# WarranWeng/EBFI-BE

Measured on AMD Instinct MI355X. Metric: interpolated frames/sec (train fwd+bwd) at B=8 256x256, higher is better.
Workload: dtype bf16x3 fwd (f16 KernelConv) / f16 bwd; 1 GPU; EVFIAutoEx (config/train_ours.yml defaults, 5.69 M params) train step: fwd + Lap/census loss + bwd + flat grad all-reduce + Adam; B=8 per GPU, 256x256 frames, TB=16 event bins, Poisson(0.35) event counts; global_batch=8, parallelism=dp1, world_size=1, launch=hipGraph replay of fwd+loss+bwd+grad packing; all-reduce and Adam eager, graph_capture_failed=False, fp16_steps_skipped=0

## Files before the change

ebfi-be_amd/csrc/conv2d.hip:

```cpp
#include <type_traits>

#include "common.hpp"
#include "c16.hpp"

using namespace ebfi;

namespace {

typedef float f32x16 __attribute__((ext_vector_type(16)));

enum { ACT_NONE = 0, ACT_LEAKY = 1, ACT_SIGMOID = 2 };

struct ConvGeom {
    int B, Cin, H, W, Cout, Ho, Wo, pad;
    int groups = 1;
    int store = 0;
};

struct EpiExtra {
    const float *addend;
    const float *mask_y;
    int mask_act;
    float mask_slope;
    _Float16 *out16 = nullptr;
// ... 1774 lines not shown
template <int KS, int DACT>
__global__ __launch_bounds__(256, 2) void conv_wgrad_bf16(const float *__restrict__ x, const float *__restrict__ gout,
                                                         const float *__restrict__ yact, float *__restrict__ slab,
                                                         ConvGeom g, float dslope, int total_tiles, int need_bias) {
    using C = WCfgB<KS>;
    constexpr int KK = KS * KS, WTX = C::WTX, CIB = C::CIB, ROWP = C::ROWP, PLANE = C::PLANE, GP = C::GP;
    constexpr int NI = C::NI, NTAP = C::NTAP;
    extern __shared__ __attribute__((aligned(16))) __bf16 smemb[];
    __bf16 *sG = smemb;
    __bf16 *sB = smemb + 64 * GP;
    unsigned *sG32 = reinterpret_cast<unsigned *>(sG), *sB32 = reinterpret_cast<unsigned *>(sB);

    const int tid = threadIdx.x, lane = tid & 63, wave = tid >> 6;
    const int co_base = blockIdx.y * 64, ci_base = blockIdx.z * CIB;
    const int ci_cnt = min(CIB, g.Cin - ci_base);
    const int mt = wave & 1, th = wave >> 1;
    const int tiles_x = (g.Wo + WTX - 1) / WTX, tiles_y = (g.Ho + WTY - 1) / WTY;
    const int HW = g.H * g.W, HWo = g.Ho * g.Wo;

    f32x16 acc[NTAP];
#pragma unroll
    for (int q = 0; q < NTAP; ++q)
#pragma unroll
        for (int r = 0; r < 16; ++r) acc[q][r] = 0.f;
    for (int i = tid; i < (KS * CIB * PLANE + ROWP) / 2; i += 256) sB32[i] = 0u;

    const int gp = tid & 31, grow = tid >> 5, gpy = gp >> 4, gpx = 2 * (gp & 15);
    const int pc = tid & 15, trow = tid >> 4;
    const unsigned go_bytes = (unsigned)g.Cout * (unsigned)HWo * 4u, x_bytes = (unsigned)g.Cin * (unsigned)HW * 4u;

    float rg[16], ri[2 * NI];
    float bsum = 0.f;
    auto prefetch = [&](int tile) {
        int t = tile;
        const int tx = t % tiles_x; t /= tiles_x;
        const int ty = t % tiles_y;
        const int b = t / tiles_y;
        const int y0 = ty * WTY, x0 = tx * WTX;
        const int iy0 = y0 - g.pad, ix0 = x0 - g.pad;
        const bool live = tile < total_tiles;
        const __amdgpu_buffer_rsrc_t rgo = make_rsrc(gout + (int64_t)(live ? b : 0) * g.Cout * HWo, live ? go_bytes : 0u);
        const __amdgpu_buffer_rsrc_t rya = make_rsrc((DACT ? yact : gout) + (int64_t)(live ? b : 0) * g.Cout * HWo,
                                                     (live && DACT) ? go_bytes : 0u);
        const __amdgpu_buffer_rsrc_t rxi = make_rsrc(x + (int64_t)(live ? b : 0) * g.Cin * HW, live ? x_bytes : 0u);
        const int gy = y0 + gpy, gx0 = x0 + gpx;
        const bool row_ok = gpx < WTX && gy < g.Ho;
        const unsigned base = (unsigned)((co_base + grow) * HWo + gy * g.Wo + gx0) * 4u;
        const unsigned g0 = (row_ok && gx0 < g.Wo) ? base : SENT, g1 = (row_ok && gx0 + 1 < g.Wo) ? base + 4u : SENT;
#pragma unroll
        for (int it = 0; it < 8; ++it) {
            const unsigned step = (unsigned)(8 * it) * (unsigned)HWo * 4u;
            float v0 = buf_ld(rgo, g0 + step), v1 = buf_ld(rgo, g1 + step);
            if constexpr (DACT != 0) {
                v0 *= act_grad_c<DACT>(buf_ld(rya, g0 + step), dslope);
                v1 *= act_grad_c<DACT>(buf_ld(rya, g1 + step), dslope);
            }
            rg[2 * it] = v0;
            rg[2 * it + 1] = v1;
        }
        const int xx = ix0 + 2 * pc;
        const bool c0_ok = xx >= 0 && xx < g.W, c1_ok = xx + 1 >= 0 && xx + 1 < g.W;
#pragma unroll
        for (int it = 0; it < NI; ++it) {
            const int r = it / (CIB / 16), ci = trow + 16 * (it % (CIB / 16));
            const int yy = iy0 + r;
            const bool r_ok = yy >= 0 && yy < g.H;
            const unsigned o = (unsigned)((ci_base + ci) * HW + yy * g.W + xx) * 4u;
            ri[2 * it] = buf_ld(rxi, (r_ok && c0_ok) ? o : SENT);
            ri[2 * it + 1] = buf_ld(rxi, (r_ok && c1_ok) ? o + 4u : SENT);
        }
    };
    auto commit = [&]() {
#pragma unroll
        for (int it = 0; it < 8; ++it) sG32[((grow + 8 * it) * GP) / 2 + gp] = pack_bf16(rg[2 * it], rg[2 * it + 1]);
#pragma unroll
        for (int it = 0; it < NI; ++it) {
            const int r = it / (CIB / 16), ci = trow + 16 * (it % (CIB / 16));
            const float v0 = ri[2 * it], v1 = ri[2 * it + 1];
            const int e = (ci * PLANE + r * ROWP) / 2 + pc;
            sB32[e] = pack_bf16(v0, v1);
            if constexpr (KS == 3) {
                const float nx = __shfl_down(v0, 1, 16);
                sB32[(CIB * PLANE) / 2 + e] = pack_bf16(v1, pc < 15 ? nx : 0.f);
                if (pc > 0) sB32[(2 * CIB * PLANE) / 2 + e - 1] = pack_bf16(v0, v1);
            }
        }
    };

    prefetch(blockIdx.x);
    for (int tile = blockIdx.x; tile < total_tiles; tile += gridDim.x) {
        __syncthreads();
        commit();
        __syncthreads();
        prefetch(tile + gridDim.x);
        if (need_bias && blockIdx.z == 0) {
            const bf16x8 *gq = reinterpret_cast<const bf16x8 *>(sG + (tid & 63) * GP + (tid >> 6) * 16);
            const bf16x8 u = gq[0], v = gq[1];
            float s = 0.f;
#pragma unroll
            for (int j = 0; j < 8; ++j) s += (float)u[j] + (float)v[j];
            bsum += s;
        }
        const __bf16 *ap = sG + (mt * 32 + (lane & 31)) * GP + (lane >> 5) * 8;
        const __bf16 *bp = sB + (lane & 31) * PLANE + (lane >> 5) * 8;
#pragma unroll
        for (int kk = 0; kk < 4; ++kk) {
            const bf16x8 a = *reinterpret_cast<const bf16x8 *>(ap + kk * 16);
#pragma unroll
            for (int j = 0; j < NTAP; ++j) {
                const int q = th * NTAP + j;
                if (q < KK) {
                    const int ky = q / KS, kx = q - ky * KS;
                    const bf16x8 bv = *reinterpret_cast<const bf16x8 *>(bp + kx * CIB * PLANE + ((kk >> 1) + ky) * ROWP +
                                                                        (kk & 1) * 16);
                    acc[j] = __builtin_amdgcn_mfma_f32_32x32x16_bf16(a, bv, acc[j], 0, 0, 0);
                }
            }
        }
    }
    const int64_t wsz = (int64_t)g.Cout * g.Cin * KK;
    float *my = slab + (int64_t)blockIdx.x * (wsz + g.Cout);
    const int ci = lane & 31;
    if (ci < ci_cnt) {
#pragma unroll
        for (int j = 0; j < NTAP; ++j) {
            const int q = th * NTAP + j;
            if (q >= KK) continue;
#pragma unroll
            for (int r = 0; r < 16; ++r) {
                const int co = co_base + mt * 32 + (r & 3) + 8 * (r >> 2) + 4 * (lane >> 5);
                if (co < g.Cout) my[((int64_t)co * KK + q) * g.Cin + ci_base + ci] = acc[j][r];
            }
        }
    }
    if (need_bias && blockIdx.z == 0) {
        __syncthreads();
        float *red = reinterpret_cast<float *>(smemb);
        red[tid] = bsum;
        __syncthreads();
        if (tid < 64 && co_base + tid < g.Cout)
            my[wsz + co_base + tid] = (red[tid] + red[tid + 64]) + (red[tid + 128] + red[tid + 192]);
    }
}

__global__ __launch_bounds__(256) void pack_table_bf16_kernel(const float *__restrict__ src, const int32_t *__restrict__ table,
                                                              int64_t n, __bf16 *__restrict__ out) {
    const int64_t e = (int64_t)blockIdx.x * 256 + threadIdx.x;
    if (e >= n) return;
    const int32_t t = table[e];
    float v = 0.f;
    if (t >= 0) v = src[t & 0x3fffffff];
    const __bf16 h = (__bf16)v;
    out[e] = (t >= 0 && (t & 0x40000000)) ? (__bf16)(v - (float)h) : h;
}

__device__ __forceinline__ void wgrad_reduce_body(const float *__restrict__ slab, int nslabs, int64_t n_weight, int64_t n_total,
                                                  float *__restrict__ gw, float *__restrict__ gb, int perm_cin, int perm_kk) {
    __shared__ float part[4][64];
    const int jj = threadIdx.x & 63, kq = threadIdx.x >> 6;
    const int64_t j = (int64_t)blockIdx.x * 64 + jj;
    float s0 = 0.f, s1 = 0.f, s2 = 0.f, s3 = 0.f;
    if (j < n_total) {
        const float *p = slab + j;
        int k = kq;
        for (; k + 28 < nslabs; k += 32) {
            const float a0 = p[(int64_t)k * n_total], a1 = p[(int64_t)(k + 4) * n_total];
            const float a2 = p[(int64_t)(k + 8) * n_total], a3 = p[(int64_t)(k + 12) * n_total];
            const float a4 = p[(int64_t)(k + 16) * n_total], a5 = p[(int64_t)(k + 20) * n_total];
            const float a6 = p[(int64_t)(k + 24) * n_total], a7 = p[(int64_t)(k + 28) * n_total];
            s0 += a0; s1 += a1; s2 += a2; s3 += a3;
            s0 += a4; s1 += a5; s2 += a6; s3 += a7;
        }
        for (; k + 12 < nslabs; k += 16) {
            s0 += p[(int64_t)k * n_total];
            s1 += p[(int64_t)(k + 4) * n_total];
            s2 += p[(int64_t)(k + 8) * n_total];
            s3 += p[(int64_t)(k + 12) * n_total];
        }
        for (; k < nslabs; k += 4) s0 += p[(int64_t)k * n_total];
    }
    part[kq][jj] = (s0 + s1) + (s2 + s3);
    __syncthreads();
    if (kq == 0 && j < n_total) {
        const float s = (part[0][jj] + part[1][jj]) + (part[2][jj] + part[3][jj]);
        if (j < n_weight) {
            int64_t o = j;
            if (perm_cin > 0) {
                const int ci = (int)(j % perm_cin);
                const int q = (int)((j / perm_cin) % perm_kk);
                const int64_t co = j / ((int64_t)perm_cin * perm_kk);
                o = (co * perm_cin + ci) * perm_kk + q;
            }
            gw[o] = s;
        } else if (gb) gb[j - n_weight] = s;
    }
}
__global__ __launch_bounds__(256) void conv_wgrad_reduce_f32(const float *__restrict__ slab, int nslabs,
                                                             int64_t n_weight, int64_t n_total,
                                                             float *__restrict__ gw, float *__restrict__ gb,
                                                             int perm_cin, int perm_kk) {
    wgrad_reduce_body(slab, nslabs, n_weight, n_total, gw, gb, perm_cin, perm_kk);
}
__global__ __launch_bounds__(256) void conv_wgrad_reduce_tall(const float *__restrict__ slab, int nslabs, int64_t n_weight, int64_t n_total,
                                                              float *__restrict__ gw, float *__restrict__ gb) {
    __shared__ float part[16][16];
    const int jj = threadIdx.x & 15, kq = threadIdx.x >> 4;
    const int64_t j = (int64_t)blockIdx.x * 16 + jj;
    float s0 = 0.f, s1 = 0.f, s2 = 0.f, s3 = 0.f;
    if (j < n_total) {
        const float *p = slab + j;
        int k = kq;
        for (; k + 112 < nslabs; k += 128) {
            float a[8];
#pragma unroll
            for (int i = 0; i < 8; ++i) a[i] = p[(int64_t)(k + 16 * i) * n_total];
            s0 += a[0]; s1 += a[1]; s2 += a[2]; s3 += a[3];
            s0 += a[4]; s1 += a[5]; s2 += a[6]; s3 += a[7];
        }
        for (; k < nslabs; k += 16) s0 += p[(int64_t)k * n_total];
    }
    part[kq][jj] = (s0 + s1) + (s2 + s3);
    __syncthreads();
    if (kq == 0 && j < n_total) {
        float s = 0.f;
#pragma unroll
        for (int i = 0; i < 16; ++i) s += part[i][jj];
        if (j < n_weight) gw[j] = s;
        else if (gb) gb[j - n_weight] = s;
    }
}
struct ReduceItem {
    const float *slab;
    float *gw, *gb;
    int64_t n_weight, n_total;
    int perm_cin;
};
struct ReduceBatch {
    ReduceItem item[4];
};
__global__ __launch_bounds__(256) void conv_wgrad_reduce_batch(ReduceBatch rb, int nslabs) {
    ReduceItem it = rb.item[0];
#pragma unroll
    for (int k = 1; k < 4; ++k)
        if ((int)blockIdx.y == k) it = rb.item[k];
    if ((int64_t)blockIdx.x * 64 >= it.n_total) return;
    wgrad_reduce_body(it.slab, nslabs, it.n_weight, it.n_total, it.gw, it.gb, it.perm_cin, 9);
}

double conv_bytes_fwd(const ConvGeom &g, int kk, bool dact) {
    return 4.0 * ((double)g.B * g.groups * g.Cin * g.H * g.W * (dact ? 2 : 1) + (double)g.B * g.Cout * g.Ho * g.Wo + (double)g.Cout * g.Cin * kk);
}
double conv_bytes_wgrad(const ConvGeom &g, int kk, bool dact, bool side_out) {
    return 4.0 * ((double)g.B * g.groups * g.Cin * g.H * g.W + (double)g.B * g.Cout * g.Ho * g.Wo * (1 + (dact ? 1 : 0) + (side_out ? 1 : 0)) +
                  (double)g.Cout * g.Cin * kk);
}

int make_geom(ConvGeom &g, int B, int Cin, int H, int W, int Cout, int ks, int stride, int pad) {
    if (B < 0 || Cin <= 0 || H <= 0 || W <= 0 || Cout <= 0) return fail(EBFI_ERR_ARG, "conv2d: non-positive dimension");
    if (ks != 1 && ks != 3 && ks != 7) return fail(EBFI_ERR_UNSUPPORTED, "conv2d: kernel size %d (1, 3 and 7 implemented)", ks);
    if (stride != 1 && stride != 2) return fail(EBFI_ERR_UNSUPPORTED, "conv2d: stride %d (1 and 2 implemented)", stride);
    if (pad < 0 || pad > ks) return fail(EBFI_ERR_ARG, "conv2d: padding %d out of range", pad);
    g = ConvGeom{B, Cin, H, W, Cout, (H + 2 * pad - ks) / stride + 1, (W + 2 * pad - ks) / stride + 1, pad};
    if (g.Ho <= 0 || g.Wo <= 0) return fail(EBFI_ERR_ARG, "conv2d: empty output");
    const int64_t lim = (1LL << 31) - (1LL << 26);
    if ((int64_t)(Cin + 64) * H * W * 4 >= lim || (int64_t)(Cout + 64) * g.Ho * g.Wo * 4 >= lim ||
        (int64_t)(Cout + 64) * (Cin + 64) * ks * ks * 4 >= lim)
        return fail(EBFI_ERR_ARG, "conv2d: one sample (or the weight) exceeds the 2 GiB reach of 32-bit buffer offsets");
    return EBFI_OK;
}

template <int KS, int S, bool TR, int DACT>
int launch_fwd_d(hipStream_t st, const float *x, const float *dact_y, const float *w, const float *bias, float *out,
                 const ConvGeom &g, int act, float slope, float dslope) {
    constexpr int CK = KS == 7 ? 2 : 8;
    const int64_t tiles = (int64_t)g.B * ceil_div(g.Ho, TY) * ceil_div(g.Wo, TX);
    if (tiles > 2147483647LL) return fail(EBFI_ERR_ARG, "conv2d: too many tiles");
    const char *name = TR ? "conv_fwd_f32/dgrad" : "conv_fwd_f32/fwd";
    const double flops = 2.0 * g.B * g.Ho * g.Wo * (double)g.Cout * g.Cin * KS * KS;
    if (g.Cout <= 32) {
        dim3 grid((unsigned)tiles, (unsigned)ceil_div(g.Cout, 32));
        ProfScope ps(name, st, flops, conv_bytes_fwd(g, KS * KS, DACT != 0));
        hipLaunchKernelGGL((conv_fwd_f32<KS, S, 1, CK, TR, DACT>), grid, dim3(256), 0, st, x, dact_y, w, bias, out, g, act,
                           slope, dslope);
    } else {
        dim3 grid((unsigned)tiles, (unsigned)ceil_div(g.Cout, 64));
        ProfScope ps(name, st, flops, conv_bytes_fwd(g, KS * KS, DACT != 0));
        hipLaunchKernelGGL((conv_fwd_f32<KS, S, 2, CK, TR, DACT>), grid, dim3(256), 0, st, x, dact_y, w, bias, out, g, act,
                           slope, dslope);
    }
    return check_launch(name);
}

template <int KS, int S, bool TR>
int launch_fwd(hipStream_t st, const float *x, const float *dact_y, const float *w, const float *bias, float *out,
               const ConvGeom &g, int act, float slope, int dact, float dslope) {
    if constexpr (TR) {
        if (dact == ACT_LEAKY) return launch_fwd_d<KS, S, TR, ACT_LEAKY>(st, x, dact_y, w, bias, out, g, act, slope, dslope);
        if (dact == ACT_SIGMOID) return launch_fwd_d<KS, S, TR, ACT_SIGMOID>(st, x, dact_y, w, bias, out, g, act, slope, dslope);
    }
    return launch_fwd_d<KS, S, TR, ACT_NONE>(st, x, dact_y, w, bias, out, g, act, slope, dslope);
}

int pick_wtx(int Wo) {
    int best = 30;
    int64_t best_cols = ceil_div(Wo, 30) * 30;
    for (int w : {28, 26}) {
// ... 748 lines not shown
                const int i = tid + (it0 + ii) * NTB;
                if (it0 + ii < C7_NWP && i < C7_PIECES) {
                    const int row = i >> 1, half = i & 1;
                    u32x4 hv, lv;
#pragma unroll
                    for (int j = 0; j < 4; ++j) {
                        const float v0f = wv[ii][2 * j], v1f = wv[ii][2 * j + 1];
                        const __bf16 a0 = (__bf16)v0f, a1 = (__bf16)v1f;
                        hv[j] = pack_bf16((float)a0, (float)a1);
                        lv[j] = pack_bf16(v0f - (float)a0, v1f - (float)a1);
                    }
                    const int d = 2 * C7S_INB + row * 32 + ((half ^ ((row >> 3) & 1)) << 4);
                    *reinterpret_cast<u32x4 *>(smd + d) = hv;
                    *reinterpret_cast<u32x4 *>(smd + C7_WB + d) = lv;
                }
            }
            __builtin_amdgcn_sched_barrier(0);
        }
        __syncthreads();
#pragma unroll
        for (int ky = 0; ky < 7; ++ky) {
            const int py = (ky + pad) & 1, dy = (py + pad - ky) / 2;
#pragma unroll
            for (int kx = 0; kx < 7; ++kx) {
                const int px = (kx + pad) & 1, dx = (px + pad - kx) / 2;
                const int ra = (ky * 7 + kx) * C7_ROWS + (l31 & 15);
                const char *ap = smd + 2 * C7S_INB + ra * 32 + ((hsel ^ ((ra >> 3) & 1)) << 4);
                const bf16x8 ah = *reinterpret_cast<const bf16x8 *>(ap), al = *reinterpret_cast<const bf16x8 *>(ap + C7_WB);
#pragma unroll
                for (int n = 0; n < 2; ++n) {
                    const int pos = (wave + dy + 1) * C7S_IW + l31 + n * 32 + dx + 1;
                    const char *bp = smd + pos * 32 + ((hsel ^ ((pos >> 3) & 1)) << 4);
                    const bf16x8 bh = *reinterpret_cast<const bf16x8 *>(bp), bl = *reinterpret_cast<const bf16x8 *>(bp + C7S_INB);
                    f32x16 &a = acc[py][px][n];
                    a = __builtin_amdgcn_mfma_f32_32x32x16_bf16(al, bh, a, 0, 0, 0);
                    a = __builtin_amdgcn_mfma_f32_32x32x16_bf16(ah, bl, a, 0, 0, 0);
                    a = __builtin_amdgcn_mfma_f32_32x32x16_bf16(ah, bh, a, 0, 0, 0);
                }
                if ((kx & 1) == 1) __builtin_amdgcn_sched_barrier(0);
            }
        }
    }
    const int u = u0 + wave;
#pragma unroll
    for (int py = 0; py < 2; ++py) {
        const int Y = 2 * u + py;
        if (u >= Hu || Y >= H) continue;
#pragma unroll
        for (int n = 0; n < 2; ++n) {
            const int v = v0 + n * 32 + l31, X = 2 * v;
            if (v >= Wu) continue;
#pragma unroll
            for (int r = 0; r < 16; ++r) {
                const int m = (r & 3) + 8 * (r >> 2) + 4 * hsel;
                if (m >= M) continue;
                float *o = gx + (((int64_t)b * M + m) * H + Y) * W + X;
                if (X + 1 < W && (W & 1) == 0) *reinterpret_cast<float2 *>(o) = make_float2(acc[py][0][n][r], acc[py][1][n][r]);
                else {
                    o[0] = acc[py][0][n][r];
                    if (X + 1 < W) o[1] = acc[py][1][n][r];
                }
            }
        }
    }
}

int launch_conv7s2_dgrad_x3(hipStream_t st, const float *g, const float *w, float *gx, int B, int K, int Hg, int Wg, int M, int H,
                            int W, int pad) {
    if (M > C7_ROWS) return fail(EBFI_ERR_UNSUPPORTED, "conv7s2_dgrad_x3: %d input channels (at most %d)", M, C7_ROWS);
    if (pad != 3) return fail(EBFI_ERR_UNSUPPORTED, "conv7s2_dgrad_x3: pad %d (3 only)", pad);
    if ((int64_t)K * Hg * Wg >= (int64_t)1 << 29) return fail(EBFI_ERR_UNSUPPORTED, "conv7s2_dgrad_x3: a sample of 2 GiB or more");
    if (int rc = ensure_dynamic_lds(reinterpret_cast<const void *>(&conv7s2_dgrad_x3_kernel<3>), C7S_LDS)) return rc;
    const int64_t tiles = (int64_t)B * ceil_div((H + 1) / 2, TYB) * ceil_div((W + 1) / 2, TX);
    {
        ProfScope ps("conv7_x3/dgrad_s2", st, 2.0 * B * (double)Hg * Wg * M * K * 49, 4.0 * B * ((double)K * Hg * Wg + (double)M * H * W));
        hipLaunchKernelGGL(conv7s2_dgrad_x3_kernel<3>, dim3((unsigned)tiles), dim3(NTB), C7S_LDS, st, g, w, gx, K, Hg, Wg, M, H, W);
    }
    return check_launch("conv7s2_dgrad_x3");
}

int launch_conv7_x3(hipStream_t st, const float *x, const float *w, const float *bias, float *out, int B, int K, int H, int W,
                    int M, int Ho, int Wo, int pad, int tr, int act, float slope, const char *role) {
    if (M > C7_ROWS) return fail(EBFI_ERR_UNSUPPORTED, "conv7_x3: %d output channels (at most %d)", M, C7_ROWS);
    if ((int64_t)K * H * W >= (int64_t)1 << 29) return fail(EBFI_ERR_UNSUPPORTED, "conv7_x3: a sample of 2 GiB or more");
    if (int rc = ensure_dynamic_lds(reinterpret_cast<const void *>(&conv7_x3_kernel), C7_LDS)) return rc;
    const int64_t tiles = (int64_t)B * ceil_div(Ho, TYB) * ceil_div(Wo, TX);
    {
        ProfScope ps(role, st, 2.0 * B * (double)Ho * Wo * M * K * 49, 4.0 * B * ((double)K * H * W + (double)M * Ho * Wo));
        hipLaunchKernelGGL(conv7_x3_kernel, dim3((unsigned)tiles), dim3(NTB), C7_LDS, st, x, w, bias, out, K, H, W, M, Ho, Wo, pad,
                           tr, act, slope);
    }
    return check_launch("conv7_x3");
}

int conv_forward_bf16_impl(const char *who, int x3, const void *input, const void *weight, const void *bias, void *output, int B,
                           int Cin, int H, int W, int Cout, int ksize, int stride, int pad, int act, float slope,
                           void *workspace, size_t workspace_bytes, void *stream) {
    if (!input || !output || (!weight && !(x3 && workspace))) return fail(EBFI_ERR_ARG, "%s: null argument", who);
    if (act < 0 || act > 2) return fail(EBFI_ERR_ARG, "%s: unknown activation %d", who, act);
    const bool k7 = x3 && ksize == 7 && stride == 1 && weight;
    if (!k7 && (stride != 1 || (ksize != 1 && ksize != 3)))
        return fail(EBFI_ERR_UNSUPPORTED, "%s: k=%d stride=%d (k in {1,3}, stride 1; split precision also k=7 with <= 16 output channels)",
                    who, ksize, stride);
    ConvGeom g;
    if (int rc = make_geom(g, B, Cin, H, W, Cout, ksize, stride, pad)) return rc;
    if (B == 0) return EBFI_OK;
    hipStream_t st = static_cast<hipStream_t>(stream);
    const float *x = static_cast<const float *>(input), *w = static_cast<const float *>(weight);
    const float *bs = static_cast<const float *>(bias);
    float *o = static_cast<float *>(output);
    if (k7) return launch_conv7_x3(st, x, w, bs, o, B, Cin, H, W, Cout, g.Ho, g.Wo, pad, 0, act, slope, "conv7_x3/fwd");
    if (ksize == 3) return launch_fwd_bf16<3>(st, x, nullptr, w, bs, o, g, 0, act, slope, 0, 0.f, workspace, workspace_bytes, x3);
    return launch_fwd_bf16<1>(st, x, nullptr, w, bs, o, g, 0, act, slope, 0, 0.f, workspace, workspace_bytes, x3);
}

int conv_backward_data_bf16_impl(const char *who, int x3, const void *grad_output, const void *saved_output, const void *weight,
                                 void *grad_input, int B, int Cin, int H, int W, int Cout, int ksize, int stride, int pad,
                                 int act, float slope, void *workspace, size_t workspace_bytes, void *stream) {
    if (!grad_output || !grad_input || (!weight && !(x3 && workspace))) return fail(EBFI_ERR_ARG, "%s: null argument", who);
    if (act != ACT_NONE && !saved_output) return fail(EBFI_ERR_ARG, "%s: activation needs saved_output", who);
    const bool k7 = x3 && ksize == 7 && stride == 1 && weight && act == ACT_NONE;
    if (stride != 1 || pad > ksize - 1 || (!k7 && ksize != 1 && ksize != 3))
        return fail(EBFI_ERR_UNSUPPORTED, "%s: k=%d stride=%d pad=%d", who, ksize, stride, pad);
    ConvGeom f;
    if (int rc = make_geom(f, B, Cin, H, W, Cout, ksize, stride, pad)) return rc;
    if (B == 0) return EBFI_OK;
    if (k7 && Cout == 3 && Cin == 16 && (int64_t)B * H * W >= 64 * 1024)
        return launch_conv7_thin_dgrad(static_cast<hipStream_t>(stream), static_cast<const float *>(grad_output), nullptr,
                                       static_cast<const float *>(weight), static_cast<float *>(grad_input), B, H, W, f.Ho, f.Wo, pad,
                                       ACT_NONE, 0.f);
    if (k7)
        return launch_conv7_x3(static_cast<hipStream_t>(stream), static_cast<const float *>(grad_output),
                               static_cast<const float *>(weight), nullptr, static_cast<float *>(grad_input), B, Cout, f.Ho, f.Wo,
                               Cin, H, W, ksize - 1 - pad, 1, ACT_NONE, 0.f, "conv7_x3/dgrad");
    ConvGeom g{B, Cout, f.Ho, f.Wo, Cin, H, W, ksize - 1 - pad};
    hipStream_t st = static_cast<hipStream_t>(stream);
    const float *go = static_cast<const float *>(grad_output), *yo = static_cast<const float *>(saved_output);
    const float *w = static_cast<const float *>(weight);
    float *gi = static_cast<float *>(grad_input);
    if (ksize == 3)
        return launch_fwd_bf16<3>(st, go, yo, w, nullptr, gi, g, 1, ACT_NONE, 0.f, act, slope, workspace, workspace_bytes, x3);
    return launch_fwd_bf16<1>(st, go, yo, w, nullptr, gi, g, 1, ACT_NONE, 0.f, act, slope, workspace, workspace_bytes, x3);
}
}

extern "C" int ebfi_pack_table_bf16(const float *src, const int32_t *table, int64_t n, void *out, void *stream) {
    if (!src || !table || !out || n < 0) return fail(EBFI_ERR_ARG, "pack_table_bf16: null argument");
    if (n == 0) return EBFI_OK;
    hipStream_t st = static_cast<hipStream_t>(stream);
    ProfScope ps("pack_table_bf16", st, 0.0, 10.0 * (double)n);
    hipLaunchKernelGGL(pack_table_bf16_kernel, dim3((unsigned)ceil_div(n, 256)), dim3(256), 0, st, src, table, n,
                       static_cast<__bf16 *>(out));
    return check_launch("pack_table_bf16");
}

extern "C" size_t ebfi_conv2d_packed_bytes(int Cin, int Cout, int ksize, int transposed) {
    return transposed ? 2 * bf16_pack_bytes(Cin, Cout, ksize) : 2 * bf16_pack_bytes(Cout, Cin, ksize);
}

extern "C" int ebfi_conv2d_pack_bf16x3(const void *weight, int Cin, int Cout, int ksize, int transposed, void *packed,
                                       size_t packed_bytes, void *stream) {
    if (!weight || !packed) return fail(EBFI_ERR_ARG, "conv2d_pack_bf16x3: null argument");
    if (Cin <= 0 || Cout <= 0 || (ksize != 1 && ksize != 3)) return fail(EBFI_ERR_ARG, "conv2d_pack_bf16x3: Cin %d Cout %d k %d", Cin, Cout, ksize);
    const int M = transposed ? Cin : Cout, K = transposed ? Cout : Cin, K16 = (K + 15) / 16 * 16;
    if (packed_bytes < ebfi_conv2d_packed_bytes(Cin, Cout, ksize, transposed))
        return fail(EBFI_ERR_WORKSPACE, "conv2d_pack_bf16x3: %zu bytes < required %zu", packed_bytes,
                    ebfi_conv2d_packed_bytes(Cin, Cout, ksize, transposed));
    hipStream_t st = static_cast<hipStream_t>(stream);
    const int64_t total = (int64_t)ksize * ksize * M * K16;
    ProfScope ps("conv_pack_w_bf16", st);
    hipLaunchKernelGGL(conv_pack_w_bf16, dim3((unsigned)ceil_div(total, 256)), dim3(256), 0, st, static_cast<const float *>(weight),
                       static_cast<__bf16 *>(packed), M, K, K16, ksize * ksize, transposed, 1);
    return check_launch("conv_pack_w_bf16");
}

extern "C" int ebfi_conv2d_forward_bf16mma(const void *input, const void *weight, const void *bias, void *output, int B,
                                           int Cin, int H, int W, int Cout, int ksize, int stride, int pad, int act,
                                           float slope, void *workspace, size_t workspace_bytes, void *stream) {
    return conv_forward_bf16_impl("conv2d_forward_bf16mma", 0, input, weight, bias, output, B, Cin, H, W, Cout, ksize, stride, pad,
                                  act, slope, workspace, workspace_bytes, stream);
}

extern "C" int ebfi_conv2d_backward_data_bf16mma(const void *grad_output, const void *saved_output, const void *weight,
                                                 void *grad_input, int B, int Cin, int H, int W, int Cout, int ksize,
                                                 int stride, int pad, int act, float slope, void *workspace,
                                                 size_t workspace_bytes, void *stream) {
    return conv_backward_data_bf16_impl("conv2d_backward_data_bf16mma", 0, grad_output, saved_output, weight, grad_input, B, Cin,
                                        H, W, Cout, ksize, stride, pad, act, slope, workspace, workspace_bytes, stream);
}

extern "C" int ebfi_conv2d_forward_bf16x3(const void *input, const void *weight, const void *bias, void *output, int B,
                                          int Cin, int H, int W, int Cout, int ksize, int stride, int pad, int act,
                                          float slope, void *workspace, size_t workspace_bytes, void *stream) {
    return conv_forward_bf16_impl("conv2d_forward_bf16x3", 1, input, weight, bias, output, B, Cin, H, W, Cout, ksize, stride, pad,
                                  act, slope, workspace, workspace_bytes, stream);
}

extern "C" int ebfi_conv2d_backward_data_bf16x3(const void *grad_output, const void *saved_output, const void *weight,
                                                void *grad_input, int B, int Cin, int H, int W, int Cout, int ksize,
                                                int stride, int pad, int act, float slope, void *workspace,
                                                size_t workspace_bytes, void *stream) {
    return conv_backward_data_bf16_impl("conv2d_backward_data_bf16x3", 1, grad_output, saved_output, weight, grad_input, B, Cin,
                                        H, W, Cout, ksize, stride, pad, act, slope, workspace, workspace_bytes, stream);
}

extern "C" int ebfi_conv2d_backward_data_s2_bf16x3(const void *grad_preact, const void *weight, void *grad_input, int B, int Cin,
                                                   int H, int W, int Cout, int ksize, int pad, void *stream) {
    if (!grad_preact || !weight || !grad_input) return fail(EBFI_ERR_ARG, "conv2d_backward_data_s2_bf16x3: null argument");
    if (ksize != 7) return fail(EBFI_ERR_UNSUPPORTED, "conv2d_backward_data_s2_bf16x3: k=%d (7 only)", ksize);
    ConvGeom f;
    if (int rc = make_geom(f, B, Cin, H, W, Cout, ksize, 2, pad)) return rc;
    if (B == 0) return EBFI_OK;
    return launch_conv7s2_dgrad_x3(static_cast<hipStream_t>(stream), static_cast<const float *>(grad_preact),
                                   static_cast<const float *>(weight), static_cast<float *>(grad_input), B, Cout, f.Ho, f.Wo, Cin, H, W,
                                   pad);
}

extern "C" int ebfi_conv2d_forward(const void *input, const void *weight, const void *bias, void *output, int B, int Cin,
                                   int H, int W, int Cout, int ksize, int stride, int pad, int act, float slope,
                                   int dtype, void *stream) {
    if (!input || !weight || !output) return fail(EBFI_ERR_ARG, "conv2d_forward: null argument");
    if (dtype != EBFI_F32) return fail(EBFI_ERR_UNSUPPORTED, "conv2d_forward: dtype %d not implemented (fp32 only)", dtype);
    if (act < 0 || act > 2) return fail(EBFI_ERR_ARG, "conv2d_forward: unknown activation %d", act);
    ConvGeom g;
    if (int rc = make_geom(g, B, Cin, H, W, Cout, ksize, stride, pad)) return rc;
    if (B == 0) return EBFI_OK;
    hipStream_t st = static_cast<hipStream_t>(stream);
    const float *x = static_cast<const float *>(input), *w = static_cast<const float *>(weight);
    const float *bs = static_cast<const float *>(bias);
    float *o = static_cast<float *>(output);
    if (ksize == 3 && stride == 1) return launch_fwd<3, 1, false>(st, x, nullptr, w, bs, o, g, act, slope, 0, 0.f);
    if (ksize == 3 && stride == 2) return launch_fwd<3, 2, false>(st, x, nullptr, w, bs, o, g, act, slope, 0, 0.f);
    if (ksize == 1 && stride == 1) return launch_fwd<1, 1, false>(st, x, nullptr, w, bs, o, g, act, slope, 0, 0.f);
    if (ksize == 7 && stride == 1) return launch_fwd<7, 1, false>(st, x, nullptr, w, bs, o, g, act, slope, 0, 0.f);
    if (ksize == 7 && stride == 2) return launch_fwd<7, 2, false>(st, x, nullptr, w, bs, o, g, act, slope, 0, 0.f);
    return fail(EBFI_ERR_UNSUPPORTED, "conv2d_forward: k=%d stride=%d not implemented", ksize, stride);
}

extern "C" int ebfi_conv2d_backward_data(const void *grad_output, const void *saved_output, const void *weight,
                                         void *grad_input, int B, int Cin, int H, int W, int Cout, int ksize,
                                         int stride, int pad, int act, float slope, int dtype, void *stream) {
    if (!grad_output || !weight || !grad_input) return fail(EBFI_ERR_ARG, "conv2d_backward_data: null argument");
    if (dtype != EBFI_F32) return fail(EBFI_ERR_UNSUPPORTED, "conv2d_backward_data: dtype %d not implemented", dtype);
    if (act != ACT_NONE && !saved_output) return fail(EBFI_ERR_ARG, "conv2d_backward_data: activation needs saved_output");
    if (stride != 1 || pad > ksize - 1)
        return fail(EBFI_ERR_UNSUPPORTED, "conv2d_backward_data: stride 1 and pad <= k-1 only (got s=%d p=%d k=%d); strided layers "
                    "zero-insert grad_output on the host side", stride, pad, ksize);
    ConvGeom f;
    if (int rc = make_geom(f, B, Cin, H, W, Cout, ksize, stride, pad)) return rc;
    if (B == 0) return EBFI_OK;
    ConvGeom g{B, Cout, f.Ho, f.Wo, Cin, H, W, ksize - 1 - pad};
    hipStream_t st = static_cast<hipStream_t>(stream);
    const float *go = static_cast<const float *>(grad_output), *yo = static_cast<const float *>(saved_output);
    const float *w = static_cast<const float *>(weight);
    float *gi = static_cast<float *>(grad_input);
    if (ksize == 3) return launch_fwd<3, 1, true>(st, go, yo, w, nullptr, gi, g, ACT_NONE, 0.f, act, slope);
    if (ksize == 7) return launch_fwd<7, 1, true>(st, go, yo, w, nullptr, gi, g, ACT_NONE, 0.f, act, slope);
    return launch_fwd<1, 1, true>(st, go, yo, w, nullptr, gi, g, ACT_NONE, 0.f, act, slope);
}

extern "C" size_t ebfi_conv2d_backward_weight_workspace(int B, int Cin, int H, int W, int Cout, int ksize, int stride,
                                                        int pad, int dtype) {
    (void)dtype;
    ConvGeom g;
    if (make_geom(g, B, Cin, H, W, Cout, ksize, stride, pad) != EBFI_OK) return 0;
    int slabs = wgrad_splits(g, ksize, stride);
    if (thin_wgrad_geometry(g, ksize, stride).kind != 0 && thin_wgrad_slabs(g) > slabs)
        slabs = thin_wgrad_slabs(g);
    if (const ShiftPlan sp = shift_wgrad_geometry(g, ksize, stride); sp.kind != 0 && shift_wgrad_slabs(g, sp) > slabs)
        slabs = shift_wgrad_slabs(g, sp);
    return (size_t)slabs * ((size_t)Cout * Cin * ksize * ksize + Cout) * sizeof(float);
}

extern "C" int ebfi_conv2d_backward_weight_ex(const void *input, const void *grad_output, const void *saved_output,
                                              void *grad_weight, void *grad_bias, void *grad_preact_out, int B, int Cin,
                                              int H, int W, int Cout, int ksize, int stride, int pad, int act, float slope,
                                              void *workspace, size_t workspace_bytes, int dtype, void *stream);

extern "C" int ebfi_conv2d_backward_weight(const void *input, const void *grad_output, const void *saved_output,
                                           void *grad_weight, void *grad_bias, int B, int Cin, int H, int W, int Cout,
                                           int ksize, int stride, int pad, int act, float slope, void *workspace,
                                           size_t workspace_bytes, int dtype, void *stream) {
    return ebfi_conv2d_backward_weight_ex(input, grad_output, saved_output, grad_weight, grad_bias, nullptr, B, Cin, H, W,
                                          Cout, ksize, stride, pad, act, slope, workspace, workspace_bytes, dtype, stream);
}

extern "C" int ebfi_conv2d_backward_weight_ex(const void *input, const void *grad_output, const void *saved_output,
                                              void *grad_weight, void *grad_bias, void *grad_preact_out, int B, int Cin,
                                              int H, int W, int Cout, int ksize, int stride, int pad, int act, float slope,
                                              void *workspace, size_t workspace_bytes, int dtype, void *stream) {
    if (!input || !grad_output || !grad_weight) return fail(EBFI_ERR_ARG, "conv2d_backward_weight: null argument");
    const bool bf16mma = dtype == EBFI_F32_BF16MMA && stride == 1 && (ksize == 1 || ksize == 3);
    const bool x3 = dtype == EBFI_F32_BF16X3MMA && stride == 1 && (ksize == 1 || ksize == 3 || ksize == 7);
    if (dtype != EBFI_F32 && dtype != EBFI_F32_BF16MMA && dtype != EBFI_F32_BF16X3MMA)
        return fail(EBFI_ERR_UNSUPPORTED, "conv2d_backward_weight: dtype %d not implemented", dtype);
    if (act != ACT_NONE && !saved_output) return fail(EBFI_ERR_ARG, "conv2d_backward_weight: activation needs saved_output");
    ConvGeom g;
    if (int rc = make_geom(g, B, Cin, H, W, Cout, ksize, stride, pad)) return rc;
    const size_t need = ebfi_conv2d_backward_weight_workspace(B, Cin, H, W, Cout, ksize, stride, pad, dtype);
    if (!workspace || workspace_bytes < need)
        return fail(EBFI_ERR_WORKSPACE, "conv2d_backward_weight: workspace %zu bytes < required %zu", workspace_bytes, need);
    hipStream_t st = static_cast<hipStream_t>(stream);
    const int64_t n_weight = (int64_t)Cout * Cin * ksize * ksize, n_total = n_weight + Cout;
    if (B == 0) {
        (void)hipMemsetAsync(grad_weight, 0, (size_t)n_weight * sizeof(float), st);
        if (grad_bias) (void)hipMemsetAsync(grad_bias, 0, (size_t)Cout * sizeof(float), st);
// ... 677 lines not shown
```

ebfi-be_amd/csrc/fuse.hip:

```cpp
#include "common.hpp"
#include "c16.hpp"

using namespace ebfi;

namespace {

typedef float f4 __attribute__((ext_vector_type(4)));

__global__ __launch_bounds__(256) void src_fwd_kernel(const float *__restrict__ a0, const float *__restrict__ s0,
                                                      const float *__restrict__ a1, const float *__restrict__ s1,
                                                      const float *__restrict__ x, float *__restrict__ out, int C, int64_t HW4,
                                                      int64_t total4, int64_t a_bs4) {
    const int64_t i = (int64_t)blockIdx.x * 256 + threadIdx.x;
    if (i >= total4) return;
    const int64_t bc = i / HW4, r = i - bc * HW4;
    const int64_t b = bc / C, c = bc - b * C;
    const f4 zero = {0.f, 0.f, 0.f, 0.f};
    const f4 xv = x ? reinterpret_cast<const f4 *>(x)[i] : zero;
    const int64_t ia = b * a_bs4 + c * HW4 + r;
    const f4 v0 = reinterpret_cast<const f4 *>(a0)[ia], v1 = reinterpret_cast<const f4 *>(a1)[ia];
    const float k0 = s0[bc], k1 = s1 ? s1[bc] : 1.f;
    f4 *o = reinterpret_cast<f4 *>(out);
    o[(b * 2 * C + c) * HW4 + r] = v0 * k0 + xv;
    o[(b * 2 * C + C + c) * HW4 + r] = v1 * k1 + xv;
// ... 160 lines not shown
    }
    ScaleSlot{slot}.record(amax);
}

__global__ __launch_bounds__(256) void src_fwd_c16_kernel(const float *__restrict__ a0, const float *__restrict__ s0,
                                                          const float *__restrict__ a1, const float *__restrict__ s1,
                                                          const float *__restrict__ x, float *__restrict__ out,
                                                          _Float16 *__restrict__ out16, float *__restrict__ slot, int C, int64_t HW4,
                                                          int W4, int64_t total, int64_t a_bs4) {
    saturate_fp16_conversions();
    const int64_t i = (int64_t)blockIdx.x * 256 + threadIdx.x;
    float amax = 0.f;
    if (i < total) {
        const int64_t q = i % HW4, bg = i / HW4;
        const int64_t G8 = 2 * C / 8, b = bg / G8, cg = bg - b * G8;
        const int64_t co = cg * 8;
        const bool second = co >= C;
        const int64_t c = second ? co - C : co;
        const f4 *pa = reinterpret_cast<const f4 *>(second ? a1 : a0) + b * a_bs4 + c * HW4 + q;
        const f4 *px = reinterpret_cast<const f4 *>(x) + (b * C + c) * HW4 + q;
        const float *ps = (second ? s1 : s0) + b * C + c;
        f4 v[8];
#pragma unroll
        for (int e = 0; e < 8; ++e) v[e] = pa[e * HW4] * ps[e] + px[e * HW4];
        if (out) {
            f4 *o = reinterpret_cast<f4 *>(out) + (b * 2 * C + co) * HW4 + q;
#pragma unroll
            for (int e = 0; e < 8; ++e) o[e * HW4] = v[e];
        }
        c16_store_quad(out16, c16_piece(b, 2 * C / 16, cg / 2, HW4, q, W4, (int)(cg & 1)), v, slot[0], amax);
    }
    ScaleSlot{slot}.record(amax);
}

template <bool A16>
__global__ __launch_bounds__(256) void src_bwd_c16_kernel(const float *__restrict__ gout, const float *__restrict__ a0,
                                                          const float *__restrict__ s0, const float *__restrict__ a1,
                                                          const float *__restrict__ s1, _Float16 *__restrict__ ga16,
                                                          float *__restrict__ slot, float *__restrict__ gx, float *__restrict__ gs0p,
                                                          float *__restrict__ gs1p, int B, int C, int64_t HW4, int W4, int64_t a_bs4,
                                                          int nslice, float mask_slope, const float *__restrict__ a_slot = nullptr) {
    saturate_fp16_conversions();
    __shared__ float red[4][16];
    const int G8 = C / 8;
    const int slice = blockIdx.x % nslice, bg = blockIdx.x / nslice;
    const int b = bg / G8, cg = bg - b * G8, c = cg * 8;
    const int64_t q0 = HW4 * slice / nslice, q1 = HW4 * (slice + 1) / nslice;
    float k0[8], k1[8], d0[8], d1[8];
#pragma unroll
    for (int e = 0; e < 8; ++e) k0[e] = s0[b * C + c + e], k1[e] = s1[b * C + c + e], d0[e] = 0.f, d1[e] = 0.f;
    const float sc = slot[0];
    float amax = 0.f;
    auto dm = [&](const f4 &v) {
        f4 m;
        m.x = v.x > 0.f ? 1.f : mask_slope; m.y = v.y > 0.f ? 1.f : mask_slope;
        m.z = v.z > 0.f ? 1.f : mask_slope; m.w = v.w > 0.f ? 1.f : mask_slope;
        return m;
    };
    const f4 *g0 = reinterpret_cast<const f4 *>(gout) + ((int64_t)b * 2 * C + c) * HW4;
    const f4 *g1 = reinterpret_cast<const f4 *>(gout) + ((int64_t)b * 2 * C + C + c) * HW4;
    const f4 *p0 = reinterpret_cast<const f4 *>(a0) + (int64_t)b * a_bs4 + (int64_t)c * HW4;
    const f4 *p1 = reinterpret_cast<const f4 *>(a1) + (int64_t)b * a_bs4 + (int64_t)c * HW4;
    [[maybe_unused]] const _Float16 *img = reinterpret_cast<const _Float16 *>(a0);
    [[maybe_unused]] const float ainv = A16 ? 1.f / a_slot[0] : 1.f;
    auto quad_from_image = [&](int64_t piece0, f4 (&v)[8]) {
        u4 pc[4];
#pragma unroll
        for (int j = 0; j < 4; ++j) pc[j] = *reinterpret_cast<const u4 *>(img + (piece0 + j) * 8);
#pragma unroll
        for (int e = 0; e < 8; ++e) {
#pragma unroll
            for (int j = 0; j < 4; ++j) {
                const unsigned wd = pc[j][e >> 1];
                const _Float16 hv = __builtin_bit_cast(_Float16, (unsigned short)((e & 1) ? (wd >> 16) : (wd & 0xffffu)));
                v[e][j] = (float)hv * ainv;
            }
        }
    };
    f4 *ox = reinterpret_cast<f4 *>(gx) + ((int64_t)b * C + c) * HW4;
    for (int64_t q = q0 + threadIdx.x; q < q1; q += 256) {
        f4 u0[8], u1[8], w[8], va[8];
#pragma unroll
        for (int e = 0; e < 8; ++e) u0[e] = g0[e * HW4 + q], u1[e] = g1[e * HW4 + q];
#pragma unroll
        for (int e = 0; e < 8; ++e) ox[e * HW4 + q] = u0[e] + u1[e];
        const int64_t pc0 = c16_piece(b, 2 * C / 16, cg / 2, HW4, q, W4, cg & 1);
        const int64_t pc1 = c16_piece(b, 2 * C / 16, (C + c) / 16, HW4, q, W4, ((C + c) >> 3) & 1);
        if constexpr (A16) quad_from_image(pc0, va);
#pragma unroll
        for (int e = 0; e < 8; ++e) {
            const f4 v = A16 ? va[e] : p0[e * HW4 + q];
            d0[e] += (u0[e].x * v.x + u0[e].y * v.y) + (u0[e].z * v.z + u0[e].w * v.w);
            w[e] = u0[e] * k0[e] * dm(v);
        }
        c16_store_quad(ga16, pc0, w, sc, amax);
        if constexpr (A16) quad_from_image(pc1, va);
#pragma unroll
        for (int e = 0; e < 8; ++e) {
            const f4 v = A16 ? va[e] : p1[e * HW4 + q];
            d1[e] += (u1[e].x * v.x + u1[e].y * v.y) + (u1[e].z * v.z + u1[e].w * v.w);
            w[e] = u1[e] * k1[e] * dm(v);
        }
        c16_store_quad(ga16, pc1, w, sc, amax);
    }
#pragma unroll
    for (int e = 0; e < 8; ++e)
#pragma unroll
        for (int d = 32; d >= 1; d >>= 1) {
            d0[e] += __shfl_xor(d0[e], d, 64);
            d1[e] += __shfl_xor(d1[e], d, 64);
        }
    if ((threadIdx.x & 63) == 0) {
#pragma unroll
        for (int e = 0; e < 8; ++e) red[threadIdx.x >> 6][e] = d0[e], red[threadIdx.x >> 6][8 + e] = d1[e];
    }
    __syncthreads();
    if (threadIdx.x < 16) {
        const float v = (red[0][threadIdx.x] + red[1][threadIdx.x]) + (red[2][threadIdx.x] + red[3][threadIdx.x]);
        float *dst = threadIdx.x < 8 ? gs0p : gs1p;
        dst[((int64_t)slice * B + b) * C + c + (threadIdx.x & 7)] = v;
    }
    ScaleSlot{slot}.record(amax);
}

int check_planes(const char *who, int B, int C, int64_t HW) {
    if (B < 0 || C <= 0 || HW <= 0) return fail(EBFI_ERR_ARG, "%s: bad dimensions", who);
    if (HW % 4 != 0) return fail(EBFI_ERR_UNSUPPORTED, "%s: H*W must be a multiple of 4 (got %lld)", who, (long long)HW);
    if ((int64_t)B * C > 2147483647LL) return fail(EBFI_ERR_ARG, "%s: too many planes", who);
    return EBFI_OK;
}


constexpr int SC_MAX_LAYERS = 32, SC_MAX_K = 8;
struct ScalarBank {
    const float *w[SC_MAX_LAYERS];
    const float *b[SC_MAX_LAYERS];
};

__global__ __launch_bounds__(256) void scalar_conv_fwd_kernel(ScalarBank bank, const float *__restrict__ v, float *__restrict__ out,
                                                              int B, int K, int C, float slope) {
    const int s = blockIdx.x;
    const float *w = nullptr, *bias = nullptr;
#pragma unroll
    for (int j = 0; j < SC_MAX_LAYERS; ++j)
        if (j == s) { w = bank.w[j]; bias = bank.b[j]; }
    for (int i = threadIdx.x; i < B * C; i += 256) {
        const int b = i / C, c = i - b * C;
        float acc = bias ? bias[c] : 0.f;
        for (int k = 0; k < K; ++k) acc = fmaf(v[b * K + k], w[c * K + k], acc);
        out[((int64_t)s * B + b) * C + c] = acc > 0.f ? acc : acc * slope;
    }
}

__global__ __launch_bounds__(256) void scalar_conv_bwd_kernel(ScalarBank bank, const float *__restrict__ v, const float *__restrict__ out,
                                                              const float *__restrict__ gout, float *__restrict__ gw, float *__restrict__ gb,
                                                              float *__restrict__ gv, int S, int B, int K, int C, float slope) {
    for (int i = threadIdx.x; i < S * C; i += 256) {
        const int s = i / C, c = i - s * C;
        float aw[SC_MAX_K], ab = 0.f;
#pragma unroll
        for (int k = 0; k < SC_MAX_K; ++k) aw[k] = 0.f;
        for (int b = 0; b < B; ++b) {
            const int64_t o = ((int64_t)s * B + b) * C + c;
            const float gp = gout[o] * (out[o] > 0.f ? 1.f : slope);
            ab += gp;
#pragma unroll
            for (int k = 0; k < SC_MAX_K; ++k)
                if (k < K) aw[k] = fmaf(gp, v[b * K + k], aw[k]);
        }
        if (gb) gb[i] = ab;
        if (gw) {
#pragma unroll
            for (int k = 0; k < SC_MAX_K; ++k)
                if (k < K) gw[(int64_t)i * K + k] = aw[k];
        }
    }
    if (gv) {
        const int wave = threadIdx.x >> 6, lane = threadIdx.x & 63;
        for (int p = wave; p < B * K; p += 4) {
            const int b = p / K, k = p - b * K;
            float acc = 0.f;
            for (int s = 0; s < S; ++s) {
                const float *w = nullptr;
#pragma unroll
                for (int j = 0; j < SC_MAX_LAYERS; ++j)
                    if (j == s) w = bank.w[j];
                for (int c = lane; c < C; c += 64) {
                    const int64_t o = ((int64_t)s * B + b) * C + c;
                    acc = fmaf(gout[o] * (out[o] > 0.f ? 1.f : slope), w[c * K + k], acc);
                }
            }
#pragma unroll
            for (int d = 32; d >= 1; d >>= 1) acc += __shfl_xor(acc, d, 64);
            if (lane == 0) gv[p] = acc;
        }
    }
}
}

extern "C" int ebfi_scale_residual_cat_forward_ex(const float *a0, const float *s0, const float *a1, const float *s1,
                                                  const float *x, float *out, int B, int C, int64_t HW, int64_t a_batch_stride,
                                                  void *stream);
extern "C" int ebfi_scale_residual_cat_forward(const float *a0, const float *s0, const float *a1, const float *s1,
                                               const float *x, float *out, int B, int C, int64_t HW, void *stream) {
    return ebfi_scale_residual_cat_forward_ex(a0, s0, a1, s1, x, out, B, C, HW, (int64_t)C * HW, stream);
}

extern "C" int ebfi_scale_residual_cat_forward_ex(const float *a0, const float *s0, const float *a1, const float *s1,
                                                  const float *x, float *out, int B, int C, int64_t HW, int64_t a_batch_stride,
                                                  void *stream) {
    if (!a0 || !s0 || !a1 || !out) return fail(EBFI_ERR_ARG, "scale_residual_cat_forward: null argument");
    if (a_batch_stride % 4 != 0 || a_batch_stride < (int64_t)C * HW) return fail(EBFI_ERR_ARG, "scale_residual_cat_forward: batch stride");
    if (int rc = check_planes("scale_residual_cat_forward", B, C, HW)) return rc;
    if (B == 0) return EBFI_OK;
    hipStream_t st = static_cast<hipStream_t>(stream);
    const int64_t total4 = (int64_t)B * C * HW / 4;
    {
        ProfScope ps("scale_residual_cat_fwd", st, 0.0, 20.0 * B * C * (double)HW);
        hipLaunchKernelGGL(src_fwd_kernel, dim3((unsigned)ceil_div(total4, 256)), dim3(256), 0, st, a0, s0, a1, s1, x, out, C, HW / 4,
                           total4, a_batch_stride / 4);
    }
    return check_launch("scale_residual_cat_fwd");
}

extern "C" int ebfi_scale_residual_cat_backward_ex(const float *grad_out, const float *a0, const float *s0, const float *a1,
                                                   const float *s1, float *grad_a0, float *grad_a1, float *grad_x,
                                                   float *grad_s0, float *grad_s1, int B, int C, int64_t HW,
                                                   int64_t a_batch_stride, int64_t grad_a_batch_stride, int mask_leaky,
                                                   float mask_slope, void *stream);
extern "C" int ebfi_scale_residual_cat_backward(const float *grad_out, const float *a0, const float *s0, const float *a1,
                                                const float *s1, float *grad_a0, float *grad_a1, float *grad_x,
                                                float *grad_s0, float *grad_s1, int B, int C, int64_t HW, void *stream) {
    return ebfi_scale_residual_cat_backward_ex(grad_out, a0, s0, a1, s1, grad_a0, grad_a1, grad_x, grad_s0, grad_s1, B, C, HW,
                                               (int64_t)C * HW, (int64_t)C * HW, 0, 0.f, stream);
}

extern "C" int ebfi_scale_residual_cat_backward_ex(const float *grad_out, const float *a0, const float *s0, const float *a1,
                                                   const float *s1, float *grad_a0, float *grad_a1, float *grad_x,
                                                   float *grad_s0, float *grad_s1, int B, int C, int64_t HW,
                                                   int64_t a_batch_stride, int64_t grad_a_batch_stride, int mask_leaky,
                                                   float mask_slope, void *stream) {
    if (a_batch_stride % 4 != 0 || grad_a_batch_stride % 4 != 0 || a_batch_stride < (int64_t)C * HW ||
        grad_a_batch_stride < (int64_t)C * HW || (mask_leaky && !a1))
        return fail(EBFI_ERR_ARG, "scale_residual_cat_backward: batch stride / mask");
    if (!grad_out || !a0 || !s0 || !grad_a0 || !grad_a1 || !grad_s0 || (s1 && (!a1 || !grad_s1)))
        return fail(EBFI_ERR_ARG, "scale_residual_cat_backward: null argument");
    if (int rc = check_planes("scale_residual_cat_backward", B, C, HW)) return rc;
    if (B == 0) return EBFI_OK;
    hipStream_t st = static_cast<hipStream_t>(stream);
    {
        ProfScope ps("scale_residual_cat_bwd", st, 0.0, 28.0 * B * C * (double)HW);
        hipLaunchKernelGGL(src_bwd_kernel, dim3((unsigned)(B * C)), dim3(256), 0, st, grad_out, a0, s0, a1, s1, grad_a0, grad_a1,
                           grad_x, grad_s0, grad_s1, C, HW / 4, a_batch_stride / 4, grad_a_batch_stride / 4, mask_leaky, mask_slope);
    }
    return check_launch("scale_residual_cat_bwd");
}

extern "C" int ebfi_to_c16(const float *src, const float *mask_y, float mask_slope, void *dst16, void *slot, int B, int C, int H, int W,
                           void *stream) {
    const int64_t HW = (int64_t)H * W;
    if (!src || !dst16 || !slot) return fail(EBFI_ERR_ARG, "to_c16: null argument");
    if (W % 4 != 0) return fail(EBFI_ERR_UNSUPPORTED, "to_c16: W %% 4 != 0 (W = %d)", W);
    if (C % 16 != 0) return fail(EBFI_ERR_UNSUPPORTED, "to_c16: %d channels (multiples of 16)", C);
    if (int rc = check_planes("to_c16", B, C, HW)) return rc;
    if (!aligned16(src) || !aligned16(dst16) || (mask_y && !aligned16(mask_y))) return fail(EBFI_ERR_ARG, "to_c16: 16-byte aligned tensors");
    if (B == 0) return EBFI_OK;
    hipStream_t st = static_cast<hipStream_t>(stream);
    const int64_t total = (int64_t)B * (C / 8) * (HW / 4);
    {
        ProfScope ps("to_c16", st, 0.0, (mask_y ? 10.0 : 6.0) * B * C * (double)HW);
        hipLaunchKernelGGL(to_c16_kernel, dim3((unsigned)ceil_div(total, 256)), dim3(256), 0, st, src, mask_y, mask_slope,
                           static_cast<_Float16 *>(dst16), static_cast<float *>(slot), C, HW / 4, W / 4, total);
    }
    return check_launch("to_c16");
}

extern "C" int ebfi_to_c16_cat2(const float *src0, int C0, const float *src1, int C1, void *dst16, void *slot, int B, int H, int W,
                                void *stream) {
    const int64_t HW = (int64_t)H * W;
    if (!src0 || !src1 || !dst16 || !slot) return fail(EBFI_ERR_ARG, "to_c16_cat2: null argument");
    if (W % 4 != 0) return fail(EBFI_ERR_UNSUPPORTED, "to_c16_cat2: W %% 4 != 0 (W = %d)", W);
    if (C0 < 8 || C1 < 8 || C0 % 8 != 0 || C1 % 8 != 0 || (C0 + C1) % 16 != 0)
        return fail(EBFI_ERR_UNSUPPORTED, "to_c16_cat2: %d + %d channels (multiples of 8, a multiple of 16 together)", C0, C1);
    if (int rc = check_planes("to_c16_cat2", B, C0 + C1, HW)) return rc;
    if (!aligned16(src0) || !aligned16(src1) || !aligned16(dst16)) return fail(EBFI_ERR_ARG, "to_c16_cat2: 16-byte aligned tensors");
    if (B == 0) return EBFI_OK;
    hipStream_t st = static_cast<hipStream_t>(stream);
    const int64_t total = (int64_t)B * ((C0 + C1) / 8) * (HW / 4);
    {
        ProfScope ps("to_c16/cat2", st, 0.0, 6.0 * B * (C0 + C1) * (double)HW);
        hipLaunchKernelGGL(to_c16_cat2_kernel, dim3((unsigned)ceil_div(total, 256)), dim3(256), 0, st, src0, C0, src1, C1,
                           static_cast<_Float16 *>(dst16), static_cast<float *>(slot), HW / 4, W / 4, total);
    }
    return check_launch("to_c16/cat2");
}

extern "C" int ebfi_scale_residual_cat_forward_c16(const float *a0, const float *s0, const float *a1, const float *s1, const float *x,
                                                   float *out, void *out16, void *slot, int B, int C, int H, int W,
                                                   int64_t a_batch_stride, void *stream) {
    const int64_t HW = (int64_t)H * W;
    if (!a0 || !s0 || !a1 || !s1 || !x || !out16 || !slot) return fail(EBFI_ERR_ARG, "scale_residual_cat_forward_c16: null argument");
    if (W % 4 != 0) return fail(EBFI_ERR_UNSUPPORTED, "scale_residual_cat_forward_c16: W %% 4 != 0 (W = %d)", W);
    if (a_batch_stride % 4 != 0 || a_batch_stride < (int64_t)C * HW) return fail(EBFI_ERR_ARG, "scale_residual_cat_forward_c16: batch stride");
    if (C % 8 != 0) return fail(EBFI_ERR_UNSUPPORTED, "scale_residual_cat_forward_c16: %d channels (multiples of 8)", C);
    if (int rc = check_planes("scale_residual_cat_forward_c16", B, C, HW)) return rc;
    if (B == 0) return EBFI_OK;
    hipStream_t st = static_cast<hipStream_t>(stream);
    const int64_t total = (int64_t)B * (2 * C / 8) * (HW / 4);
    {
        ProfScope ps("scale_residual_cat_fwd", st, 0.0, (out ? 24.0 : 16.0) * B * C * (double)HW);
        hipLaunchKernelGGL(src_fwd_c16_kernel, dim3((unsigned)ceil_div(total, 256)), dim3(256), 0, st, a0, s0, a1, s1, x, out,
                           static_cast<_Float16 *>(out16), static_cast<float *>(slot), C, HW / 4, W / 4, total, a_batch_stride / 4);
    }
    return check_launch("scale_residual_cat_fwd");
}

extern "C" int ebfi_scale_residual_cat_backward_slices(void) { return 8; }

extern "C" int ebfi_scale_residual_cat_backward_c16(const float *grad_out, const float *a0, const float *s0, const float *a1,
                                                    const float *s1, void *grad_a16, void *slot, float *grad_x, float *grad_s0_part,
                                                    float *grad_s1_part, int B, int C, int H, int W, int64_t a_batch_stride,
                                                    float mask_slope, void *stream) {
    const int64_t HW = (int64_t)H * W;
    if (W % 4 != 0) return fail(EBFI_ERR_UNSUPPORTED, "scale_residual_cat_backward_c16: W %% 4 != 0 (W = %d)", W);
    if (!grad_out || !a0 || !s0 || !a1 || !s1 || !grad_a16 || !slot || !grad_x || !grad_s0_part || !grad_s1_part)
        return fail(EBFI_ERR_ARG, "scale_residual_cat_backward_c16: null argument");
    if (a_batch_stride % 4 != 0 || a_batch_stride < (int64_t)C * HW) return fail(EBFI_ERR_ARG, "scale_residual_cat_backward_c16: batch stride");
    if (C % 16 != 0) return fail(EBFI_ERR_UNSUPPORTED, "scale_residual_cat_backward_c16: %d channels (multiples of 16)", C);
    if (int rc = check_planes("scale_residual_cat_backward_c16", B, C, HW)) return rc;
    if (B == 0) return EBFI_OK;
    hipStream_t st = static_cast<hipStream_t>(stream);
    const int nslice = ebfi_scale_residual_cat_backward_slices();
    {
        ProfScope ps("scale_residual_cat_bwd", st, 0.0, 24.0 * B * C * (double)HW);
        hipLaunchKernelGGL(src_bwd_c16_kernel<false>, dim3((unsigned)(B * (C / 8) * nslice)), dim3(256), 0, st, grad_out, a0, s0, a1, s1,
                           static_cast<_Float16 *>(grad_a16), static_cast<float *>(slot), grad_x, grad_s0_part, grad_s1_part, B, C,
                           HW / 4, W / 4, a_batch_stride / 4, nslice, mask_slope, nullptr);
    }
    return check_launch("scale_residual_cat_bwd");
}

extern "C" int ebfi_scale_residual_cat_backward_c16a(const float *grad_out, const void *a16, const void *a_slot, const float *s0,
                                                     const float *s1, void *grad_a16, void *slot, float *grad_x, float *grad_s0_part,
                                                     float *grad_s1_part, int B, int C, int H, int W, float mask_slope, void *stream) {
    const int64_t HW = (int64_t)H * W;
    if (W % 4 != 0) return fail(EBFI_ERR_UNSUPPORTED, "scale_residual_cat_backward_c16a: W %% 4 != 0 (W = %d)", W);
    if (!grad_out || !a16 || !a_slot || !s0 || !s1 || !grad_a16 || !slot || !grad_x || !grad_s0_part || !grad_s1_part)
        return fail(EBFI_ERR_ARG, "scale_residual_cat_backward_c16a: null argument");
    if (C % 16 != 0) return fail(EBFI_ERR_UNSUPPORTED, "scale_residual_cat_backward_c16a: %d channels (multiples of 16)", C);
    if (!aligned16(a16) || !aligned16(grad_a16)) return fail(EBFI_ERR_ARG, "scale_residual_cat_backward_c16a: 16-byte aligned images");
    if (int rc = check_planes("scale_residual_cat_backward_c16a", B, C, HW)) return rc;
    if (B == 0) return EBFI_OK;
    hipStream_t st = static_cast<hipStream_t>(stream);
    const int nslice = ebfi_scale_residual_cat_backward_slices();
    {
        ProfScope ps("scale_residual_cat_bwd", st, 0.0, 20.0 * B * C * (double)HW);
        hipLaunchKernelGGL(src_bwd_c16_kernel<true>, dim3((unsigned)(B * (C / 8) * nslice)), dim3(256), 0, st, grad_out,
                           static_cast<const float *>(a16), s0, static_cast<const float *>(a16), s1, static_cast<_Float16 *>(grad_a16),
                           static_cast<float *>(slot), grad_x, grad_s0_part, grad_s1_part, B, C, HW / 4, W / 4, (int64_t)0, nslice,
                           mask_slope, static_cast<const float *>(a_slot));
    }
    return check_launch("scale_residual_cat_bwd");
}

extern "C" int ebfi_gather_sum(const float *src, const int32_t *idx, float *out, int64_t n_out, int R, void *stream) {
    if (!src || !idx || !out) return fail(EBFI_ERR_ARG, "gather_sum: null argument");
    if (n_out < 0 || R <= 0) return fail(EBFI_ERR_ARG, "gather_sum: bad dimensions");
    if (n_out == 0) return EBFI_OK;
    hipStream_t st = static_cast<hipStream_t>(stream);
    hipLaunchKernelGGL(gather_sum_kernel, dim3((unsigned)ceil_div(n_out, 256)), dim3(256), 0, st, src, idx, out, n_out, R);
    return check_launch("gather_sum");
}

extern "C" int ebfi_prodmean_forward(const float *a, const float *b, float *out, int64_t planes, int64_t HW, void *stream) {
    if (!a || !b || !out) return fail(EBFI_ERR_ARG, "prodmean_forward: null argument");
    if (planes < 0 || planes > 2147483647LL || HW <= 0) return fail(EBFI_ERR_ARG, "prodmean_forward: bad dimensions");
    if (HW % 4 != 0) return fail(EBFI_ERR_UNSUPPORTED, "prodmean_forward: H*W must be a multiple of 4");
    if (planes == 0) return EBFI_OK;
    hipStream_t st = static_cast<hipStream_t>(stream);
    {
        ProfScope ps("prodmean_fwd", st, 0.0, 8.0 * planes * (double)HW);
        hipLaunchKernelGGL(prodmean_fwd_kernel, dim3((unsigned)planes), dim3(256), 0, st, a, b, out, HW / 4);
    }
    return check_launch("prodmean_fwd");
}

extern "C" int ebfi_prodmean_backward(const float *a, const float *b, const float *grad_out, float *grad_a, float *grad_b,
                                      int64_t planes, int64_t HW, void *stream) {
    if (!a || !b || !grad_out || !grad_a || !grad_b) return fail(EBFI_ERR_ARG, "prodmean_backward: null argument");
    if (planes < 0 || HW <= 0) return fail(EBFI_ERR_ARG, "prodmean_backward: bad dimensions");
    if (HW % 4 != 0) return fail(EBFI_ERR_UNSUPPORTED, "prodmean_backward: H*W must be a multiple of 4");
    if (planes == 0) return EBFI_OK;
    hipStream_t st = static_cast<hipStream_t>(stream);
    const int64_t total4 = planes * HW / 4;
    {
        ProfScope ps("prodmean_bwd", st, 0.0, 16.0 * planes * (double)HW);
        hipLaunchKernelGGL(prodmean_bwd_kernel, dim3((unsigned)ceil_div(total4, 256)), dim3(256), 0, st, a, b, grad_out, grad_a, grad_b,
                           HW / 4, total4);
    }
    return check_launch("prodmean_bwd");
}

static int scalar_bank(ScalarBank &bank, const void *const *weights, const void *const *biases, int S, int B, int K, int C, const char *what) {
    if (!weights || S < 1 || S > SC_MAX_LAYERS || K < 1 || K > SC_MAX_K || B < 0 || C < 1 || (int64_t)S * B * C > (1 << 20))
        return fail(EBFI_ERR_ARG, "%s: S = %d layers (<= %d), K = %d (<= %d), B = %d, C = %d", what, S, SC_MAX_LAYERS, K, SC_MAX_K, B, C);
    for (int j = 0; j < SC_MAX_LAYERS; ++j) {
        bank.w[j] = j < S ? static_cast<const float *>(weights[j]) : nullptr;
        bank.b[j] = (j < S && biases) ? static_cast<const float *>(biases[j]) : nullptr;
        if (j < S && !bank.w[j]) return fail(EBFI_ERR_ARG, "%s: weight %d is NULL", what, j);
    }
    return EBFI_OK;
}

extern "C" int ebfi_scalar_conv_forward(const float *v, const void *const *weights, const void *const *biases, float *out, int S, int B,
                                        int K, int C, float slope, void *stream) {
    ScalarBank bank;
    if (int rc = scalar_bank(bank, weights, biases, S, B, K, C, "scalar_conv_forward")) return rc;
    if (!v || !out) return fail(EBFI_ERR_ARG, "scalar_conv_forward: null argument");
    if (B == 0) return EBFI_OK;
    hipStream_t st = static_cast<hipStream_t>(stream);
    {
        ProfScope ps("scalar_conv_fwd", st, 2.0 * S * B * C * K, 4.0 * (S * (double)C * (K + 1) + B * K + (double)S * B * C));
        hipLaunchKernelGGL(scalar_conv_fwd_kernel, dim3((unsigned)S), dim3(256), 0, st, bank, v, out, B, K, C, slope);
    }
    return check_launch("scalar_conv_fwd");
}

extern "C" int ebfi_scalar_conv_backward(const float *v, const void *const *weights, const float *out, const float *grad_out,
                                         float *grad_weight, float *grad_bias, float *grad_v, int S, int B, int K, int C, float slope,
                                         void *stream) {
    ScalarBank bank;
    if (int rc = scalar_bank(bank, weights, nullptr, S, B, K, C, "scalar_conv_backward")) return rc;
    if (!v || !out || !grad_out) return fail(EBFI_ERR_ARG, "scalar_conv_backward: null argument");
    if (B == 0) return EBFI_OK;
    hipStream_t st = static_cast<hipStream_t>(stream);
    {
        ProfScope ps("scalar_conv_bwd", st, 4.0 * S * B * C * K, 4.0 * (2.0 * S * B * C + 2.0 * S * C * (K + 1) + 2.0 * B * K));
        hipLaunchKernelGGL(scalar_conv_bwd_kernel, dim3(1), dim3(256), 0, st, bank, v, out, grad_out, grad_weight, grad_bias, grad_v,
                           S, B, K, C, slope);
    }
    return check_launch("scalar_conv_bwd");
}
```

ebfi-be_amd/csrc/imgops.hip:

```cpp
#include "common.hpp"

using namespace ebfi;

namespace {

__device__ __forceinline__ int reflect(int i, int n) {
    if (i < 0) return -i;
    if (i >= n) return 2 * (n - 1) - i;
    return i;
}

__global__ void gauss5_fwd_kernel(const float *__restrict__ x, float *__restrict__ out, int64_t planes, int H, int W,
                                  float factor) {
    const int64_t idx = (int64_t)blockIdx.x * blockDim.x + threadIdx.x;
    const int64_t hw = (int64_t)H * W;
    if (idx >= planes * hw) return;
    const int64_t p = idx / hw;
    const int y = (int)((idx - p * hw) / W), xx = (int)(idx - p * hw - (int64_t)y * W);
    const float k[5] = {1.f / 16, 4.f / 16, 6.f / 16, 4.f / 16, 1.f / 16};
    const float *src = x + p * hw;
    float acc = 0.f;
#pragma unroll
    for (int i = 0; i < 5; ++i) {
        const float *row = src + (int64_t)reflect(y + i - 2, H) * W;
        float h = 0.f;
#pragma unroll
        for (int j = 0; j < 5; ++j) h += k[j] * row[reflect(xx + j - 2, W)];
        acc += k[i] * h;
    }
    out[idx] = acc * factor;
}

__global__ void gauss5_bwd_kernel(const float *__restrict__ gout, float *__restrict__ gin, int64_t planes, int H, int W,
                                  float factor) {
    const int64_t idx = (int64_t)blockIdx.x * blockDim.x + threadIdx.x;
    const int64_t hw = (int64_t)H * W;
    if (idx >= planes * hw) return;
    const int64_t p = idx / hw;
    const int y = (int)((idx - p * hw) / W), xx = (int)(idx - p * hw - (int64_t)y * W);
    const float k[5] = {1.f / 16, 4.f / 16, 6.f / 16, 4.f / 16, 1.f / 16};
    const float *src = gout + p * hw;
    int vy[3], vx[3], ny = 0, nx = 0;
    vy[ny++] = y;
    if (y >= 1 && y <= 2) vy[ny++] = -y;
    if (y >= H - 3 && y <= H - 2) vy[ny++] = 2 * (H - 1) - y;
    vx[nx++] = xx;
    if (xx >= 1 && xx <= 2) vx[nx++] = -xx;
    if (xx >= W - 3 && xx <= W - 2) vx[nx++] = 2 * (W - 1) - xx;
    float acc = 0.f;
    for (int a = 0; a < ny; ++a)
        for (int i = 0; i < 5; ++i) {
            const int oy = vy[a] - i + 2;
            if (oy < 0 || oy >= H) continue;
            const float *row = src + (int64_t)oy * W;
            float h = 0.f;
            for (int b = 0; b < nx; ++b)
#pragma unroll
                for (int j = 0; j < 5; ++j) {
                    const int ox = vx[b] - j + 2;
                    if (ox >= 0 && ox < W) h += k[j] * row[ox];
                }
            acc += k[i] * h;
        }
    gin[idx] = acc * factor;
}

constexpr int CT = 16, CR = 3, CTW = CT + 2 * CR;

__device__ __forceinline__ void census_stage(const float *__restrict__ x, const float *__restrict__ y, int C, int H, int W,
                                             int b, int ty0, int tx0, float (*gx)[CTW + 1], float (*gy)[CTW + 1]) {
    const int64_t hw = (int64_t)H * W;
    const float invc = 1.f / (float)C;
    for (int i = threadIdx.x; i < CTW * CTW; i += CT * CT) {
        const int ly = i / CTW, lx = i - ly * CTW;
        const int py = ty0 + ly - CR, px = tx0 + lx - CR;
        float sx = 0.f, sy = 0.f;
        if (py >= 0 && py < H && px >= 0 && px < W) {
            const int64_t o = (int64_t)b * C * hw + (int64_t)py * W + px;
            for (int c = 0; c < C; ++c) {
                sx += x[o + c * hw];
                sy += y[o + c * hw];
            }
            sx *= invc;
            sy *= invc;
        }
        gx[ly][lx] = sx;
        gy[ly][lx] = sy;
    }
}

__device__ __forceinline__ float census_t(float d) { return d * rsqrtf(0.81f + d * d); }

__global__ __launch_bounds__(CT *CT) void census_fwd_kernel(const float *__restrict__ x, const float *__restrict__ y,
                                                            float *__restrict__ partial, int C, int H, int W) {
    __shared__ float gx[CTW][CTW + 1], gy[CTW][CTW + 1];
    __shared__ float red[4];
    const int b = blockIdx.z, ty0 = blockIdx.y * CT, tx0 = blockIdx.x * CT;
    census_stage(x, y, C, H, W, b, ty0, tx0, gx, gy);
    __syncthreads();
    const int ly = threadIdx.x / CT, lx = threadIdx.x % CT;
    const int py = ty0 + ly, px = tx0 + lx;
    float acc = 0.f;
    if (py >= CR && py < H - CR && px >= CR && px < W - CR) {
        const float cx = gx[ly + CR][lx + CR], cy = gy[ly + CR][lx + CR];
#pragma unroll
        for (int i = 0; i < 7; ++i)
#pragma unroll
            for (int j = 0; j < 7; ++j) {
                const float u = census_t(gx[ly + i][lx + j] - cx) - census_t(gy[ly + i][lx + j] - cy);
                const float q = u * u;
                acc += q / (0.1f + q);
            }
        acc *= (1.f / 49.f);
    }
#pragma unroll
    for (int d = 32; d >= 1; d >>= 1) acc += __shfl_xor(acc, d, 64);
    if ((threadIdx.x & 63) == 0) red[threadIdx.x >> 6] = acc;
    __syncthreads();
    if (threadIdx.x == 0)
        partial[((int64_t)b * gridDim.y + blockIdx.y) * gridDim.x + blockIdx.x] = (red[0] + red[1]) + (red[2] + red[3]);
}

__device__ __forceinline__ float census_dterm(float dx, float dy) {
    const float rx = rsqrtf(0.81f + dx * dx);
    const float u = dx * rx - census_t(dy);
    const float den = 0.1f + u * u;
    return (0.2f * u / (den * den)) * (0.81f * rx * rx * rx);
}

__global__ __launch_bounds__(CT *CT) void census_bwd_kernel(const float *__restrict__ x, const float *__restrict__ y,
                                                            const float *__restrict__ grad_loss, float *__restrict__ grad_x,
                                                            int C, int H, int W, float norm) {
    __shared__ float gx[CTW][CTW + 1], gy[CTW][CTW + 1];
    const int b = blockIdx.z, ty0 = blockIdx.y * CT, tx0 = blockIdx.x * CT;
    census_stage(x, y, C, H, W, b, ty0, tx0, gx, gy);
    __syncthreads();
    const int ly = threadIdx.x / CT, lx = threadIdx.x % CT;
    const int py = ty0 + ly, px = tx0 + lx;
    if (py >= H || px >= W) return;
    const float cx = gx[ly + CR][lx + CR], cy = gy[ly + CR][lx + CR];
    const float self_in = (py >= CR && py < H - CR && px >= CR && px < W - CR) ? 1.f : 0.f;
    float acc = 0.f;
#pragma unroll
    for (int i = 0; i < 7; ++i) {
        const int qy = py + (i - CR);
        const bool row_in = qy >= CR && qy < H - CR;
#pragma unroll
        for (int j = 0; j < 7; ++j) {
            const int qx = px + (j - CR);
            const float wgt = self_in + ((row_in && qx >= CR && qx < W - CR) ? 1.f : 0.f);
            acc -= wgt * census_dterm(gx[ly + i][lx + j] - cx, gy[ly + i][lx + j] - cy);
        }
    }
    const float g = acc * norm * grad_loss[0] / (float)C;
    const int64_t hw = (int64_t)H * W;
    for (int c = 0; c < C; ++c) grad_x[((int64_t)b * C + c) * hw + (int64_t)py * W + px] = g;
}

template <bool REPLICATE>
__global__ __launch_bounds__(256) void pad2d_bwd_kernel(const float *__restrict__ gp, float *__restrict__ gx, int64_t planes,
                                                        int H, int W, int p) {
    const int Hp = H + 2 * p, Wp = W + 2 * p;
    const int64_t total = planes * H * W;
    const int64_t idx = (int64_t)blockIdx.x * 256 + threadIdx.x;
    if (idx >= total) return;
    const int j = (int)(idx % W);
    const int i = (int)((idx / W) % H);
    const int64_t pl = idx / ((int64_t)W * H);
    const float *g = gp + pl * Hp * Wp;
    float acc = 0.f;
    if constexpr (REPLICATE) {
        const int ylo = i == 0 ? 0 : i + p, yhi = i == H - 1 ? H - 1 + 2 * p : i + p;
        const int xlo = j == 0 ? 0 : j + p, xhi = j == W - 1 ? W - 1 + 2 * p : j + p;
        for (int y = ylo; y <= yhi; ++y)
            for (int x = xlo; x <= xhi; ++x) acc += g[(int64_t)y * Wp + x];
    } else {
        int ys[3], xs[3], ny = 0, nx = 0;
        ys[ny++] = i + p;
        if (i >= 1 && i <= p) ys[ny++] = p - i;
        if (i <= H - 2 && i >= H - 1 - p) ys[ny++] = 2 * (H - 1) - i + p;
        xs[nx++] = j + p;
        if (j >= 1 && j <= p) xs[nx++] = p - j;
        if (j <= W - 2 && j >= W - 1 - p) xs[nx++] = 2 * (W - 1) - j + p;
        for (int a = 0; a < ny; ++a)
            for (int b = 0; b < nx; ++b) acc += g[(int64_t)ys[a] * Wp + xs[b]];
    }
    gx[idx] = acc;
}

}

extern "C" int ebfi_pad2d_backward(const float *grad_padded, float *grad_input, int64_t planes, int H, int W, int pad, int replicate,
                                   void *stream) {
    if (!grad_padded || !grad_input) return fail(EBFI_ERR_ARG, "pad2d_backward: null argument");
    if (planes < 0 || H < 1 || W < 1 || pad < 0 || (!replicate && (pad >= H || pad >= W)))
        return fail(EBFI_ERR_ARG, "pad2d_backward: pad %d on %d x %d (reflection needs pad < H, W)", pad, H, W);
    if (planes == 0) return EBFI_OK;
    hipStream_t st = static_cast<hipStream_t>(stream);
    const int64_t total = planes * H * W;
    {
        ProfScope ps(replicate ? "replicate_pad_bwd" : "reflect_pad_bwd", st, 0.0, 4.0 * ((double)total + (double)planes * (H + 2 * pad) * (W + 2 * pad)));
        if (replicate)
            hipLaunchKernelGGL(pad2d_bwd_kernel<true>, dim3((unsigned)ceil_div(total, (int64_t)256)), dim3(256), 0, st, grad_padded, grad_input,
                               planes, H, W, pad);
        else
            hipLaunchKernelGGL(pad2d_bwd_kernel<false>, dim3((unsigned)ceil_div(total, (int64_t)256)), dim3(256), 0, st, grad_padded, grad_input,
                               planes, H, W, pad);
    }
    return check_launch("pad2d_bwd");
}

extern "C" int ebfi_gauss5_forward(const float *input, float *output, int64_t planes, int H, int W, float factor,
                                   void *stream) {
    if (!input || !output || planes < 0 || H < 3 || W < 3) return fail(EBFI_ERR_ARG, "gauss5_forward: bad argument (H, W >= 3)");
    if (planes == 0) return EBFI_OK;
    hipStream_t st = static_cast<hipStream_t>(stream);
    const int64_t total = planes * H * W;
    {
        ProfScope ps("gauss5_fwd", st, 0.0, 8.0 * total);
        hipLaunchKernelGGL(gauss5_fwd_kernel, dim3((unsigned)ceil_div(total, 256)), dim3(256), 0, st, input, output, planes, H, W,
                           factor);
    }
    return check_launch("gauss5_fwd");
}

extern "C" int ebfi_gauss5_backward(const float *grad_output, float *grad_input, int64_t planes, int H, int W, float factor,
                                    void *stream) {
    if (!grad_output || !grad_input || planes < 0 || H < 3 || W < 3)
        return fail(EBFI_ERR_ARG, "gauss5_backward: bad argument (H, W >= 3)");
    if (planes == 0) return EBFI_OK;
    hipStream_t st = static_cast<hipStream_t>(stream);
    const int64_t total = planes * H * W;
    {
        ProfScope ps("gauss5_bwd", st, 0.0, 8.0 * total);
        hipLaunchKernelGGL(gauss5_bwd_kernel, dim3((unsigned)ceil_div(total, 256)), dim3(256), 0, st, grad_output, grad_input,
                           planes, H, W, factor);
    }
    return check_launch("gauss5_bwd");
}

extern "C" int64_t ebfi_census_partials(int B, int H, int W) { return (int64_t)B * ceil_div(H, CT) * ceil_div(W, CT); }

extern "C" int ebfi_census_forward(const float *x, const float *y, float *partial, int B, int C, int H, int W, void *stream) {
    if (!x || !y || !partial) return fail(EBFI_ERR_ARG, "census_forward: null argument");
    if (B < 0 || C <= 0 || H <= 0 || W <= 0 || B > 65535) return fail(EBFI_ERR_ARG, "census_forward: bad dimensions");
    if (B == 0) return EBFI_OK;
    hipStream_t st = static_cast<hipStream_t>(stream);
    {
        ProfScope ps("census_fwd", st, 0.0, 8.0 * B * C * (double)H * W);
        hipLaunchKernelGGL(census_fwd_kernel, dim3(ceil_div(W, CT), ceil_div(H, CT), B), dim3(CT * CT), 0, st, x, y, partial, C, H, W);
    }
    return check_launch("census_fwd");
}

extern "C" int ebfi_census_backward(const float *x, const float *y, const float *grad_loss, float *grad_x, int B, int C, int H,
                                    int W, void *stream) {
    if (!x || !y || !grad_loss || !grad_x) return fail(EBFI_ERR_ARG, "census_backward: null argument");
    if (B < 0 || C <= 0 || H <= 0 || W <= 0 || B > 65535) return fail(EBFI_ERR_ARG, "census_backward: bad dimensions");
    if (B == 0) return EBFI_OK;
    hipStream_t st = static_cast<hipStream_t>(stream);
    const float norm = (float)(1.0 / (49.0 * (double)B * (double)H * (double)W));
    {
        ProfScope ps("census_bwd", st, 0.0, 12.0 * B * C * (double)H * W);
        hipLaunchKernelGGL(census_bwd_kernel, dim3(ceil_div(W, CT), ceil_div(H, CT), B), dim3(CT * CT), 0, st, x, y, grad_loss,
                           grad_x, C, H, W, norm);
    }
    return check_launch("census_bwd");
}
```

ebfi-be_amd/ebfi_amd/_native.py:

```python
import ctypes
import os
import re
import subprocess
import threading

PKG_ROOT = os.path.dirname(os.path.dirname(os.path.abspath(__file__)))
REPO_ROOT = os.path.dirname(PKG_ROOT)
_DEV = os.environ.get("EBFI_DEV") == "1"


def dev_env(name, default=None):
    return os.environ.get(name, default) if _DEV else default


LIB_PATH = dev_env("EBFI_LIB_PATH") or os.path.join(PKG_ROOT, "lib", "libebfi_hip.so")
HEADER = os.path.join(REPO_ROOT, "include", "ebfi_hip.h")
BUILD_SCRIPT = os.path.join(PKG_ROOT, "csrc", "build.sh")

EBFI_F32, EBFI_F32_BF16MMA, EBFI_F32_BF16X3MMA = 0, 2, 3
EBFI_ERR_UNSUPPORTED = -3
ABI_VERSION = 14


class EbfiNativeError(RuntimeError):
    pass


_lock = threading.Lock()
_lib = None

_c = ctypes
_vp, _i, _i64, _sz = _c.c_void_p, _c.c_int, _c.c_int64, _c.c_size_t
_p64 = _c.POINTER(_c.c_int64)

SIGNATURES = {
    "ebfi_abi_version": (_i, []),
    "ebfi_last_error": (_c.c_char_p, []),
    "ebfi_fac_forward": (_i, [_vp, _p64, _p64, _vp, _p64, _p64, _i, _vp, _p64, _p64, _i, _vp]),
    "ebfi_fac_backward": (_i, [_vp, _p64, _p64, _vp, _p64, _p64, _i, _vp, _p64, _vp, _p64, _vp, _p64, _i, _vp]),
    "ebfi_fac_backward_ex": (_i, [_vp, _p64, _p64, _vp, _p64, _p64, _i, _vp, _p64, _vp, _p64, _vp, _p64, _c.c_float, _i, _vp]),
    "ebfi_dcn_forward": (_i, [_vp] * 6 + [_i] * 14 + [_i, _vp]),
    "ebfi_dcn_backward_workspace": (_sz, [_i] * 14 + [_i]),
    "ebfi_dcn_backward": (_i, [_vp] * 11 + [_i] * 14 + [_vp, _sz, _i, _vp]),
    "ebfi_conv2d_forward": (_i, [_vp] * 4 + [_i] * 8 + [_i, _c.c_float, _i, _vp]),
    "ebfi_conv2d_backward_data": (_i, [_vp] * 4 + [_i] * 8 + [_i, _c.c_float, _i, _vp]),
    "ebfi_conv2d_backward_weight_workspace": (_sz, [_i] * 8 + [_i]),
    "ebfi_conv2d_backward_weight": (_i, [_vp] * 5 + [_i] * 8 + [_i, _c.c_float, _vp, _sz, _i, _vp]),
    "ebfi_conv2d_backward_weight_ex": (_i, [_vp] * 6 + [_i] * 8 + [_i, _c.c_float, _vp, _sz, _i, _vp]),
    "ebfi_conv2d_bf16_workspace": (_sz, [_i, _i, _i]),
    "ebfi_conv2d_forward_bf16mma": (_i, [_vp] * 4 + [_i] * 8 + [_i, _c.c_float, _vp, _sz, _vp]),
    "ebfi_conv2d_backward_data_bf16mma": (_i, [_vp] * 4 + [_i] * 8 + [_i, _c.c_float, _vp, _sz, _vp]),
    "ebfi_conv2d_forward_bf16x3": (_i, [_vp] * 4 + [_i] * 8 + [_i, _c.c_float, _vp, _sz, _vp]),
    "ebfi_conv2d_backward_data_bf16x3": (_i, [_vp] * 4 + [_i] * 8 + [_i, _c.c_float, _vp, _sz, _vp]),
    "ebfi_conv2d_packed_bytes": (_sz, [_i, _i, _i, _i]),
    "ebfi_conv2d_pack_bf16x3": (_i, [_vp, _i, _i, _i, _i, _vp, _sz, _vp]),
    "ebfi_pack_table_bf16": (_i, [_vp, _vp, _i64, _vp, _vp]),
    "ebfi_f16_scales_finish": (_i, [_vp, _i, _vp, _vp]),
    "ebfi_pack_table_f16": (_i, [_vp, _vp, _i64, _vp, _vp, _vp, _vp]),
    "ebfi_conv2d_packed_f16": (_i, [_vp, _vp, _sz, _vp, _vp] + [_i] * 8 + [_i, _c.c_float, _vp, _vp, _i, _c.c_float, _vp, _vp, _vp]),
    "ebfi_conv2d_backward_weight_f16g": (_i, [_vp] * 6 + [_i] * 8 + [_i, _c.c_float, _vp, _vp, _vp, _sz, _vp]),
    "ebfi_conv2d_backward_weight_f16g_ex": (_i, [_vp] * 6 + [_i] * 9 + [_i, _c.c_float, _vp, _vp, _vp, _sz, _vp]),
    "ebfi_to_c16": (_i, [_vp, _vp, _c.c_float, _vp, _vp, _i, _i, _i, _i, _vp]),
    "ebfi_to_c16_cat2": (_i, [_vp, _i, _vp, _i, _vp, _vp, _i, _i, _i, _vp]),
    "ebfi_conv2d_packed_x3_c16": (_i, [_vp, _vp, _sz, _vp, _vp] + [_i] * 8 + [_i, _c.c_float, _vp, _vp, _i, _c.c_float, _vp, _vp, _i, _vp]),
    "ebfi_conv2d_packed_f16_c16": (_i, [_vp, _i, _vp, _sz, _vp, _vp] + [_i] * 8 + [_i, _c.c_float, _vp, _vp, _i, _c.c_float,
                                        _vp, _vp, _vp, _vp, _i, _i, _vp]),
    "ebfi_conv2d_backward_weight_f16c": (_i, [_vp, _vp, _i, _vp, _vp] + [_i] * 6 + [_vp, _vp, _vp, _sz, _vp]),
    "ebfi_conv2d_backward_weight_f16c_batch_workspace": (_sz, [_i, _vp, _vp]),
    "ebfi_conv2d_backward_weight_f16c_batch": (_i, [_i] + [_vp] * 9 + [_i, _i, _i, _vp, _sz, _vp]),
    "ebfi_fac_forward_p16": (_i, [_vp, _i, _vp, _vp, _vp, _i, _i, _i, _i, _i, _vp]),
    "ebfi_fac_backward_p16": (_i, [_vp, _i, _vp, _vp, _vp, _vp, _vp, _vp, _c.c_float, _i, _i, _i, _i, _i, _vp]),
    "ebfi_scale_residual_cat_forward_c16": (_i, [_vp] * 8 + [_i, _i, _i, _i, _i64, _vp]),
    "ebfi_scale_residual_cat_backward_slices": (_i, []),
    "ebfi_scale_residual_cat_backward_c16": (_i, [_vp] * 10 + [_i, _i, _i, _i, _i64, _c.c_float, _vp]),
    "ebfi_scale_residual_cat_backward_c16a": (_i, [_vp] * 10 + [_i, _i, _i, _i, _c.c_float, _vp]),
    "ebfi_conv2d_packed_x3_rc": (_i, [_vp, _vp, _sz, _vp, _vp] + [_i] * 6 + [_c.c_float, _vp, _vp, _i, _vp, _vp, _vp, _vp, _vp]),
    "ebfi_conv2d_thin_forward": (_i, [_vp, _vp, _vp, _vp] + [_i] * 8 + [_i, _c.c_float, _vp]),
    "ebfi_kernelconv_fac_fused_x3": (_i, [_vp, _vp, _sz, _vp, _vp, _vp] + [_i] * 6 + [_c.c_float, _vp]),
    "ebfi_kernelconv_fac_fused_f16": (_i, [_vp, _i, _vp, _sz, _vp, _vp, _vp] + [_i] * 6 + [_c.c_float, _vp, _vp, _vp]),
    "ebfi_conv2d_packed_x3": (_i, [_vp, _vp, _sz, _vp, _vp] + [_i] * 8 + [_i, _c.c_float, _vp, _vp, _i, _c.c_float, _vp]),
    "ebfi_conv2d_backward_weight_x3g": (_i, [_vp] * 4 + [_i] * 8 + [_vp, _sz, _vp]),
    "ebfi_scale_residual_cat_forward_ex": (_i, [_vp] * 6 + [_i, _i, _i64, _i64, _vp]),
    "ebfi_scale_residual_cat_backward_ex": (_i, [_vp] * 10 + [_i, _i, _i64, _i64, _i64, _i, _c.c_float, _vp]),
    "ebfi_scalar_conv_forward": (_i, [_vp, _vp, _vp, _vp, _i, _i, _i, _i, _c.c_float, _vp]),
    "ebfi_scalar_conv_backward": (_i, [_vp, _vp, _vp, _vp, _vp, _vp, _vp, _i, _i, _i, _i, _c.c_float, _vp]),
    "ebfi_events_workspace": (_sz, [_i]),
    "ebfi_events_to_stack": (_i, [_vp, _vp, _vp, _vp, _i64, _i, _i, _i, _vp, _vp, _sz, _vp]),
    "ebfi_frame2lap": (_i, [_vp, _vp, _i, _i, _i, _vp]),
    "ebfi_frame2dcp": (_i, [_vp, _vp, _vp, _i, _i, _i, _i, _vp]),
    "ebfi_scale_residual_cat_forward": (_i, [_vp] * 6 + [_i, _i, _i64, _vp]),
    "ebfi_scale_residual_cat_backward": (_i, [_vp] * 10 + [_i, _i, _i64, _vp]),
    "ebfi_prodmean_forward": (_i, [_vp, _vp, _vp, _i64, _i64, _vp]),
    "ebfi_prodmean_backward": (_i, [_vp] * 5 + [_i64, _i64, _vp]),
    "ebfi_gather_sum": (_i, [_vp, _vp, _vp, _i64, _i, _vp]),
    "ebfi_se_gate_workspace": (_c.c_size_t, [_i, _i, _i64]),
    "ebfi_se_gate_forward": (_i, [_vp] * 8 + [_i, _i, _i64, _i, _c.c_float, _vp]),
    "ebfi_se_gate_backward": (_i, [_vp] * 11 + [_i, _i, _i64, _i, _c.c_float, _vp]),
    "ebfi_conv2d_packed_x3_shuffled": (_i, [_vp, _vp, _c.c_size_t, _vp, _vp] + [_i] * 6 + [_c.c_float, _i, _vp]),
    "ebfi_conv2d_packed_f16_shuffled": (_i, [_vp, _i, _vp, _c.c_size_t, _vp, _vp] + [_i] * 6 + [_c.c_float, _vp, _i, _c.c_float, _vp, _vp, _i, _vp]),
    "ebfi_se_gate_forward_ps": (_i, [_vp] * 7 + [_i, _i, _i, _i, _i, _c.c_float, _vp]),
    "ebfi_se_gate_backward_ps": (_i, [_vp] * 10 + [_i, _i, _i, _i, _i, _c.c_float, _vp]),
    "ebfi_groupnorm_workspace": (_sz, [_i, _i]),
    "ebfi_groupnorm_forward": (_i, [_vp] * 6 + [_i, _i, _i64, _i, _c.c_float, _vp, _sz, _vp]),
    "ebfi_groupnorm_backward": (_i, [_vp] * 8 + [_i, _i, _i64, _i, _vp, _sz, _vp]),
    "ebfi_census_partials": (_i64, [_i, _i, _i]),
    "ebfi_census_forward": (_i, [_vp, _vp, _vp, _i, _i, _i, _i, _vp]),
    "ebfi_census_backward": (_i, [_vp, _vp, _vp, _vp, _i, _i, _i, _i, _vp]),
    "ebfi_gauss5_forward": (_i, [_vp, _vp, _i64, _i, _i, _c.c_float, _vp]),
    "ebfi_gauss5_backward": (_i, [_vp, _vp, _i64, _i, _i, _c.c_float, _vp]),
    "ebfi_ed_head_workspace": (_sz, [_i, _i, _i64]),
    "ebfi_ed_head_forward": (_i, [_vp] * 7 + [_i, _i, _i64, _i, _c.c_float, _vp, _sz, _vp]),
    "ebfi_ed_head_backward": (_i, [_vp] * 11 + [_i, _i, _i64, _i, _vp, _sz, _vp]),
    "ebfi_conv2d_backward_data_s2_bf16x3": (_i, [_vp, _vp, _vp, _i, _i, _i, _i, _i, _i, _i, _vp]),
    "ebfi_adam_step": (_i, [_vp, _vp, _vp, _vp, _vp, _i64] + [_c.c_double] * 4 + [_vp]),
    "ebfi_adam_step_guarded": (_i, [_vp, _vp, _vp, _vp, _vp, _i64] + [_c.c_double] * 4 + [_vp, _vp, _vp]),
    "ebfi_pad2d_backward": (_i, [_vp, _vp, _i64, _i, _i, _i, _i, _vp]),
    "ebfi_grad_gather": (_i, [_vp, _vp, _i, _vp, _i64, _i, _vp, _vp]),
    "ebfi_laploss_workspace_floats": (_i64, [_i64, _i, _i, _i]),
    "ebfi_laploss_partials": (_i64, [_i64, _i, _i, _i]),
    "ebfi_laploss_forward": (_i, [_vp, _vp, _vp, _c.c_float, _c.c_float, _vp, _vp, _i64, _i, _i, _i, _vp]),
    "ebfi_laploss_backward": (_i, [_vp, _vp, _vp, _i64, _i, _i, _i, _vp]),
    "ebfi_image_metrics_workspace": (_i64, [_i64, _i, _i, _i]),
    "ebfi_image_metrics": (_i, [_vp, _p64, _vp, _p64, _i64, _i, _i, _i, _c.c_float, _vp, _i64, _vp, _vp, _vp, _vp]),
    "ebfi_lpips_params_bytes": (_i64, []),
    "ebfi_lpips_pack_params": (_i, [_vp, _vp, _vp, _vp, _i64, _vp]),
    "ebfi_lpips_workspace": (_i64, [_i64, _i, _i, _i]),
    "ebfi_lpips_alex": (_i, [_vp, _p64, _vp, _p64, _i64, _i, _i, _i, _i, _vp, _vp, _i64, _vp, _vp, _vp]),
    "ebfi_charbonnier_workspace": (_i64, [_i64, _i, _i, _i]),
    "ebfi_charbonnier_forward": (_i, [_vp, _p64, _vp, _p64, _i64, _i, _i, _i, _c.c_float, _vp, _i64, _vp, _vp]),
    "ebfi_charbonnier_backward": (_i, [_vp, _p64, _vp, _p64, _i64, _i, _i, _i, _c.c_float, _vp, _vp, _vp]),
    "ebfi_duty_head_workspace": (_i64, [_i64, _i, _i]),
    "ebfi_duty_head_forward": (_i, [_vp, _p64, _vp, _i64, _i, _i, _c.c_float, _vp, _i64, _vp, _vp, _vp]),
    "ebfi_duty_head_backward": (_i, [_vp, _vp, _vp, _i64, _i, _i, _c.c_float, _vp, _vp]),
    "ebfi_frames_u8_to_planar": (_i, [_vp, _p64, _i64, _i, _i, _i, _i, _i, _i, _i, _i, _i, _vp, _vp]),
    "ebfi_planar_to_u8": (_i, [_vp, _p64, _i64, _i, _i, _vp, _vp]),
    "ebfi_period_frames_u8": (_i, [_vp, _p64, _i64, _i64, _i, _i, _i, _i, _i, _i, _i, _i, _i, _vp, _vp, _vp]),
    "ebfi_event_cnt_image_workspace": (_i64, [_i64, _i, _i, _i]),
    "ebfi_event_cnt_image": (_i, [_vp, _p64, _i64, _i, _i, _i, _i, _i, _i, _vp, _vp, _i64, _vp]),
    "ebfi_prof_enable": (None, [_i]),
    "ebfi_prof_set_capacity": (_i, [_i]),
    "ebfi_prof_reset": (None, []),
    "ebfi_prof_collect": (_i, [_c.POINTER(_i)]),
    "ebfi_prof_num_kernels": (_i, []),
    "ebfi_prof_get": (_i, [_i, _c.POINTER(_c.c_char_p), _c.POINTER(_i64), _c.POINTER(_c.c_double)]),
    "ebfi_prof_get_work": (_i, [_i, _c.POINTER(_c.c_double), _c.POINTER(_c.c_double)]),
}


def declared_symbols():
    text = open(HEADER).read()
    text = re.sub(r"/\*.*?\*/", "", text, flags=re.S)
    return sorted(set(re.findall(r"\b(ebfi_[a-z0-9_]+)\s*\(", text)))


def build(verbose=False):
    out = None if verbose else subprocess.DEVNULL
    subprocess.check_call(["bash", BUILD_SCRIPT], stdout=out)
    return LIB_PATH


def _counted(fn, name, n):
    def call(*a):
        if len(a) != n:
            raise TypeError("%s takes %d arguments (include/ebfi_hip.h), %d given" % (name, n, len(a)))
        return fn(*a)
    call.__name__ = name
    return call


def lib():
    global _lib
    if _lib is not None:
        return _lib
    with _lock:
        if _lib is not None:
            return _lib
        if not os.path.exists(LIB_PATH):
            raise EbfiNativeError(
                "native library %s is missing: run `python -c 'import __graft_entry__ as g; g.build()'` "
                "(or ebfi-be_amd/csrc/build.sh).  There is no CPU fallback." % LIB_PATH)
        try:
            h = ctypes.CDLL(LIB_PATH)
        except OSError as e:
            raise EbfiNativeError("cannot load %s: %s" % (LIB_PATH, e)) from e
        for name, (res, args) in SIGNATURES.items():
            try:
                fn = getattr(h, name)
            except AttributeError as e:
                raise EbfiNativeError("%s does not export %s" % (LIB_PATH, name)) from e
            fn.restype = res
            fn.argtypes = args
            setattr(h, name, _counted(fn, name, len(args)))
        if h.ebfi_abi_version() != ABI_VERSION:
            raise EbfiNativeError("ABI version mismatch: library %d, binding %d" % (h.ebfi_abi_version(), ABI_VERSION))
        _lib = h
    return _lib


def check(rc, what):
    if rc != 0:
        msg = lib().ebfi_last_error()
        raise EbfiNativeError("%s failed (%d): %s" % (what, rc, msg.decode() if msg else "?"))


def i64x4(vals):
    return (_c.c_int64 * 4)(*[int(v) for v in vals])


def ptr(t):
    return _vp(t.data_ptr()) if t is not None else _vp(0)


def stream_ptr(device=None):
    import torch
    return _vp(torch.cuda.current_stream(device).cuda_stream)


def dtype_code(t):
    import torch
    if t.dtype == torch.float32:
        return EBFI_F32
    raise EbfiNativeError("unsupported dtype %s (the ops take float32 tensors, like the reference's)" % t.dtype)


def require_gpu(*tensors):
    for t in tensors:
        if t is not None and not t.is_cuda:
            raise NotImplementedError(
                "ebfi_amd ops run on an MI355X through libebfi_hip.so only; got a %s tensor "
                "(the reference's FAC has no CPU path either: KernelConv2D.py:38-39)" % t.device)


def prof_enable(on=True):
    lib().ebfi_prof_enable(1 if on else 0)


def prof_reset():
    lib().ebfi_prof_reset()


def prof_fold():
    dropped = _i(0)
    lib().ebfi_prof_collect(ctypes.byref(dropped))
    return dropped.value


def prof_collect(strict=True):
    h = lib()
    dropped = _i(0)
    h.ebfi_prof_collect(ctypes.byref(dropped))
    if strict and dropped.value:
        raise EbfiNativeError("profiler dropped %d launches (pending capacity exceeded): fold once per step with "
                              "prof_fold() or raise ebfi_prof_set_capacity" % dropped.value)
    out = {}
    for k in range(h.ebfi_prof_num_kernels()):
        name, n, ms = _c.c_char_p(), _i64(0), _c.c_double(0)
        fl, by = _c.c_double(0), _c.c_double(0)
        h.ebfi_prof_get(k, ctypes.byref(name), ctypes.byref(n), ctypes.byref(ms))
        h.ebfi_prof_get_work(k, ctypes.byref(fl), ctypes.byref(by))
        out[name.value.decode()] = (n.value, ms.value, fl.value, by.value)
# ... 3 lines not shown
```

ebfi-be_amd/ebfi_amd/engine.py:

```python
import contextlib

import torch

from .dp import FlatAdam, FlatGradBucket, broadcast_parameters
from .loss import TrainLoss
from .model import EVFIAutoEx

DEFAULT_MODEL_ARGS = dict(
    FrameBasech=64, EventBasech=64, InterCH=64, TB=16, norm=None, activation="LeakyReLU",
    UseGTEx=False, FixEx=None, BlurryFashion="RGBLap", BLInch=4, UseEvents=True, LoadPretrainEX=False,
    PretrainedEXPath=None, FrozenEX=False, step=12, DualPath=True, residual=True, DetailEnabled=True,
    channels=[16, 24, 32, 64])


def synthetic_batch(B, H, W, TB=16, device="cuda", seed=123, rank=0, on_device=False):
    dev = torch.device(device)
    if on_device and dev.type == "cuda":
        g = torch.Generator(device=dev).manual_seed(seed + rank)
        rnd = lambda *shape: torch.rand(*shape, generator=g, device=dev)
        frame = rnd(B, 3, H, W)
        event = torch.poisson(torch.full((B, TB, 2, H, W), 0.35, device=dev), generator=g)
        t = rnd(B, 1)
        gtex = rnd(B, 1) * 0.4 + 0.55
        return frame, event, t, gtex, rnd(B, 3, H, W)
    g = torch.Generator(device="cpu").manual_seed(seed + rank)
    frame = torch.rand(B, 3, H, W, generator=g)
    event = torch.poisson(torch.full((B, TB, 2, H, W), 0.35), generator=g)
    t = torch.rand(B, 1, generator=g)
    gtex = torch.rand(B, 1, generator=g) * 0.4 + 0.55
    target = torch.rand(B, 3, H, W, generator=g)
    return tuple(v.to(device) for v in (frame, event, t, gtex, target))


def synthetic_batch_from_raw_events(B, H, W, TB=16, device="cuda", seed=123, rank=0, rate=0.35, on_device=False):
    from .encodings import events_to_stack
    dev = torch.device(device)
    on_device = on_device and dev.type == "cuda"
    frame, _, t, gtex, target = synthetic_batch(B, H, W, 0 if on_device else TB, device=device, seed=seed, rank=rank,
                                                on_device=on_device)
    gdev = dev if on_device else torch.device("cpu")
    g = torch.Generator(device=gdev).manual_seed(seed + rank + 7919)
    n = int(rate * H * W * TB)
    stacks = []
    for _ in range(B):
        xs = torch.randint(0, W, (n,), generator=g, device=gdev).to(device)
        ys = torch.randint(0, H, (n,), generator=g, device=gdev).to(device)
        ts = torch.sort(torch.rand(n, generator=g, dtype=torch.float64, device=gdev))[0].to(device)
        ps = (torch.randint(0, 2, (n,), generator=g, device=gdev) * 2 - 1).float().to(device)
        stacks.append(events_to_stack(xs, ys, ts, ps, TB, sensor_size=(H, W)).transpose(0, 1))
    return frame, torch.stack(stacks).contiguous(), t, gtex, target


def synthetic_validation_batch(B, H, W, TB=16, num_frames=4, device="cuda", seed=0):
    g = torch.Generator(device="cpu").manual_seed(int(seed))
    frame = torch.rand(B, 3, H, W, generator=g)
    event = torch.poisson(torch.full((B, TB, 2, H, W), 0.35), generator=g)
    gtex = torch.rand(B, 1, generator=g) * 0.4 + 0.55
    latent = torch.rand(B, num_frames, 3, H, W, generator=g)
    ts = (torch.arange(num_frames) / num_frames).expand(B, num_frames).contiguous()
    return tuple(v.to(device) for v in (frame, event, ts, gtex, latent))


class Engine:
    def __init__(self, model_args=None, device="cuda", precision="fp32", lr=1e-4, seed=None, train=True, graph=False,
                 accu_step=1, betas=(0.9, 0.999), backward_f16=None, forward_f16="filters", strict_graph=None):
        if precision not in ("fp32", "bf16x3", "bf16"):
            raise ValueError("precision must be 'fp32', 'bf16x3' or 'bf16'")
        self.device = torch.device(device)
        self.precision = precision
        if seed is not None:
            torch.manual_seed(seed)
        self.model_args = dict(DEFAULT_MODEL_ARGS, **(model_args or {}))
        self.model = EVFIAutoEx(**self.model_args).to(self.device)
        broadcast_parameters(self.model, 0)
        self.iteration = 0
        self.accu_step = max(1, int(accu_step))
        self._micro = 0
        self.calibration_steps = 2
        self._steps_run = 0
        self._accum = None
        self.use_graph = bool(graph) and self.device.type == "cuda"
        self._graphs = {}
        self.graph_capture_failed, self.graph_capture_error = False, None
        if strict_graph is None:
            from .dp import is_distributed
            strict_graph = is_distributed()
        self.strict_graph = bool(strict_graph)
        if train:
            self.model.train()
            self.loss = TrainLoss(self.model_args.get("DetailEnabled", True)).to(self.device)
            self.bucket = FlatGradBucket(self.model)
            self.optimizer = FlatAdam(self.bucket.params, lr=lr, betas=tuple(betas))
        else:
            self.model.eval()
        self.bank = None
        if backward_f16 is None:
            backward_f16 = True
        use_book = train and precision == "bf16x3" and backward_f16
        forward_f16 = forward_f16 if use_book else None
        if forward_f16 == "none":
            forward_f16 = None
        from .f16scale import FORWARD_LEVELS
        if forward_f16 not in FORWARD_LEVELS:
            raise ValueError("forward_f16 must be one of %r" % (FORWARD_LEVELS,))
        if self.device.type == "cuda":
            from . import weightbank
            self.bank = weightbank.build_for(self.model, flat=self.optimizer.flat.data, params=self.optimizer.params,
                                             fwd16=forward_f16) if train else weightbank.build_for(self.model, inference=True)
        self.book = None
        if use_book and self.bank is not None:
            from . import f16scale
            self.book = f16scale.ScaleBook(self.device)
            self.bank.attach_scale_book(self.book)
            self.book.forward_f16 = forward_f16

    @property
    def settled(self):
        if self.book is not None and self.precision == "bf16x3" and self._steps_run < self.calibration_steps:
            return False
        return not self.use_graph or bool(self._graphs)

    @contextlib.contextmanager
    def _autocast(self):
        from . import conv
        prev = conv.get_compute_dtype()
        conv.set_compute_dtype(self.precision)
        try:
            yield
        finally:
            conv.set_compute_dtype(prev)

    def _bank(self):
        if self.bank is None or self.precision != "bf16x3":
            return contextlib.nullcontext()
        self.bank.refresh()
        return self.bank.active()

    def _book(self):
        if self.book is None or self.precision != "bf16x3":
            return contextlib.nullcontext()
        return self.book.active()

    def _fwd_bwd(self, frame, event, t, gtex, target):
        with self._autocast(), self._bank(), self._book() as book:
            if book is not None and self._steps_run < self.calibration_steps:
                book.calibrated.clear()
            sharp_pre, sharp = self.model(frame, event, t, gtex)
            loss = self.loss(sharp_pre.float(), sharp.float(), target, self.iteration, self.accu_step)
            loss.backward()
            if book is not None:
                book.finish()
        return loss.detach()

    def _begin_micro_step(self):
        if self.book is not None and self.precision == "bf16x3" and self._micro == 0:
            self.book.begin_step()

    def _guard(self):
        return self.book.guard if (self.book is not None and self.precision == "bf16x3") else None

    def _finish_micro_step(self, wire):
        if self.accu_step > 1:
            if self._micro == 0:
                self._accum = wire.clone() if self._accum is None else self._accum.copy_(wire)
            else:
                self._accum.add_(wire)
            self._micro += 1
            if self._micro < self.accu_step:
                return False
            self._micro = 0
            wire = self._accum
        self.bucket.adopt(wire)
        self.bucket.reduce_mean_packed()
        guard = self._guard()
        self.optimizer.step(self.bucket.flat, guard=guard, flag=self.bucket.flag if guard is not None else None)
        self.iteration += 1
        self._steps_run += 1
        return True

    def train_step(self, frame, event, t, gtex, target):
        calibrating = self.book is not None and self.precision == "bf16x3" and self._steps_run < self.calibration_steps
        if self.use_graph and not calibrating:
            return self.train_step_graph(frame, event, t, gtex, target)
        self._begin_micro_step()
        self.bucket.zero()
        loss = self._fwd_bwd(frame, event, t, gtex, target)
        self.bucket.gather(self._guard())
        self._finish_micro_step(self.bucket.wire)
        return loss

    def train_step_graph(self, frame, event, t, gtex, target):
        inputs = (frame, event, t, gtex, target)
        phase = self.iteration < 10e3
        key = (self.precision, phase, self.accu_step) + tuple((tuple(v.shape), v.dtype) for v in inputs)
        entry = self._graphs.get(key)
        if entry is None:
            static_in = [torch.empty_like(v) for v in inputs]
            for s, v in zip(static_in, inputs):
                s.copy_(v)
            guard = self._guard()
            saved = None if guard is None else guard.clone()
            side = torch.cuda.Stream(self.device)
            side.wait_stream(torch.cuda.current_stream(self.device))
            with torch.cuda.stream(side):
                for _ in range(2):
                    self.bucket.zero()
                    self._fwd_bwd(*static_in)
            torch.cuda.current_stream(self.device).wait_stream(side)
            self.bucket.zero()
            graph = torch.cuda.CUDAGraph()
            try:
                with torch.cuda.graph(graph, capture_error_mode="thread_local"):
                    loss = self._fwd_bwd(*static_in)
                    self.bucket.gather(guard)
                    wire = self.bucket.wire
            except RuntimeError as err:
                if saved is not None:
                    torch.cuda.synchronize(self.device)
                    guard.copy_(saved)
                if self.strict_graph:
                    raise RuntimeError("ebfi_amd.engine: hipGraph capture failed and strict_graph is set (the default for one "
                                       "rank of several): %s" % str(err).splitlines()[0]) from err
                import sys
                print("ebfi_amd.engine: hipGraph capture failed (%s); continuing with eager launches" % str(err).splitlines()[0],
                      file=sys.stderr, flush=True)
                self.use_graph = False
                self.graph_capture_failed, self.graph_capture_error = True, str(err).splitlines()[0]
                torch.cuda.synchronize(self.device)
                return self.train_step(frame, event, t, gtex, target)
            if saved is not None:
                guard.copy_(saved)
            entry = (graph, static_in, loss, wire, [p.grad for p in self.bucket.params])
            self._graphs[key] = entry
        graph, static_in, loss, wire, grads = entry
        self._begin_micro_step()
        for s, v in zip(static_in, inputs):
            if s.data_ptr() != v.data_ptr():
                s.copy_(v)
        graph.replay()
        self.bucket.adopt(wire)
        for p, g in zip(self.bucket.params, grads):
            p.grad = g
        self._finish_micro_step(wire)
        return loss.clone()

    @torch.no_grad()
    def infer(self, frame, event, t, gtex=None):
        with self._autocast(), self._bank():
            return self.model(frame, event, t, gtex)[-1]

    VALID_KEYS = ("valid_loss", "valid_psnr", "valid_ssim")

    def validator(self, group=None):
        cache = self.__dict__.setdefault("_validators", {})
        if group not in cache:
            cache[group] = ClipInterpolator(self.model, precision=self.precision, graph=self.device.type == "cuda", hoist=True,
                                            group=group)
        return cache[group]

    @torch.no_grad()
    def validate(self, batch, load=0, group=None, refresh=True, eps=1e-3):
        from .loss import charbonnier_per_sample
        from .metrics import frame_metrics
        if isinstance(batch, dict):
            latent = batch["SeqLatentF"][:, load]
            latent = latent.reshape((latent.shape[0], -1) + tuple(latent.shape[-3:]))
            frame = batch["SeqBlurryF"][:, load, 0]
            event = batch["SeqHREv"][:, load]
            ts = batch["RelativeLatentTs"][:, load, 0]
            gtex = batch["SeqExposureDuty"][:, load, 0]
        else:
            frame, event, ts, gtex, latent = batch
        frame, event, gtex = frame.contiguous(), event.contiguous(), None if gtex is None else gtex.contiguous()
        B, num_i = int(ts.shape[0]), int(ts.shape[-1])
        if latent.dim() != 5 or latent.shape[0] != B or latent.shape[1] != num_i:
            raise ValueError("validate: LatentF %s does not match Ts %s" % (tuple(latent.shape), tuple(ts.shape)))
        interp = self.validator(group)
        if refresh:
            interp.refresh_weights()
            interp._captured.clear()
        final = interp(frame, event, gtex, [ts[:, i] for i in range(num_i)])
        pred = final.reshape((B * num_i,) + tuple(final.shape[2:])).float()
        target = latent.reshape((B * num_i,) + tuple(latent.shape[2:])).float()
        loss = charbonnier_per_sample(pred, target, eps).double().sum() / num_i
        psnr, ssim, _ = frame_metrics(pred, target)
        values = torch.stack([loss, psnr.double().mean(), ssim.double().mean()])
        return {k: values[i] for i, k in enumerate(self.VALID_KEYS)}


class ClipInterpolator:

    GROUP_PIXELS = 16 * 256 * 256

    def __init__(self, model, precision="bf16x3", graph=True, hoist=True, filters_f16=True, group=None):
        self.model = model
        self.precision, self.graph, self.hoist = precision, bool(graph), bool(hoist)
        self.group = None if group is None else max(1, int(group))
        self.graph_capture_failed, self.graph_capture_error = False, None
        self.bank = self.book = None
        if precision == "bf16x3" and next(model.parameters()).is_cuda:
            from . import f16scale, weightbank
            if filters_f16:
                self.book = f16scale.ScaleBook(next(model.parameters()).device, capacity=64)
            self.bank = weightbank.build_for(model, inference=True, book=self.book)
            self.bank.refresh()
        self._captured = {}

    @contextlib.contextmanager
    def _ctx(self):
        from . import conv
        prev = conv.get_compute_dtype()
        conv.set_compute_dtype(self.precision)
        modes = [(m, m.training) for m in self.model.modules()]
        self.model.eval()
        try:
            if self.bank is not None:
                self.bank.ensure_fresh()
            with (self.bank.active() if self.bank is not None else contextlib.nullcontext()):
                yield
        finally:
            conv.set_compute_dtype(prev)
            for m, flag in modes:
                m.training = flag

    def refresh_weights(self):
        if self.bank is not None:
            self.bank.refresh()

    def _step(self, state, frame, event, gtex, t):
        return self.model.decode(state, t)[-1] if self.hoist else self.model(frame, event, t, gtex)[-1]

    @torch.no_grad()
    def __call__(self, frame, event, gtex, timestamps, out=None, timing=False):
        timestamps = list(timestamps)
        if not timestamps:
            raise ValueError("ClipInterpolator: no timestamps")
        B, dev = frame.shape[0], frame.device
        ev = [torch.cuda.Event(enable_timing=True) for _ in range(3)] if (timing and dev.type == "cuda") else None
        with self._ctx():
            if ev:
                ev[0].record()
            state = self.model.encode(frame, event, gtex) if self.hoist else None
            if ev:
                ev[1].record()
            result = out
            n = len(timestamps)
            k = 1
            if self.hoist:
                k = self.group if self.group is not None else max(1, self.GROUP_PIXELS // max(1, B * frame.shape[-2] * frame.shape[-1]))
                k = max(1, min(k, n))
            self.last_group = k

            def put(i, value, count=1):
                nonlocal result
# ... 80 lines not shown
```

ebfi-be_amd/ebfi_amd/loss.py:

```python
import os

import torch
import torch.nn as nn
import torch.nn.functional as F

from . import _native as N


class _Gauss5(torch.autograd.Function):

    @staticmethod
    def forward(ctx, x, factor):
        x = x.contiguous()
        ctx.factor = float(factor)
        out = torch.empty_like(x)
        H, W = x.shape[-2:]
        with torch.cuda.device_of(x):
            rc = N.lib().ebfi_gauss5_forward(N.ptr(x), N.ptr(out), x.numel() // (H * W), H, W, ctx.factor,
                                             N.stream_ptr(x.device))
        N.check(rc, "ebfi_gauss5_forward")
        return out

    @staticmethod
    def backward(ctx, g):
        g = g.contiguous()
        gin = torch.empty_like(g)
        H, W = g.shape[-2:]
        with torch.cuda.device_of(g):
            rc = N.lib().ebfi_gauss5_backward(N.ptr(g), N.ptr(gin), g.numel() // (H * W), H, W, ctx.factor,
                                              N.stream_ptr(g.device))
        N.check(rc, "ebfi_gauss5_backward")
        return gin, None


class _Census(torch.autograd.Function):

    @staticmethod
    def forward(ctx, x, y):
        x, y = x.contiguous(), y.contiguous()
        B, C, H, W = x.shape
        lib = N.lib()
        partial = torch.empty(int(lib.ebfi_census_partials(B, H, W)), dtype=torch.float32, device=x.device)
        with torch.cuda.device_of(x):
            rc = lib.ebfi_census_forward(N.ptr(x), N.ptr(y), N.ptr(partial), B, C, H, W, N.stream_ptr(x.device))
        N.check(rc, "ebfi_census_forward")
        ctx.save_for_backward(x, y)
        return partial.sum() / float(B * H * W)

    @staticmethod
    def backward(ctx, g):
        x, y = ctx.saved_tensors
        B, C, H, W = x.shape
        g = g.contiguous().float().reshape(1)
        gx = torch.empty_like(x)
        with torch.cuda.device_of(x):
            rc = N.lib().ebfi_census_backward(N.ptr(x), N.ptr(y), N.ptr(g), N.ptr(gx), B, C, H, W, N.stream_ptr(x.device))
        N.check(rc, "ebfi_census_backward")
        return gx, None


class _LapLoss(torch.autograd.Function):

    LEVELS = 5

    @staticmethod
    def usable(a, b, target):
        H, W = a.shape[-2:]
        m = 1 << (_LapLoss.LEVELS - 1)
        ok = lambda t: t.is_cuda and t.dtype == torch.float32 and t.shape == a.shape
        return a.dim() == 4 and ok(a) and ok(target) and (b is None or ok(b)) and H % m == 0 and W % m == 0 and \
            2 * H // m >= 3 and 2 * W // m >= 3 and not target.requires_grad

    @staticmethod
    def forward(ctx, a, b, target, coef_a, coef_b):
        a, target = a.contiguous(), target.contiguous()
        b = b.contiguous() if b is not None else None
        B, C, H, W = a.shape
        ppt, L = B * C, _LapLoss.LEVELS
        planes = ppt * (2 if b is not None else 1)
        lib = N.lib()
        ws = torch.empty(int(lib.ebfi_laploss_workspace_floats(planes, H, W, L)), dtype=torch.float32, device=a.device)
        partial = torch.empty(int(lib.ebfi_laploss_partials(planes, H, W, L)), dtype=torch.float32, device=a.device)
        with torch.cuda.device_of(a):
            rc = lib.ebfi_laploss_forward(N.ptr(a), N.ptr(b) if b is not None else None, N.ptr(target), float(coef_a),
                                          float(coef_b), N.ptr(ws), N.ptr(partial), ppt, H, W, L, N.stream_ptr(a.device))
        N.check(rc, "ebfi_laploss_forward")
        ctx.ws, ctx.shape, ctx.two = ws, (B, C, H, W), b is not None
        return partial.sum()

    @staticmethod
    def backward(ctx, g):
        if ctx.ws is None:
            raise RuntimeError("laploss: the workspace of this forward was already consumed by a backward pass")
        B, C, H, W = ctx.shape
        n = 2 if ctx.two else 1
        g = g.contiguous().float().reshape(1)
        out = torch.empty((n * B, C, H, W), dtype=torch.float32, device=g.device)
        with torch.cuda.device_of(out):
            rc = N.lib().ebfi_laploss_backward(N.ptr(g), N.ptr(ctx.ws), N.ptr(out), n * B * C, H, W, _LapLoss.LEVELS,
                                               N.stream_ptr(out.device))
        N.check(rc, "ebfi_laploss_backward")
        ctx.ws = None
        return out[:B], (out[B:] if ctx.two else None), None, None, None


class GaussianConv(nn.Module):

    def __init__(self):
        super().__init__()
        k1 = torch.tensor([1., 4., 6., 4., 1.])
        self.kernel = nn.Parameter((k1[:, None] * k1[None, :] / 256).repeat(3, 1, 1, 1), requires_grad=False)
        self.taps = (1.0 / 16, 4.0 / 16, 6.0 / 16, 4.0 / 16, 1.0 / 16)

    def forward(self, x, factor=1):
        H, W = x.shape[-2:]
        if x.is_cuda and x.dtype == torch.float32 and H >= 3 and W >= 3:
            return _Gauss5.apply(x, factor)
        p = F.pad(x, (2, 2, 2, 2), mode="reflect")
        h = sum(t * p[..., :, j:j + W] for j, t in enumerate(self.taps))
        v = sum(t * h[..., i:i + H, :] for i, t in enumerate(self.taps))
        return v * factor if factor != 1 else v


class LaplacianPyramid(nn.Module):
    def __init__(self, max_level=5):
        super().__init__()
        self.gaussian_conv = GaussianConv()
        self.max_level = max_level

    def expand(self, x):
        B, C, H, W = x.shape
        up = x.new_zeros(B, C, 2 * H, 2 * W)
        up[:, :, ::2, ::2] = x
        return self.gaussian_conv(up, factor=4)

    def forward(self, X):
        pyramid, cur = [], X
        for _ in range(self.max_level - 1):
            reduced = F.avg_pool2d(self.gaussian_conv(cur), 2)
            pyramid.append(cur - self.expand(reduced))
            cur = reduced
        pyramid.append(cur)
        return pyramid


class LaplacianLoss(nn.Module):
    def __init__(self):
        super().__init__()
        self.lap = LaplacianPyramid()

    def forward(self, x, y, y_pyramid=None):
        yp = y_pyramid if y_pyramid is not None else self.lap(y)
        return sum((2 ** i) * F.l1_loss(a, b, reduction="sum") for i, (a, b) in enumerate(zip(self.lap(x), yp)))


class Ternary(nn.Module):
    def __init__(self, patch_size=7):
        super().__init__()
        self.patch_size = patch_size
        n = patch_size * patch_size
        self.register_buffer("w", torch.eye(n).view(n, 1, patch_size, patch_size), persistent=False)

    def transform(self, t):
        g = t.mean(dim=1, keepdim=True)
        H, W = g.shape[-2:]
        k, r = self.patch_size, self.patch_size // 2
        gp = F.pad(g, (r, r, r, r))
        patches = torch.cat([gp[..., i:i + H, j:j + W] for i in range(k) for j in range(k)], dim=1)
        d = patches - g
        return d / torch.sqrt(0.81 + d ** 2)

    def forward(self, x, y, y_transform=None):
        if x.is_cuda and x.dtype == torch.float32 and y.dtype == torch.float32 and self.patch_size == 7 and \
                not y.requires_grad and x.shape[-1] > 6 and x.shape[-2] > 6:
            return _Census.apply(x, y)
        ty = y_transform if y_transform is not None else self.transform(y).detach()
        diff = self.transform(x) - ty
        dist = (diff ** 2 / (0.1 + diff ** 2)).mean(dim=1, keepdim=True)
        p = self.patch_size // 2
        mask = torch.zeros_like(dist)
        mask[:, :, p:-p, p:-p] = 1
        return (dist * mask).mean()


class TrainLoss(nn.Module):

    def __init__(self, detail_enabled=True):
        super().__init__()
        self.Lap, self.census, self.detail_enabled = LaplacianLoss(), Ternary(), detail_enabled

    def forward(self, sharp_pre, sharp, target, iteration=0, accu_step=1):
        c_sharp, c_pre = (0.1, 1.0) if iteration < 10e3 else (1.0, 0.1)
        if not self.detail_enabled:
            c_sharp, c_pre, sharp_pre = 1.0, 0.0, None
        if _LapLoss.usable(sharp, sharp_pre, target):
            total = _LapLoss.apply(sharp, sharp_pre, target, c_sharp, c_pre) + c_sharp * self.census(sharp, target)
            if sharp_pre is not None:
                total = total + c_pre * self.census(sharp_pre, target)
            return total / accu_step
        with torch.no_grad():
            yp = self.Lap.lap(target)
            ty = None if target.is_cuda else self.census.transform(target)
        term = lambda p: self.Lap(p, target, yp) + self.census(p, target, ty)
        if sharp_pre is None:
            return term(sharp) / accu_step
        return (c_sharp * term(sharp) + c_pre * term(sharp_pre)) / accu_step


_cb_workspaces = {}


def _cb_workspace(device, stream, shape):
    key = (device, stream, shape)
    ws = _cb_workspaces.get(key)
    if ws is None:
        nbytes = N.lib().ebfi_charbonnier_workspace(*shape)
        ws = torch.empty(max(nbytes // 8, 2), dtype=torch.float64, device=device)
        _cb_workspaces[key] = ws
    return ws


def _cb_check(x, y, eps):
    N.require_gpu(x, y)
    if x.dim() != 4 or x.shape != y.shape:
        raise ValueError("Charbonnier loss takes two [N, C, H, W] tensors of one shape, got %s and %s"
                         % (tuple(x.shape), tuple(y.shape)))
    if x.dtype != torch.float32 or y.dtype != torch.float32:
        raise ValueError("Charbonnier loss takes float32 tensors, got %s / %s" % (x.dtype, y.dtype))
    if x.device != y.device:
        raise ValueError("x on %s, y on %s" % (x.device, y.device))
    if not eps > 0:
        raise ValueError("eps must be positive, got %r" % (eps,))
    x = x if x.stride(3) == 1 or x.shape[3] == 1 else x.contiguous()
    y = y if y.stride(3) == 1 or y.shape[3] == 1 else y.contiguous()
    return x, y


def _cb_strides(t):
    return N.i64x4(tuple(t.stride())[:3] + (1,))


def _cb_forward(x, y, eps):
    n, c, h, w = (int(v) for v in x.shape)
    out = torch.empty(n, dtype=torch.float32, device=x.device)
    if n == 0 or c * h * w == 0:
        return out.zero_()
    with torch.cuda.device_of(x):
        stream = N.stream_ptr(x.device)
        ws = _cb_workspace(x.device, stream.value, (n, c, h, w))
        rc = N.lib().ebfi_charbonnier_forward(N.ptr(x), _cb_strides(x), N.ptr(y), _cb_strides(y), n, c, h, w, float(eps),
                                              N.ptr(ws), ws.numel() * 8, N.ptr(out), stream)
    N.check(rc, "ebfi_charbonnier_forward")
    return out


@torch.no_grad()
def charbonnier_per_sample(x, y, eps=1e-3):
    x, y = _cb_check(x, y, eps)
    return _cb_forward(x, y, eps)


class _Charbonnier(torch.autograd.Function):

    @staticmethod
    def forward(ctx, x, y, eps):
        ctx.eps = float(eps)
        ctx.save_for_backward(x, y)
        return _cb_forward(x, y, eps).sum()

    @staticmethod
    def backward(ctx, g):
        x, y = ctx.saved_tensors
        n, c, h, w = (int(v) for v in x.shape)
        g = g.contiguous().float().reshape(1)
        gx = torch.empty((n, c, h, w), dtype=torch.float32, device=x.device)
        if gx.numel():
            with torch.cuda.device_of(x):
                rc = N.lib().ebfi_charbonnier_backward(N.ptr(x), _cb_strides(x), N.ptr(y), _cb_strides(y), n, c, h, w, ctx.eps,
                                                       N.ptr(g), N.ptr(gx), N.stream_ptr(x.device))
            N.check(rc, "ebfi_charbonnier_backward")
        return (gx if ctx.needs_input_grad[0] else None), (-gx if ctx.needs_input_grad[1] else None), None


class CharbonnierLoss(nn.Module):

    def __init__(self, eps=1e-3):
        super().__init__()
        self.eps = eps

    def forward(self, x, y):
        x, y = _cb_check(x, y, self.eps)
        return _Charbonnier.apply(x, y, self.eps)


_dh_workspaces = {}


def _dh_workspace(device, stream, shape):
    key = (device, stream, shape)
    ws = _dh_workspaces.get(key)
    if ws is None:
        nbytes = N.lib().ebfi_duty_head_workspace(*shape)
        ws = torch.empty(max(nbytes // 8, 2), dtype=torch.float64, device=device)
        _dh_workspaces[key] = ws
    return ws


def _dh_check(ex, duty):
    N.require_gpu(ex, duty)
    if ex.dim() != 4 or ex.shape[1] != 1:
        raise ValueError("the duty head takes a [B, 1, H, W] map, got %s" % (tuple(ex.shape),))
    if ex.dtype != torch.float32:
        raise ValueError("the duty head takes a float32 map, got %s" % ex.dtype)
    if ex.shape[0] == 0 or ex.shape[2] * ex.shape[3] == 0:
        raise ValueError("the duty head needs a non-empty map, got %s" % (tuple(ex.shape),))
    if duty is not None:
        if duty.numel() != ex.shape[0] or duty.dtype != torch.float32 or duty.device != ex.device:
            raise ValueError("duty must be a float32 [B, 1] tensor on the map's device, got %s %s on %s for B = %d"
                             % (duty.dtype, tuple(duty.shape), duty.device, ex.shape[0]))
        duty = duty.detach().reshape(-1).contiguous()
    return (ex if ex.stride(3) == 1 or ex.shape[3] == 1 else ex.contiguous()), duty


def _dh_forward(ex, duty, scale):
    b, _, h, w = (int(v) for v in ex.shape)
    Ex = torch.empty((b, 1), dtype=torch.float32, device=ex.device)
    loss = torch.empty((), dtype=torch.float32, device=ex.device) if duty is not None else None
    with torch.cuda.device_of(ex):
        stream = N.stream_ptr(ex.device)
        ws = _dh_workspace(ex.device, stream.value, (b, h, w))
        rc = N.lib().ebfi_duty_head_forward(N.ptr(ex), N.i64x4(tuple(ex.stride())[:3] + (1,)), N.ptr(duty), b, h, w, float(scale),
                                            N.ptr(ws), ws.numel() * 8, N.ptr(Ex), N.ptr(loss), stream)
    N.check(rc, "ebfi_duty_head_forward")
    return Ex, loss


@torch.no_grad()
def duty_head(ex):
    ex, _ = _dh_check(ex, None)
    return _dh_forward(ex, None, 1.0)[0]


class _DutyMSE(torch.autograd.Function):

    @staticmethod
    def forward(ctx, ex, duty, scale):
        Ex, loss = _dh_forward(ex, duty, scale)
        ctx.scale, ctx.shape = float(scale), tuple(int(v) for v in ex.shape)
        ctx.save_for_backward(Ex, duty)
        ctx.mark_non_differentiable(Ex)
        return loss, Ex
# ... 28 lines not shown
```

ebfi-be_amd/ebfi_amd/weightbank.py:

```python
import contextlib

import numpy as np
import torch

from . import _native as N

_ACTIVE = None
LO_FLAG = 1 << 30


def active_bank():
    return _ACTIVE


def lookup(param, kind="id"):
    if _ACTIVE is None or param is None:
        return None
    return _ACTIVE.sites.get((param.data_ptr(), kind))


class Site:
    __slots__ = ("bank", "kind", "M", "K", "ks", "groups", "fwd_off", "tr_off", "fwd_bytes", "tr_bytes", "bias_off", "has_bias",
                 "w_inv", "w_R", "b_inv", "b_R", "w_shapes", "b_shapes", "key", "tr16_off", "tr16_bytes", "w_slot", "weights",
                 "fwd16_off", "fwd16_bytes", "fwd16_tag")

    def fwd_ptr(self):
        return N._vp(self.bank.packed.data_ptr() + self.fwd_off)

    def tr_ptr(self):
        return N._vp(self.bank.packed.data_ptr() + self.tr_off)

    def tr16_ptr(self):
        if self.bank.packed16 is None or self.tr16_bytes == 0:
            return None
        return N._vp(self.bank.packed16.data_ptr() + 2 * self.tr16_off)

    def fwd16_ptr(self):
        if self.bank.packed16 is None or self.fwd16_bytes == 0:
            return None
        return N._vp(self.bank.packed16.data_ptr() + 2 * self.fwd16_off)

    def w_slot_ptr(self):
        return self.bank.book.ptr(self.w_slot)

    def bias(self):
        return self.bank.bias_buf[self.bias_off:self.bias_off + self.M] if self.has_bias else None


def _ids_like(p, flat_off):
    return (torch.arange(p.numel(), dtype=torch.float64) + (flat_off + 1)).view(p.shape)


def _adjoint_table(src_ids, n_src, first):
    fwd = src_ids.reshape(-1).astype(np.int64)
    dest = np.nonzero(fwd >= 0)[0]
    order = np.argsort(fwd[dest], kind="stable")
    srcs, dest = fwd[dest][order] - first, dest[order]
    counts = np.bincount(srcs, minlength=n_src)
    R = int(max(1, counts.max()))
    starts = np.concatenate([[0], np.cumsum(counts)[:-1]])
    inv = np.full((n_src, R), -1, dtype=np.int32)
    inv[srcs, np.arange(len(srcs)) - starts[srcs]] = dest
    return inv, R


class WeightBank:
    def __init__(self, params, flat=None, inference=False, fwd16=None):
        self.inference = bool(inference)
        self.fwd16 = fwd16
        self.params = list(params)
        self.owns_flat = flat is None
        self._offsets, off = {}, 0
        for p in self.params:
            self._offsets[p.data_ptr()] = (off, p)
            off += p.numel()
        self.numel = off
        self.device = self.params[0].device
        self.flat = torch.cat([p.detach().reshape(-1).float() for p in self.params]) if flat is None else flat
        if self.flat.numel() != self.numel:
            raise ValueError("flat buffer has %d elements, parameters %d" % (self.flat.numel(), self.numel))
        if self.numel >= LO_FLAG:
            raise ValueError("more than 2^30 parameters")
        self.sites = {}
        self._tables, self._n_packed = [], 0
        self._bias_tables, self._n_bias = [], 0
        self.packed = self.table = self.bias_buf = self.bias_table = None
        self._stamp = None
        self.book = None
        self._tables16, self._n16, self._segs = [], 0, []
        self.packed16 = self.table16 = self.block_slot = None

    def _offset(self, p):
        ent = self._offsets.get(p.data_ptr())
        if ent is None or ent[1].shape != p.shape:
            raise KeyError("parameter is not part of this bank")
        return ent[0]

    def register(self, weights, biases=None, kind="id", fold_w=None, fold_b=None, groups=1, need_tr=True, fwd16=False):
        weights = list(weights) if isinstance(weights, (list, tuple)) else [weights]
        biases = list(biases) if isinstance(biases, (list, tuple)) else ([biases] if biases is not None else [])
        if any(b is None for b in biases):
            if not all(b is None for b in biases):
                raise ValueError("a concatenated site needs a bias on every part or on none")
            biases = []
        key = (weights[0].data_ptr(), kind)
        if key in self.sites:
            return self.sites[key]
        ident = lambda t: t
        fw, fb = fold_w or ident, fold_b or ident
        ids = torch.cat([fw(_ids_like(w, self._offset(w))) for w in weights], dim=0).round().to(torch.int64) - 1
        M, K, ks, ks2 = ids.shape
        if ks != ks2 or ks not in (1, 3):
            raise ValueError("weight bank holds 1x1 / 3x3 kernels, got %dx%d" % (ks, ks2))
        KK, K16, M16 = ks * ks, (K + 15) // 16 * 16, (M + 15) // 16 * 16
        pad = lambda t, n: torch.cat([t, t.new_full(t.shape[:-1] + (n - t.shape[-1],), -1)], dim=-1)
        fwd = pad(ids.permute(2, 3, 0, 1).reshape(KK, M, K), K16).reshape(-1)
        if M % groups != 0:
            raise ValueError("%d output channels do not split into %d groups" % (M, groups))
        Mg = M // groups
        tr = pad(ids.flip((2, 3)).view(groups, Mg, K, ks, ks).permute(3, 4, 0, 2, 1).reshape(KK, groups * K, Mg),
                 (Mg + 15) // 16 * 16).reshape(-1)
        s = Site()
        s.bank, s.kind, s.M, s.K, s.ks, s.groups = self, kind, int(M), int(K), int(ks), int(groups)
        s.key, s.weights = key, weights
        s.fwd16_tag = fwd16 if isinstance(fwd16, str) else None
        s.tr_off, s.tr_bytes, s.tr16_off, s.tr16_bytes, s.w_slot, s.fwd16_off, s.fwd16_bytes = 0, 0, 0, 0, -1, 0, 0
        images16 = []
        if ks == 3 and need_tr and not self.inference:
            images16.append(("tr16", tr))
        if ks == 3 and (fwd16 or (self.fwd16 == "all" and need_tr)):
            images16.append(("fwd16", fwd))
        if images16:
            for name, img in images16:
                setattr(s, name + "_off", self._n16)
                setattr(s, name + "_bytes", 2 * img.numel())
                padn = (-img.numel()) % 256
                self._tables16.append(torch.cat([img.to(torch.int32), torch.full((padn,), -1, dtype=torch.int32)]))
                self._segs.append((self._n16, s))
                self._n16 += img.numel() + padn
        for name, img in (("fwd", fwd), ("tr", tr)) if need_tr else (("fwd", fwd),):
            lo = torch.where(img >= 0, img | LO_FLAG, img)
            setattr(s, name + "_off", 2 * self._n_packed)
            setattr(s, name + "_bytes", 4 * img.numel())
            self._tables += [img.to(torch.int32), lo.to(torch.int32)]
            self._n_packed += 2 * img.numel()
        idn = ids.numpy()
        s.w_inv, s.w_R, s.w_shapes = [], [], [tuple(w.shape) for w in weights]
        for w in weights:
            o = self._offset(w)
            inv, R = _adjoint_table(np.where((idn >= o) & (idn < o + w.numel()), idn, -1), w.numel(), o)
            s.w_inv.append(torch.from_numpy(inv).to(self.device))
            s.w_R.append(R)
        s.has_bias = len(biases) > 0
        s.bias_off, s.b_inv, s.b_R, s.b_shapes = self._n_bias, [], [], [tuple(b.shape) for b in biases]
        if s.has_bias:
            bids = torch.cat([fb(_ids_like(b, self._offset(b))) for b in biases], dim=0).round().to(torch.int64) - 1
            if bids.numel() != M:
                raise ValueError("folded bias has %d entries for %d output channels" % (bids.numel(), M))
            self._bias_tables.append(bids.to(torch.int32))
            self._n_bias += int(M)
            bn = bids.numpy()
            for b in biases:
                o = self._offset(b)
                inv, R = _adjoint_table(np.where((bn >= o) & (bn < o + b.numel()), bn, -1), b.numel(), o)
                s.b_inv.append(torch.from_numpy(inv).to(self.device))
                s.b_R.append(R)
        self.sites[key] = s
        self.packed = None
        return s

    def _finalize(self):
        self.table = torch.cat(self._tables).to(self.device) if self._tables else None
        self.packed = torch.empty(max(self._n_packed, 8), dtype=torch.bfloat16, device=self.device)
        self.bias_table = torch.cat(self._bias_tables).to(self.device) if self._bias_tables else None
        self.bias_buf = torch.empty(max(self._n_bias, 1), dtype=torch.float32, device=self.device)
        if self.book is not None and self._tables16:
            self.table16 = torch.cat(self._tables16).to(self.device)
            self.packed16 = torch.empty(self._n16, dtype=torch.float16, device=self.device)
            counts = []
            for (off, site), nxt in zip(self._segs, [o for o, _ in self._segs[1:]] + [self._n16]):
                site.w_slot = self.book.slot((site.key, "w"))
                counts.append((nxt - off) // 256)
            self.block_slot = torch.repeat_interleave(torch.tensor([site.w_slot for _, site in self._segs], dtype=torch.int32),
                                                      torch.tensor(counts)).to(self.device)

    def attach_scale_book(self, book):
        self.book = book
        self.packed = None

    def _current_stamp(self):
        if self.owns_flat:
            return sum(p._version for p in self.params)
        return self.flat._version

    def refresh(self):
        if self.packed is None:
            self._finalize()
        if self.owns_flat:
            torch.cat([p.detach().reshape(-1) for p in self.params], out=self.flat)
        lib = N.lib()
        with torch.cuda.device(self.device):
            st = N.stream_ptr(self.device)
            if self.table is not None:
                N.check(lib.ebfi_pack_table_bf16(N.ptr(self.flat), N.ptr(self.table), self.table.numel(), N.ptr(self.packed), st),
                        "ebfi_pack_table_bf16")
            if self.bias_table is not None:
                N.check(lib.ebfi_gather_sum(N.ptr(self.flat), N.ptr(self.bias_table), N.ptr(self.bias_buf), self._n_bias, 1, st),
                        "ebfi_gather_sum")
            if self.packed16 is not None:
                for _, site in self._segs:
                    if self.inference:
                        self.book.calibrated.discard(site.w_slot)
                    self.book.calibrate(site.w_slot, *site.weights)
                N.check(lib.ebfi_pack_table_f16(N.ptr(self.flat), N.ptr(self.table16), self.table16.numel(), N.ptr(self.packed16),
                                                N.ptr(self.block_slot), N.ptr(self.book.slots), st), "ebfi_pack_table_f16")
        self._stamp = self._current_stamp()

    def ensure_fresh(self):
        if self.packed is None or self._stamp != self._current_stamp():
            self.refresh()

    @contextlib.contextmanager
    def active(self):
        global _ACTIVE
        prev, _ACTIVE = _ACTIVE, self
        try:
            yield self
        finally:
            _ACTIVE = prev


def build_for(model, flat=None, params=None, inference=False, fwd16=None, book=None):
    import torch.nn as nn

    from . import fold3d
    params = list(params) if params is not None else [p for p in model.parameters()]
    bank = WeightBank(params, flat, inference=inference, fwd16=fwd16)
    if book is not None:
        bank.attach_scale_book(book)
    known = set(p.data_ptr() for p in params)
    ok = lambda *ts: all(t is None or t.data_ptr() in known for t in ts)
    for m in model.modules():
        if isinstance(m, nn.Conv2d) and ok(m.weight, m.bias):
            k = m.kernel_size
            if k[0] == k[1] and k[0] in (1, 3) and m.stride == (1, 1) and m.dilation == (1, 1) and m.groups == 1:
                tag = getattr(m, "_ebfi_fwd16", None)
                from .f16scale import FORWARD_LEVELS
                want = tag is not None and fwd16 is not None and FORWARD_LEVELS.index(tag) <= FORWARD_LEVELS.index(fwd16)
                bank.register(m.weight, m.bias, "id", fwd16=tag if want else False)
        elif isinstance(m, nn.Conv3d) and ok(m.weight, m.bias):
            kd, kh, kw = m.kernel_size
            if kd in (1, 3) and kh == kw and kh in (1, 3) and (kh == 1 or m.stride[1] == 1) and m.stride[0] == 1 and \
                    m.padding[0] == kd // 2 and m.dilation == (1, 1, 1) and m.groups == 1:
                bank.register(m.weight, m.bias, "conv3d", fold3d.fold_conv3d_weight, fold3d._rep2)
        elif isinstance(m, nn.ConvTranspose3d) and ok(m.weight, m.bias):
            if m.kernel_size == (3, 4, 4) and m.stride == (1, 2, 2) and m.padding == (1, 1, 1) and m.groups == 1:
                bank.register(m.weight, m.bias, "convT3d", fold3d.fold_conv_transpose3d_weight, fold3d._rep8)
    for m in model.modules():
        hook = getattr(m, "_ebfi_bank_register", None)
        if hook is not None:
            hook(bank)
    return bank
```

include/ebfi_hip.h:

```cpp
#ifndef EBFI_HIP_H
#define EBFI_HIP_H

#include <stddef.h>
#include <stdint.h>

#ifdef __cplusplus
extern "C" {
#endif

#define EBFI_ABI_VERSION 14

typedef enum {
    EBFI_OK = 0,
    EBFI_ERR_ARG = -1,
    EBFI_ERR_LAUNCH = -2,
    EBFI_ERR_UNSUPPORTED = -3,
    EBFI_ERR_WORKSPACE = -4
} ebfi_status;

typedef enum { EBFI_F32 = 0, EBFI_F32_BF16MMA = 2, EBFI_F32_BF16X3MMA = 3 } ebfi_dtype;

int ebfi_abi_version(void);
const char *ebfi_last_error(void);

int ebfi_fac_forward(const void *input, const int64_t input_shape[4], const int64_t input_stride[4],
                     const void *kernel, const int64_t kernel_shape[4], const int64_t kernel_stride[4],
                     int kernel_size,
                     void *output, const int64_t output_shape[4], const int64_t output_stride[4],
                     int dtype, void *stream);

int ebfi_fac_backward(const void *input, const int64_t input_shape[4], const int64_t input_stride[4],
                      const void *kernel, const int64_t kernel_shape[4], const int64_t kernel_stride[4],
                      int kernel_size,
                      const void *grad_output, const int64_t grad_output_stride[4],
                      void *grad_input, const int64_t grad_input_stride[4],
                      void *grad_kernel, const int64_t grad_kernel_stride[4],
                      int dtype, void *stream);

int ebfi_fac_backward_ex(const void *input, const int64_t input_shape[4], const int64_t input_stride[4],
                         const void *kernel, const int64_t kernel_shape[4], const int64_t kernel_stride[4],
                         int kernel_size,
                         const void *grad_output, const int64_t grad_output_stride[4],
                         void *grad_input, const int64_t grad_input_stride[4],
                         void *grad_kernel, const int64_t grad_kernel_stride[4],
                         float kernel_leaky_slope, int dtype, void *stream);

int ebfi_dcn_forward(const void *input, const void *weight, const void *bias, const void *offset,
                     const void *mask, void *output,
                     int B, int C, int H, int W, int Co, int kh, int kw, int sh, int sw,
                     int ph, int pw, int dh, int dw, int deformable_group,
                     int dtype, void *stream);

size_t ebfi_dcn_backward_workspace(int B, int C, int H, int W, int Co, int kh, int kw, int sh, int sw,
                                   int ph, int pw, int dh, int dw, int deformable_group, int dtype);

int ebfi_dcn_backward(const void *input, const void *weight, const void *bias, const void *offset,
                      const void *mask, const void *grad_output,
                      void *grad_input, void *grad_offset, void *grad_mask, void *grad_weight,
                      void *grad_bias,
                      int B, int C, int H, int W, int Co, int kh, int kw, int sh, int sw,
                      int ph, int pw, int dh, int dw, int deformable_group,
                      void *workspace, size_t workspace_bytes, int dtype, void *stream);

int ebfi_conv2d_forward(const void *input, const void *weight, const void *bias, void *output,
                        int B, int Cin, int H, int W, int Cout, int ksize, int stride, int pad,
                        int act, float slope, int dtype, void *stream);

int ebfi_conv2d_backward_data(const void *grad_output, const void *saved_output, const void *weight,
                              void *grad_input, int B, int Cin, int H, int W, int Cout, int ksize,
                              int stride, int pad, int act, float slope, int dtype, void *stream);

size_t ebfi_conv2d_backward_weight_workspace(int B, int Cin, int H, int W, int Cout, int ksize,
                                             int stride, int pad, int dtype);

int ebfi_conv2d_backward_weight(const void *input, const void *grad_output, const void *saved_output,
                                void *grad_weight, void *grad_bias,
                                int B, int Cin, int H, int W, int Cout, int ksize, int stride, int pad,
                                int act, float slope, void *workspace, size_t workspace_bytes,
                                int dtype, void *stream);

int ebfi_conv2d_backward_weight_ex(const void *input, const void *grad_output, const void *saved_output,
                                   void *grad_weight, void *grad_bias, void *grad_preact_out,
                                   int B, int Cin, int H, int W, int Cout, int ksize, int stride, int pad,
                                   int act, float slope, void *workspace, size_t workspace_bytes,
                                   int dtype, void *stream);

size_t ebfi_conv2d_bf16_workspace(int Cin, int Cout, int ksize);
int ebfi_conv2d_forward_bf16mma(const void *input, const void *weight, const void *bias, void *output,
                                int B, int Cin, int H, int W, int Cout, int ksize, int stride, int pad,
                                int act, float slope, void *workspace, size_t workspace_bytes, void *stream);
int ebfi_conv2d_backward_data_bf16mma(const void *grad_output, const void *saved_output, const void *weight,
                                      void *grad_input, int B, int Cin, int H, int W, int Cout, int ksize,
                                      int stride, int pad, int act, float slope,
                                      void *workspace, size_t workspace_bytes, void *stream);

int ebfi_conv2d_forward_bf16x3(const void *input, const void *weight, const void *bias, void *output,
                               int B, int Cin, int H, int W, int Cout, int ksize, int stride, int pad,
                               int act, float slope, void *workspace, size_t workspace_bytes, void *stream);
int ebfi_conv2d_backward_data_bf16x3(const void *grad_output, const void *saved_output, const void *weight,
                                     void *grad_input, int B, int Cin, int H, int W, int Cout, int ksize,
                                     int stride, int pad, int act, float slope,
                                     void *workspace, size_t workspace_bytes, void *stream);

int ebfi_conv2d_backward_data_s2_bf16x3(const void *grad_preact, const void *weight, void *grad_input, int B, int Cin,
                                        int H, int W, int Cout, int ksize, int pad, void *stream);

size_t ebfi_conv2d_packed_bytes(int Cin, int Cout, int ksize, int transposed);
int ebfi_conv2d_pack_bf16x3(const void *weight, int Cin, int Cout, int ksize, int transposed, void *packed,
                            size_t packed_bytes, void *stream);
int ebfi_pack_table_bf16(const float *src, const int32_t *table, int64_t n, void *out, void *stream);

int ebfi_conv2d_thin_forward(const void *input, const void *weight, const void *bias, void *output, int B, int Cin, int H, int W,
                             int Cout, int ksize, int stride, int pad, int act, float slope, void *stream);

int ebfi_conv2d_packed_x3(const void *input, const void *packed, size_t packed_bytes, const void *bias, void *output,
                          int B, int Cin_per_group, int H, int W, int Cout, int ksize, int pad, int groups, int act,
                          float slope, const void *addend, const void *mask_y, int mask_act, float mask_slope, void *stream);
int ebfi_kernelconv_fac_fused_x3(const void *input, const void *packed, size_t packed_bytes, const void *bias32,
                                 const void *feat, void *output, int B, int Cin, int H, int W, int C, int fac_ksize,
                                 float slope, void *stream);

int ebfi_kernelconv_fac_fused_f16(const void *input, int input_is_c16, const void *packed16, size_t packed_bytes,
                                  const void *bias32, const void *feat, void *output, int B, int Cin, int H, int W, int C,
                                  int fac_ksize, float slope, void *in_slot, const void *w_slot, void *stream);
int ebfi_f16_scales_finish(void *slots, int n, void *flag, void *stream);
int ebfi_pack_table_f16(const float *src, const int32_t *table, int64_t n, void *out, const int32_t *block_slot,
                        void *slots, void *stream);
int ebfi_conv2d_packed_f16(const void *input, const void *packed16, size_t packed_bytes, const void *bias, void *output,
                           int B, int Cin_per_group, int H, int W, int Cout, int ksize, int pad, int groups, int act,
                           float slope, const void *addend, const void *mask_y, int mask_act, float mask_slope,
                           void *in_slot, const void *w_slot, void *stream);
int ebfi_conv2d_backward_weight_f16g(const void *input, const void *grad_output, const void *saved_output,
                                     void *grad_weight, void *grad_bias, void *grad_preact_out, int B,
                                     int Cin_per_group, int H, int W, int Cout, int ksize, int pad, int groups, int act,
                                     float slope, void *x_slot, void *g_slot, void *workspace,
                                     size_t workspace_bytes, void *stream);
int ebfi_conv2d_backward_weight_f16g_ex(const void *input, const void *grad_output, const void *saved_output,
                                        void *grad_weight, void *grad_bias, void *grad_preact_out, int grad_preact_is_c16, int B,
                                        int Cin_per_group, int H, int W, int Cout, int ksize, int pad, int groups, int act,
                                        float slope, void *x_slot, void *g_slot, void *workspace,
                                        size_t workspace_bytes, void *stream);
int ebfi_to_c16(const float *src, const float *mask_y, float mask_slope, void *dst16, void *slot, int B, int C, int H, int W,
                void *stream);
int ebfi_to_c16_cat2(const float *src0, int C0, const float *src1, int C1, void *dst16, void *slot, int B, int H, int W, void *stream);
int ebfi_conv2d_packed_x3_c16(const void *input, const void *packed, size_t packed_bytes, const void *bias, void *output,
                              int B, int Cin_per_group, int H, int W, int Cout, int ksize, int pad, int groups, int act,
                              float slope, const void *addend, const void *mask_y, int mask_act, float mask_slope,
                              void *out16, void *slot16, int out16_planar, void *stream);
int ebfi_conv2d_packed_f16_c16(const void *input, int input_is_c16, const void *packed16, size_t packed_bytes,
                               const void *bias, void *output, int B, int Cin_per_group, int H, int W, int Cout, int ksize,
                               int pad, int groups, int act, float slope, const void *addend, const void *mask_y,
                               int mask_act, float mask_slope, void *in_slot, const void *w_slot, void *out16,
                               void *slot16, int out16_planar, int mask_is_c16, void *stream);
int ebfi_conv2d_packed_x3_shuffled(const void *input, const void *packed, size_t packed_bytes, const void *bias, void *output,
                                   int B, int Cin, int H, int W, int Cout, int act, float slope, int out_layout, void *stream);
int ebfi_conv2d_packed_f16_shuffled(const void *input, int input_is_c16, const void *packed16, size_t packed_bytes,
                                    const void *bias, void *output, int B, int Cin, int H, int W, int Cout, int act, float slope,
                                    const void *mask_y, int mask_act, float mask_slope, void *in_slot, const void *w_slot,
                                    int out_layout, void *stream);
int ebfi_conv2d_backward_weight_f16c(const void *input16, const void *grad16, int grad_is_planar, void *grad_weight,
                                     void *grad_bias, int B, int Cin_per_group, int H, int W, int Cout, int groups,
                                     const void *x_slot, const void *g_slot, void *workspace, size_t workspace_bytes,
                                     void *stream);
size_t ebfi_conv2d_backward_weight_f16c_batch_workspace(int n, const int *Cin_per_group, const int *Cout);
int ebfi_conv2d_backward_weight_f16c_batch(int n, const void *const *input16, const void *const *grad16, void *const *grad_weight,
                                           void *const *grad_bias, const int *Cin_per_group, const int *Cout, const int *groups,
                                           void *const *x_slot, void *const *g_slot, int B, int H, int W, void *workspace,
                                           size_t workspace_bytes, void *stream);
int ebfi_fac_forward_p16(const float *input, int input_is_unpadded, const void *filters16, const void *f_slot, float *output, int B,
                         int C, int Ho, int Wo, int K, void *stream);
int ebfi_fac_backward_p16(const float *input, int input_is_unpadded, const void *filters16, const void *f_slot,
                          const float *grad_output, float *grad_input, void *grad_kernel16, void *g_slot, float kernel_leaky_slope,
                          int B, int C, int Ho, int Wo, int K, void *stream);
int ebfi_scale_residual_cat_forward_c16(const float *a0, const float *s0, const float *a1, const float *s1, const float *x,
                                        float *out, void *out16, void *slot, int B, int C, int H, int W,
                                        int64_t a_batch_stride, void *stream);
int ebfi_scale_residual_cat_backward_slices(void);
int ebfi_scale_residual_cat_backward_c16(const float *grad_out, const float *a0, const float *s0, const float *a1,
                                         const float *s1, void *grad_a16, void *slot, float *grad_x, float *grad_s0_part,
                                         float *grad_s1_part, int B, int C, int H, int W, int64_t a_batch_stride,
                                         float mask_slope, void *stream);
int ebfi_scale_residual_cat_backward_c16a(const float *grad_out, const void *a16, const void *a_slot, const float *s0, const float *s1,
                                          void *grad_a16, void *slot, float *grad_x, float *grad_s0_part, float *grad_s1_part, int B,
                                          int C, int H, int W, float mask_slope, void *stream);
int ebfi_conv2d_packed_x3_rc(const void *input, const void *packed, size_t packed_bytes, const void *bias, void *output, int B,
                             int Cin_per_group, int H, int W, int Cout, int groups, float slope, const void *post_scale,
                             const void *post_res, int res_channels, void *pre16, void *pre_slot, void *out16, void *slot16,
                             void *stream);
int ebfi_conv2d_backward_weight_x3g(const void *input, const void *grad_output, void *grad_weight, void *grad_bias,
                                    int B, int Cin_per_group, int H, int W, int Cout, int ksize, int pad, int groups,
                                    void *workspace, size_t workspace_bytes, void *stream);

size_t ebfi_events_workspace(int bins);
int ebfi_events_to_stack(const double *xs, const double *ys, const double *ts, const float *ps,
                         int64_t n, int bins, int H, int W, float *out,
                         void *workspace, size_t workspace_bytes, void *stream);

int ebfi_frame2lap(const float *frame, float *out, int B, int H, int W, void *stream);
int ebfi_frame2dcp(const float *frame, float *out, float *scratch , int B, int H, int W,
                   int window, void *stream);

int ebfi_scalar_conv_forward(const float *v, const void *const *weights, const void *const *biases, float *out, int S, int B,
                             int K, int C, float slope, void *stream);
int ebfi_scalar_conv_backward(const float *v, const void *const *weights, const float *out, const float *grad_out,
                              float *grad_weight, float *grad_bias, float *grad_v, int S, int B, int K, int C, float slope,
                              void *stream);

int ebfi_scale_residual_cat_forward(const float *a0, const float *s0, const float *a1, const float *s1, const float *x,
                                    float *out, int B, int C, int64_t HW, void *stream);
int ebfi_scale_residual_cat_backward(const float *grad_out, const float *a0, const float *s0, const float *a1,
                                     const float *s1, float *grad_a0, float *grad_a1, float *grad_x,
                                     float *grad_s0, float *grad_s1, int B, int C, int64_t HW, void *stream);

int ebfi_scale_residual_cat_forward_ex(const float *a0, const float *s0, const float *a1, const float *s1, const float *x,
                                       float *out, int B, int C, int64_t HW, int64_t a_batch_stride, void *stream);
int ebfi_scale_residual_cat_backward_ex(const float *grad_out, const float *a0, const float *s0, const float *a1,
                                        const float *s1, float *grad_a0, float *grad_a1, float *grad_x, float *grad_s0,
                                        float *grad_s1, int B, int C, int64_t HW, int64_t a_batch_stride,
                                        int64_t grad_a_batch_stride, int mask_leaky, float mask_slope, void *stream);

int ebfi_prodmean_forward(const float *a, const float *b, float *out, int64_t planes, int64_t HW, void *stream);
int ebfi_prodmean_backward(const float *a, const float *b, const float *grad_out, float *grad_a, float *grad_b,
                           int64_t planes, int64_t HW, void *stream);

int ebfi_gather_sum(const float *src, const int32_t *idx, float *out, int64_t n_out, int R, void *stream);

size_t ebfi_se_gate_workspace(int B, int C, int64_t N);
int ebfi_se_gate_forward(const float *x, const float *weight, const float *bias, const float *res, float *out, float *mean,
                         float *gate, float *workspace, int B, int C, int64_t N, int act, float slope, void *stream);
int ebfi_se_gate_backward(const float *grad_out, const float *out, const float *x, const float *weight, const float *gate,
                          const float *mean, float *grad_x, float *grad_res, float *grad_weight, float *grad_bias,
                          float *workspace, int B, int C, int64_t N, int act, float slope, void *stream);

int ebfi_se_gate_forward_ps(const float *x, const float *weight, const float *bias, float *out, float *mean, float *gate,
                            float *workspace, int B, int C, int h, int w, int act, float slope, void *stream);
int ebfi_se_gate_backward_ps(const float *grad_out, const float *out, const float *x, const float *weight, const float *gate,
                             const float *mean, float *grad_x, float *grad_weight, float *grad_bias, float *workspace, int B, int C,
                             int h, int w, int act, float slope, void *stream);

size_t ebfi_groupnorm_workspace(int B, int C);
int ebfi_groupnorm_forward(const float *x, const float *gamma, const float *beta, float *y, float *mean, float *rstd,
                           int B, int C, int64_t HW, int groups, float eps,
                           void *workspace, size_t workspace_bytes, void *stream);
int ebfi_groupnorm_backward(const float *grad_y, const float *x, const float *gamma, const float *mean,
                            const float *rstd, float *grad_x, float *grad_gamma, float *grad_beta,
                            int B, int C, int64_t HW, int groups,
                            void *workspace, size_t workspace_bytes, void *stream);

size_t ebfi_ed_head_workspace(int B, int C, int64_t HW);
int ebfi_ed_head_forward(const float *ev, const float *bl, const float *gamma, const float *beta, float *out, float *atten,
                         double *stats, int B, int C, int64_t HW, int groups, float eps,
                         void *workspace, size_t workspace_bytes, void *stream);
int ebfi_ed_head_backward(const float *grad_out, const float *ev, const float *bl, const float *gamma, const float *beta,
                          const float *atten, const double *stats, float *grad_ev, float *grad_bl, float *grad_gamma,
                          float *grad_beta, int B, int C, int64_t HW, int groups,
                          void *workspace, size_t workspace_bytes, void *stream);

int ebfi_gauss5_forward(const float *input, float *output, int64_t planes, int H, int W, float factor, void *stream);
int ebfi_gauss5_backward(const float *grad_output, float *grad_input, int64_t planes, int H, int W, float factor,
                         void *stream);

int64_t ebfi_census_partials(int B, int H, int W);
int ebfi_census_forward(const float *x, const float *y, float *partial, int B, int C, int H, int W, void *stream);
int ebfi_census_backward(const float *x, const float *y, const float *grad_loss, float *grad_x,
                         int B, int C, int H, int W, void *stream);

int64_t ebfi_laploss_workspace_floats(int64_t planes, int H, int W, int levels);
int64_t ebfi_laploss_partials(int64_t planes, int H, int W, int levels);
int ebfi_laploss_forward(const float *pred_a, const float *pred_b, const float *target, float coef_a, float coef_b,
                         float *workspace, float *partial, int64_t planes_per_term, int H, int W, int levels, void *stream);
int ebfi_laploss_backward(const float *grad_loss, float *workspace, float *grad_pred, int64_t planes, int H, int W,
                          int levels, void *stream);

int ebfi_pad2d_backward(const float *grad_padded, float *grad_input, int64_t planes, int H, int W, int pad, int replicate, void *stream);

int ebfi_adam_step(float *param, const float *grad, float *exp_avg, float *exp_avg_sq, const float *step, int64_t n,
                   double lr, double beta1, double beta2, double eps, void *stream);
int ebfi_adam_step_guarded(float *param, const float *grad, float *exp_avg, float *exp_avg_sq, float *step, int64_t n,
                           double lr, double beta1, double beta2, double eps, int *guard, const float *flag, void *stream);

int ebfi_grad_gather(const void *const *grads, const int64_t *numels, int count, float *flat, int64_t total, int pad,
                     const int *guard, void *stream);


int64_t ebfi_image_metrics_workspace(int64_t N, int C, int H, int W);
int ebfi_image_metrics(const float *pred, const int64_t pred_strides[4], const float *target, const int64_t target_strides[4],
                       int64_t N, int C, int H, int W, float ssim_data_range, void *workspace, int64_t workspace_bytes,
                       float *out_psnr, float *out_ssim, float *out_mse, void *stream);

int64_t ebfi_lpips_params_bytes(void);
int ebfi_lpips_pack_params(const float *const *conv_w, const float *const *conv_b, const float *const *lin_w, void *params,
                           int64_t params_bytes, void *stream);
int64_t ebfi_lpips_workspace(int64_t N, int C, int H, int W);
int ebfi_lpips_alex(const float *pred, const int64_t pred_strides[4], const float *target, const int64_t target_strides[4],
                    int64_t N, int C, int H, int W, int normalize, const void *params, void *workspace, int64_t workspace_bytes,
                    float *out_lpips, float *out_layers, void *stream);

int64_t ebfi_charbonnier_workspace(int64_t N, int C, int H, int W);
int ebfi_charbonnier_forward(const float *x, const int64_t x_strides[4], const float *y, const int64_t y_strides[4], int64_t N,
                             int C, int H, int W, float eps, void *workspace, int64_t workspace_bytes, float *out, void *stream);
int ebfi_charbonnier_backward(const float *x, const int64_t x_strides[4], const float *y, const int64_t y_strides[4], int64_t N,
                              int C, int H, int W, float eps, const float *g, float *grad_x, void *stream);

int64_t ebfi_duty_head_workspace(int64_t B, int H, int W);
int ebfi_duty_head_forward(const float *ex, const int64_t ex_strides[4], const float *duty, int64_t B, int H, int W, float scale,
                           void *workspace, int64_t workspace_bytes, float *Ex_out, float *loss_out, void *stream);
int ebfi_duty_head_backward(const float *g, const float *Ex, const float *duty, int64_t B, int H, int W, float scale,
                            float *grad_ex, void *stream);

int ebfi_frames_u8_to_planar(const uint8_t *src, const int64_t src_strides[3], int64_t n, int H0, int W0, int i, int j, int h,
                             int w, int reverse_channels, int flip_h, int flip_v, float *out, void *stream);
int ebfi_planar_to_u8(const float *in, const int64_t in_strides[3], int64_t n, int H, int W, uint8_t *out, void *stream);

int ebfi_period_frames_u8(const uint8_t *src, const int64_t src_strides[3], int64_t n, int64_t n_blur, int H0, int W0, int i,
                          int j, int h, int w, int reverse_channels, int flip_h, int flip_v, float *sharp, float *blur,
                          void *stream);

enum { EBFI_EVENT_BLUE_RED = 0, EBFI_EVENT_GREEN_RED = 1, EBFI_EVENT_GRAY = 2 };
int64_t ebfi_event_cnt_image_workspace(int64_t n, int H, int W, int is_norm);
int ebfi_event_cnt_image(const float *ev, const int64_t ev_strides[3], int64_t n, int H, int W, int color_scheme,
                         int is_black_background, int is_norm, int use_opencv, uint8_t *out, void *workspace,
                         int64_t workspace_bytes, void *stream);

#define EBFI_PROF_MAX_PENDING 65536
void ebfi_prof_enable(int on);
int ebfi_prof_set_capacity(int max_pending);
void ebfi_prof_reset(void);
int ebfi_prof_collect(int *dropped);
int ebfi_prof_num_kernels(void);
int ebfi_prof_get(int index, const char **name, int64_t *launches, double *total_ms);
int ebfi_prof_get_work(int index, double *flops, double *bytes);

#ifdef __cplusplus
}
#endif
#endif
```

Baseline: 555.6 frames/s.

## Pack bf16 weight pairs by block, fuse census pair loss, parallelize scalar-conv bwd

Weight packing now runs block-wise: each thread handles two entries and writes the hi and lo bf16 halves, using a per-block descriptor and an active-block list. This halves table reads and allows packing only the weight images that are actually requested. A new census pair kernel computes the census loss for two predictions against one target in a single pass, sharing the target's tile staging and transform. The scalar-conv backward moves from a single 256-thread block to a multi-block grid of one wave per output. Together these cut launch count and serial work, in exchange for more bookkeeping and capture-time restrictions around on-demand packing.

```diff
diff --git a/ebfi-be_amd/csrc/conv2d.hip b/ebfi-be_amd/csrc/conv2d.hip
--- a/ebfi-be_amd/csrc/conv2d.hip
+++ b/ebfi-be_amd/csrc/conv2d.hip
@@ -1950,6 +1950,28 @@
     if (t >= 0) v = src[t & 0x3fffffff];
     const __bf16 h = (__bf16)v;
     out[e] = (t >= 0 && (t & 0x40000000)) ? (__bf16)(v - (float)h) : h;
+}
+
+constexpr int PACK_PAIR_BLOCK = 512;
+__global__ __launch_bounds__(256) void pack_pairs_bf16_kernel(const float *__restrict__ src, const int32_t *__restrict__ table,
+                                                              const int4 *__restrict__ desc, const int32_t *__restrict__ active,
+                                                              __bf16 *__restrict__ out) {
+    const int blk = active[blockIdx.x];
+    const int4 d = desc[blk];
+    const int e = 2 * threadIdx.x;
+    if (e >= d.w) return;
+    const int64_t hi_at = (int64_t)(((uint64_t)(uint32_t)d.y << 32) | (uint32_t)d.x) + e;
+    const int2 t = *reinterpret_cast<const int2 *>(table + (int64_t)blk * PACK_PAIR_BLOCK + e);
+    const float v0 = t.x >= 0 ? src[t.x] : 0.f, v1 = t.y >= 0 ? src[t.y] : 0.f;
+    typedef __bf16 bf16x2 __attribute__((ext_vector_type(2)));
+    const __bf16 h0 = (__bf16)v0, h1 = (__bf16)v1;
+    bf16x2 hi, lo;
+    hi[0] = h0;
+    hi[1] = h1;
+    lo[0] = (__bf16)(v0 - (float)h0);
+    lo[1] = (__bf16)(v1 - (float)h1);
+    *reinterpret_cast<bf16x2 *>(out + hi_at) = hi;
+    *reinterpret_cast<bf16x2 *>(out + hi_at + d.z) = lo;
 }
 
 __device__ __forceinline__ void wgrad_reduce_body(const float *__restrict__ slab, int nslabs, int64_t n_weight, int64_t n_total,
@@ -3004,6 +3026,21 @@
     hipLaunchKernelGGL(pack_table_bf16_kernel, dim3((unsigned)ceil_div(n, 256)), dim3(256), 0, st, src, table, n,
                        static_cast<__bf16 *>(out));
     return check_launch("pack_table_bf16");
+}
+
+extern "C" int ebfi_pack_pairs_block(void) { return PACK_PAIR_BLOCK; }
+
+extern "C" int ebfi_pack_pairs_bf16(const float *src, const int32_t *table, const void *desc, const int32_t *active, int64_t n_active,
+                                    int64_t n_entries, void *out, void *stream) {
+    if (!src || !table || !desc || !active || !out || n_active < 0 || n_active > 2147483647LL || n_entries < 0 ||
+        n_entries > n_active * PACK_PAIR_BLOCK)
+        return fail(EBFI_ERR_ARG, "pack_pairs_bf16: bad argument");
+    if (n_active == 0) return EBFI_OK;
+    hipStream_t st = static_cast<hipStream_t>(stream);
+    ProfScope ps("pack_table_bf16", st, 0.0, 12.0 * (double)n_entries + 20.0 * (double)n_active);
+    hipLaunchKernelGGL(pack_pairs_bf16_kernel, dim3((unsigned)n_active), dim3(256), 0, st, src, table, static_cast<const int4 *>(desc),
+                       active, static_cast<__bf16 *>(out));
+    return check_launch("pack_pairs_bf16");
 }
 
 extern "C" size_t ebfi_conv2d_packed_bytes(int Cin, int Cout, int ksize, int transposed) {
diff --git a/ebfi-be_amd/csrc/fuse.hip b/ebfi-be_amd/csrc/fuse.hip
--- a/ebfi-be_amd/csrc/fuse.hip
+++ b/ebfi-be_amd/csrc/fuse.hip
@@ -336,10 +336,13 @@
     }
 }
 
-__global__ __launch_bounds__(256) void scalar_conv_bwd_kernel(ScalarBank bank, const float *__restrict__ v, const float *__restrict__ out,
-                                                              const float *__restrict__ gout, float *__restrict__ gw, float *__restrict__ gb,
-                                                              float *__restrict__ gv, int S, int B, int K, int C, float slope) {
-    for (int i = threadIdx.x; i < S * C; i += 256) {
+__global__ __launch_bounds__(64) void scalar_conv_bwd_kernel(ScalarBank bank, const float *__restrict__ v, const float *__restrict__ out,
+                                                             const float *__restrict__ gout, float *__restrict__ gw, float *__restrict__ gb,
+                                                             float *__restrict__ gv, int n_wb, int S, int B, int K, int C, float slope) {
+    const int lane = threadIdx.x;
+    if ((int)blockIdx.x < n_wb) {
+        const int i = blockIdx.x * 64 + lane;
+        if (i >= S * C) return;
         const int s = i / C, c = i - s * C;
         float aw[SC_MAX_K], ab = 0.f;
 #pragma unroll
@@ -358,27 +361,25 @@
             for (int k = 0; k < SC_MAX_K; ++k)
                 if (k < K) gw[(int64_t)i * K + k] = aw[k];
         }
-    }
-    if (gv) {
-        const int wave = threadIdx.x >> 6, lane = threadIdx.x & 63;
-        for (int p = wave; p < B * K; p += 4) {
-            const int b = p / K, k = p - b * K;
-            float acc = 0.f;
-            for (int s = 0; s < S; ++s) {
-                const float *w = nullptr;
-#pragma unroll
-                for (int j = 0; j < SC_MAX_LAYERS; ++j)
-                    if (j == s) w = bank.w[j];
-                for (int c = lane; c < C; c += 64) {
-                    const int64_t o = ((int64_t)s * B + b) * C + c;
-                    acc = fmaf(gout[o] * (out[o] > 0.f ? 1.f : slope), w[c * K + k], acc);
-                }
-            }
-#pragma unroll
-            for (int d = 32; d >= 1; d >>= 1) acc += __shfl_xor(acc, d, 64);
-            if (lane == 0) gv[p] = acc;
-        }
-    }
+        return;
+    }
+    const int p = blockIdx.x - n_wb;
+    if (!gv || p >= B * K) return;
+    const int b = p / K, k = p - b * K;
+    float acc = 0.f;
+    for (int s = 0; s < S; ++s) {
+        const float *w = nullptr;
+#pragma unroll
+        for (int j = 0; j < SC_MAX_LAYERS; ++j)
+            if (j == s) w = bank.w[j];
+        for (int c = lane; c < C; c += 64) {
+            const int64_t o = ((int64_t)s * B + b) * C + c;
+            acc = fmaf(gout[o] * (out[o] > 0.f ? 1.f : slope), w[c * K + k], acc);
+        }
+    }
+#pragma unroll
+    for (int d = 32; d >= 1; d >>= 1) acc += __shfl_xor(acc, d, 64);
+    if (lane == 0) gv[p] = acc;
 }
 }
 
@@ -620,8 +621,10 @@
     hipStream_t st = static_cast<hipStream_t>(stream);
     {
         ProfScope ps("scalar_conv_bwd", st, 4.0 * S * B * C * K, 4.0 * (2.0 * S * B * C + 2.0 * S * C * (K + 1) + 2.0 * B * K));
-        hipLaunchKernelGGL(scalar_conv_bwd_kernel, dim3(1), dim3(256), 0, st, bank, v, out, grad_out, grad_weight, grad_bias, grad_v,
-                           S, B, K, C, slope);
+        const int n_wb = (grad_weight || grad_bias) ? (int)ceil_div(S * C, 64) : 0, n_v = grad_v ? B * K : 0;
+        if (n_wb + n_v > 0)
+            hipLaunchKernelGGL(scalar_conv_bwd_kernel, dim3((unsigned)(n_wb + n_v)), dim3(64), 0, st, bank, v, out, grad_out, grad_weight,
+                               grad_bias, grad_v, n_wb, S, B, K, C, slope);
     }
     return check_launch("scalar_conv_bwd");
 }
diff --git a/ebfi-be_amd/csrc/imgops.hip b/ebfi-be_amd/csrc/imgops.hip
--- a/ebfi-be_amd/csrc/imgops.hip
+++ b/ebfi-be_amd/csrc/imgops.hip
@@ -155,6 +155,162 @@
     const float g = acc * norm * grad_loss[0] / (float)C;
     const int64_t hw = (int64_t)H * W;
     for (int c = 0; c < C; ++c) grad_x[((int64_t)b * C + c) * hw + (int64_t)py * W + px] = g;
+}
+
+__device__ __forceinline__ float census_rsq(float s) { return __builtin_amdgcn_rsqf(s); }
+
+template <bool TWO>
+__device__ __forceinline__ void census_stage3(const float *__restrict__ xa, const float *__restrict__ xb, const float *__restrict__ y,
+                                              int C, int H, int W, int b, int ty0, int tx0, float (*ga)[CTW + 1],
+                                              float (*gb)[CTW + 1], float (*gy)[CTW + 1]) {
+    const int64_t hw = (int64_t)H * W;
+    const float invc = 1.f / (float)C;
+    for (int i = threadIdx.x; i < CTW * CTW; i += CT * CT) {
+        const int ly = i / CTW, lx = i - ly * CTW;
+        const int py = ty0 + ly - CR, px = tx0 + lx - CR;
+        float sa = 0.f, sb = 0.f, sy = 0.f;
+        if (py >= 0 && py < H && px >= 0 && px < W) {
+            const int64_t o = (int64_t)b * C * hw + (int64_t)py * W + px;
+            if (C == 3) {
+                const float a0 = xa[o], a1 = xa[o + hw], a2 = xa[o + 2 * hw];
+                const float y0 = y[o], y1 = y[o + hw], y2 = y[o + 2 * hw];
+                float b0 = 0.f, b1 = 0.f, b2 = 0.f;
+                if (TWO) { b0 = xb[o]; b1 = xb[o + hw]; b2 = xb[o + 2 * hw]; }
+                sa = ((sa + a0) + a1) + a2;
+                sy = ((sy + y0) + y1) + y2;
+                sb = ((sb + b0) + b1) + b2;
+            } else {
+                for (int c = 0; c < C; ++c) {
+                    sa += xa[o + c * hw];
+                    sy += y[o + c * hw];
+                    if (TWO) sb += xb[o + c * hw];
+                }
+            }
+            sa *= invc;
+            sb *= invc;
+            sy *= invc;
+        }
+        ga[ly][lx] = sa;
+        gy[ly][lx] = sy;
+        if (TWO) gb[ly][lx] = sb;
+    }
+}
+
+__device__ __forceinline__ float census_fterm(float dx, float ty) {
+    const float u = fmaf(dx, census_rsq(fmaf(dx, dx, 0.81f)), -ty);
+    return __fdiv_rn(__fmul_rn(u, u), fmaf(u, u, 0.1f));
+}
+
+__device__ __forceinline__ void census_tile_sum(float acc, float *red, float *dst) {
+#pragma unroll
+    for (int d = 32; d >= 1; d >>= 1) acc += __shfl_xor(acc, d, 64);
+    if ((threadIdx.x & 63) == 0) red[threadIdx.x >> 6] = acc;
+    __syncthreads();
+    if (threadIdx.x == 0) *dst = (red[0] + red[1]) + (red[2] + red[3]);
+}
+
+template <bool TWO>
+__global__ __launch_bounds__(CT *CT) void census2_fwd_kernel(const float *__restrict__ xa, const float *__restrict__ xb,
+                                                             const float *__restrict__ y, float *__restrict__ partial, int64_t P,
+                                                             int C, int H, int W) {
+    __shared__ float ga[CTW][CTW + 1], gb[TWO ? CTW : 1][CTW + 1], gy[CTW][CTW + 1];
+    __shared__ float red[2][4];
+    const int b = blockIdx.z, ty0 = blockIdx.y * CT, tx0 = blockIdx.x * CT;
+    census_stage3<TWO>(xa, xb, y, C, H, W, b, ty0, tx0, ga, gb, gy);
+    __syncthreads();
+    const int ly = threadIdx.x / CT, lx = threadIdx.x % CT;
+    const int py = ty0 + ly, px = tx0 + lx;
+    float acca = 0.f, accb = 0.f;
+    if (py >= CR && py < H - CR && px >= CR && px < W - CR) {
+        const float ca = ga[ly + CR][lx + CR], cy = gy[ly + CR][lx + CR], cb = TWO ? gb[ly + CR][lx + CR] : 0.f;
+#pragma unroll
+        for (int i = 0; i < 7; ++i)
+#pragma unroll
+            for (int j = 0; j < 7; ++j) {
+                const float dy = gy[ly + i][lx + j] - cy;
+                const float ty = __fmul_rn(dy, census_rsq(fmaf(dy, dy, 0.81f)));
+                acca += census_fterm(ga[ly + i][lx + j] - ca, ty);
+                if (TWO) accb += census_fterm(gb[ly + i][lx + j] - cb, ty);
+            }
+        acca *= (1.f / 49.f);
+        accb *= (1.f / 49.f);
+    }
+    const int64_t tile = ((int64_t)b * gridDim.y + blockIdx.y) * gridDim.x + blockIdx.x;
+    census_tile_sum(acca, red[0], partial + tile);
+    if (TWO) census_tile_sum(accb, red[1], partial + P + tile);
+}
+
+template <bool TWO>
+__global__ __launch_bounds__(256) void census2_finish_kernel(const float *__restrict__ partial, int64_t P, float n, float wa, float wb,
+                                                             float *__restrict__ loss) {
+    __shared__ float red[2][4];
+    float sa = 0.f, sb = 0.f;
+    for (int64_t i = threadIdx.x; i < P; i += 256) {
+        sa += partial[i];
+        if (TWO) sb += partial[P + i];
+    }
+#pragma unroll
+    for (int d = 32; d >= 1; d >>= 1) {
+        sa += __shfl_xor(sa, d, 64);
+        if (TWO) sb += __shfl_xor(sb, d, 64);
+    }
+    if ((threadIdx.x & 63) == 0) {
+        red[0][threadIdx.x >> 6] = sa;
+        red[1][threadIdx.x >> 6] = sb;
+    }
+    __syncthreads();
+    if (threadIdx.x == 0) {
+        const float la = __fmul_rn(wa, __fdiv_rn((red[0][0] + red[0][1]) + (red[0][2] + red[0][3]), n));
+        const float lb = __fmul_rn(wb, __fdiv_rn((red[1][0] + red[1][1]) + (red[1][2] + red[1][3]), n));
+        loss[0] = TWO ? la + lb : la;
+    }
+}
+
+__device__ __forceinline__ float census_dterm_t(float dx, float ty) {
+    const float rx = census_rsq(fmaf(dx, dx, 0.81f));
+    const float u = fmaf(dx, rx, -ty);
+    const float den = fmaf(u, u, 0.1f);
+    return __fmul_rn(__fdiv_rn(__fmul_rn(0.2f, u), __fmul_rn(den, den)), __fmul_rn(__fmul_rn(__fmul_rn(0.81f, rx), rx), rx));
+}
+
+template <bool TWO>
+__global__ __launch_bounds__(CT *CT) void census2_bwd_kernel(const float *__restrict__ xa, const float *__restrict__ xb,
+                                                             const float *__restrict__ y, const float *__restrict__ grad_loss,
+                                                             float wa, float wb, float *__restrict__ grad_xa,
+                                                             float *__restrict__ grad_xb, int C, int H, int W, float norm) {
+    __shared__ float ga[CTW][CTW + 1], gb[TWO ? CTW : 1][CTW + 1], gy[CTW][CTW + 1];
+    const int b = blockIdx.z, ty0 = blockIdx.y * CT, tx0 = blockIdx.x * CT;
+    census_stage3<TWO>(xa, xb, y, C, H, W, b, ty0, tx0, ga, gb, gy);
+    __syncthreads();
+    const int ly = threadIdx.x / CT, lx = threadIdx.x % CT;
+    const int py = ty0 + ly, px = tx0 + lx;
+    if (py >= H || px >= W) return;
+    const float ca = ga[ly + CR][lx + CR], cy = gy[ly + CR][lx + CR], cb = TWO ? gb[ly + CR][lx + CR] : 0.f;
+    const float self_in = (py >= CR && py < H - CR && px >= CR && px < W - CR) ? 1.f : 0.f;
+    float acca = 0.f, accb = 0.f;
+#pragma unroll
+    for (int i = 0; i < 7; ++i) {
+        const int qy = py + (i - CR);
+        const bool row_in = qy >= CR && qy < H - CR;
+#pragma unroll
+        for (int j = 0; j < 7; ++j) {
+            const int qx = px + (j - CR);
+            const float wgt = self_in + ((row_in && qx >= CR && qx < W - CR) ? 1.f : 0.f);
+            const float dy = gy[ly + i][lx + j] - cy;
+            const float ty = __fmul_rn(dy, census_rsq(fmaf(dy, dy, 0.81f)));
+            acca = fmaf(-wgt, census_dterm_t(ga[ly + i][lx + j] - ca, ty), acca);
+            if (TWO) accb = fmaf(-wgt, census_dterm_t(gb[ly + i][lx + j] - cb, ty), accb);
+        }
+    }
+    const float gl = grad_loss[0];
+    const float g_a = __fdiv_rn(__fmul_rn(__fmul_rn(acca, norm), __fmul_rn(gl, wa)), (float)C);
+    const float g_b = __fdiv_rn(__fmul_rn(__fmul_rn(accb, norm), __fmul_rn(gl, wb)), (float)C);
+    const int64_t hw = (int64_t)H * W;
+    for (int c = 0; c < C; ++c) {
+        const int64_t o = ((int64_t)b * C + c) * hw + (int64_t)py * W + px;
+        grad_xa[o] = g_a;
+        if (TWO) grad_xb[o] = g_b;
+    }
 }
 
 template <bool REPLICATE>
@@ -267,3 +423,56 @@
     }
     return check_launch("census_bwd");
 }
+
+static int census_pair_check(const char *who, const void *xa, const void *y, int B, int C, int H, int W) {
+    if (!xa || !y) return fail(EBFI_ERR_ARG, "%s: null argument", who);
+    if (B < 0 || C <= 0 || H <= 0 || W <= 0 || B > 65535) return fail(EBFI_ERR_ARG, "%s: bad dimensions", who);
+    return EBFI_OK;
+}
+
+extern "C" int ebfi_census_pair_forward(const float *xa, const float *xb, const float *y, float wa, float wb, float *partial,
+                                        float *loss, int B, int C, int H, int W, void *stream) {
+    if (int rc = census_pair_check("census_pair_forward", xa, y, B, C, H, W)) return rc;
+    if (!partial || !loss) return fail(EBFI_ERR_ARG, "census_pair_forward: null argument");
+    if (B == 0) return fail(EBFI_ERR_ARG, "census_pair_forward: empty batch");
+    hipStream_t st = static_cast<hipStream_t>(stream);
+    const int64_t P = ebfi_census_partials(B, H, W);
+    const dim3 grid(ceil_div(W, CT), ceil_div(H, CT), B);
+    const float n = (float)((double)B * (double)H * (double)W);
+    {
+        ProfScope ps("census2_fwd", st, 0.0, 4.0 * (xb ? 3 : 2) * B * C * (double)H * W);
+        if (xb)
+            hipLaunchKernelGGL(census2_fwd_kernel<true>, grid, dim3(CT * CT), 0, st, xa, xb, y, partial, P, C, H, W);
+        else
+            hipLaunchKernelGGL(census2_fwd_kernel<false>, grid, dim3(CT * CT), 0, st, xa, xb, y, partial, P, C, H, W);
+    }
+    if (int rc = check_launch("census2_fwd")) return rc;
+    {
+        ProfScope ps("census2_finish", st, 0.0, 4.0 * (xb ? 2 : 1) * (double)P);
+        if (xb)
+            hipLaunchKernelGGL(census2_finish_kernel<true>, dim3(1), dim3(256), 0, st, partial, P, n, wa, wb, loss);
+        else
+            hipLaunchKernelGGL(census2_finish_kernel<false>, dim3(1), dim3(256), 0, st, partial, P, n, wa, wb, loss);
+    }
+    return check_launch("census2_finish");
+}
+
+extern "C" int ebfi_census_pair_backward(const float *xa, const float *xb, const float *y, float wa, float wb, const float *grad_loss,
+                                         float *grad_xa, float *grad_xb, int B, int C, int H, int W, void *stream) {
+    if (int rc = census_pair_check("census_pair_backward", xa, y, B, C, H, W)) return rc;
+    if (!grad_loss || !grad_xa || (xb && !grad_xb)) return fail(EBFI_ERR_ARG, "census_pair_backward: null argument");
+    if (B == 0) return EBFI_OK;
+    hipStream_t st = static_cast<hipStream_t>(stream);
+    const float norm = (float)(1.0 / (49.0 * (double)B * (double)H * (double)W));
+    const dim3 grid(ceil_div(W, CT), ceil_div(H, CT), B);
+    {
+        ProfScope ps("census2_bwd", st, 0.0, 4.0 * (xb ? 5 : 3) * B * C * (double)H * W);
+        if (xb)
+            hipLaunchKernelGGL(census2_bwd_kernel<true>, grid, dim3(CT * CT), 0, st, xa, xb, y, grad_loss, wa, wb, grad_xa, grad_xb, C, H,
+                               W, norm);
+        else
+            hipLaunchKernelGGL(census2_bwd_kernel<false>, grid, dim3(CT * CT), 0, st, xa, xb, y, grad_loss, wa, wb, grad_xa, grad_xb, C,
+                               H, W, norm);
+    }
+    return check_launch("census2_bwd");
+}
diff --git a/ebfi-be_amd/ebfi_amd/_native.py b/ebfi-be_amd/ebfi_amd/_native.py
--- a/ebfi-be_amd/ebfi_amd/_native.py
+++ b/ebfi-be_amd/ebfi_amd/_native.py
@@ -55,6 +55,8 @@
     "ebfi_conv2d_packed_bytes": (_sz, [_i, _i, _i, _i]),
     "ebfi_conv2d_pack_bf16x3": (_i, [_vp, _i, _i, _i, _i, _vp, _sz, _vp]),
     "ebfi_pack_table_bf16": (_i, [_vp, _vp, _i64, _vp, _vp]),
+    "ebfi_pack_pairs_block": (_i, []),
+    "ebfi_pack_pairs_bf16": (_i, [_vp, _vp, _vp, _vp, _i64, _i64, _vp, _vp]),
     "ebfi_f16_scales_finish": (_i, [_vp, _i, _vp, _vp]),
     "ebfi_pack_table_f16": (_i, [_vp, _vp, _i64, _vp, _vp, _vp, _vp]),
     "ebfi_conv2d_packed_f16": (_i, [_vp, _vp, _sz, _vp, _vp] + [_i] * 8 + [_i, _c.c_float, _vp, _vp, _i, _c.c_float, _vp, _vp, _vp]),
@@ -106,6 +108,8 @@
     "ebfi_census_partials": (_i64, [_i, _i, _i]),
     "ebfi_census_forward": (_i, [_vp, _vp, _vp, _i, _i, _i, _i, _vp]),
     "ebfi_census_backward": (_i, [_vp, _vp, _vp, _vp, _i, _i, _i, _i, _vp]),
+    "ebfi_census_pair_forward": (_i, [_vp, _vp, _vp, _c.c_float, _c.c_float, _vp, _vp, _i, _i, _i, _i, _vp]),
+    "ebfi_census_pair_backward": (_i, [_vp, _vp, _vp, _c.c_float, _c.c_float, _vp, _vp, _vp, _i, _i, _i, _i, _vp]),
     "ebfi_gauss5_forward": (_i, [_vp, _vp, _i64, _i, _i, _c.c_float, _vp]),
     "ebfi_gauss5_backward": (_i, [_vp, _vp, _i64, _i, _i, _c.c_float, _vp]),
     "ebfi_ed_head_workspace": (_sz, [_i, _i, _i64]),
diff --git a/ebfi-be_amd/ebfi_amd/engine.py b/ebfi-be_amd/ebfi_amd/engine.py
--- a/ebfi-be_amd/ebfi_amd/engine.py
+++ b/ebfi-be_amd/ebfi_amd/engine.py
@@ -112,6 +112,7 @@
             from . import f16scale
             self.book = f16scale.ScaleBook(self.device)
             self.bank.attach_scale_book(self.book)
+            self.bank.pack_on_demand = True
             self.book.forward_f16 = forward_f16
 
     @property
@@ -200,6 +201,8 @@
                 s.copy_(v)
             guard = self._guard()
             saved = None if guard is None else guard.clone()
+            if self.bank is not None and not self._graphs:
+                self.bank.forget_requests()
             side = torch.cuda.Stream(self.device)
             side.wait_stream(torch.cuda.current_stream(self.device))
             with torch.cuda.stream(side):
diff --git a/ebfi-be_amd/ebfi_amd/loss.py b/ebfi-be_amd/ebfi_amd/loss.py
--- a/ebfi-be_amd/ebfi_amd/loss.py
+++ b/ebfi-be_amd/ebfi_amd/loss.py
@@ -57,6 +57,49 @@
             rc = N.lib().ebfi_census_backward(N.ptr(x), N.ptr(y), N.ptr(g), N.ptr(gx), B, C, H, W, N.stream_ptr(x.device))
         N.check(rc, "ebfi_census_backward")
         return gx, None
+
+
+class _CensusPair(torch.autograd.Function):
+
+    @staticmethod
+    def forward(ctx, a, b, target, coef_a, coef_b):
+        a, target = a.contiguous(), target.contiguous()
+        b = b.contiguous() if b is not None else None
+        B, C, H, W = a.shape
+        lib = N.lib()
+        partial = torch.empty(2 * int(lib.ebfi_census_partials(B, H, W)), dtype=torch.float32, device=a.device)
+        loss = torch.empty((), dtype=torch.float32, device=a.device)
+        with torch.cuda.device_of(a):
+            rc = lib.ebfi_census_pair_forward(N.ptr(a), N.ptr(b) if b is not None else None, N.ptr(target), float(coef_a),
+                                              float(coef_b), N.ptr(partial), N.ptr(loss), B, C, H, W, N.stream_ptr(a.device))
+        N.check(rc, "ebfi_census_pair_forward")
+        ctx.save_for_backward(*((a, target) if b is None else (a, target, b)))
+        ctx.coefs = (float(coef_a), float(coef_b))
+        return loss
+
+    @staticmethod
+    def backward(ctx, g):
+        a, target = ctx.saved_tensors[:2]
+        b = ctx.saved_tensors[2] if len(ctx.saved_tensors) > 2 else None
+        B, C, H, W = a.shape
+        g = g.contiguous().float().reshape(1)
+        ga = torch.empty_like(a)
+        gb = torch.empty_like(b) if b is not None else None
+        with torch.cuda.device_of(a):
+            rc = N.lib().ebfi_census_pair_backward(N.ptr(a), N.ptr(b) if b is not None else None, N.ptr(target), ctx.coefs[0],
+                                                   ctx.coefs[1], N.ptr(g), N.ptr(ga), N.ptr(gb) if b is not None else None,
+                                                   B, C, H, W, N.stream_ptr(a.device))
+        N.check(rc, "ebfi_census_pair_backward")
+        return ga, gb, None, None, None
+
+
+def census_pair(a, b, target, coef_a, coef_b):
+    N.require_gpu(a, target)
+    if a.dim() != 4 or a.shape != target.shape or (b is not None and b.shape != a.shape) or min(a.shape[-2:]) <= 6:
+        raise ValueError("census_pair takes [B, C, H, W] images of one shape with H, W > 6, got %s" % (tuple(a.shape),))
+    if any(t is not None and t.dtype != torch.float32 for t in (a, b, target)) or target.requires_grad:
+        raise ValueError("census_pair takes float32 images and a target that needs no gradient")
+    return _CensusPair.apply(a, b, target, coef_a, coef_b)
 
 
 class _LapLoss(torch.autograd.Function):
@@ -194,9 +237,7 @@
         if not self.detail_enabled:
             c_sharp, c_pre, sharp_pre = 1.0, 0.0, None
         if _LapLoss.usable(sharp, sharp_pre, target):
-            total = _LapLoss.apply(sharp, sharp_pre, target, c_sharp, c_pre) + c_sharp * self.census(sharp, target)
-            if sharp_pre is not None:
-                total = total + c_pre * self.census(sharp_pre, target)
+            total = _LapLoss.apply(sharp, sharp_pre, target, c_sharp, c_pre) + census_pair(sharp, sharp_pre, target, c_sharp, c_pre)
             return total / accu_step
         with torch.no_grad():
             yp = self.Lap.lap(target)
diff --git a/ebfi-be_amd/ebfi_amd/weightbank.py b/ebfi-be_amd/ebfi_amd/weightbank.py
--- a/ebfi-be_amd/ebfi_amd/weightbank.py
+++ b/ebfi-be_amd/ebfi_amd/weightbank.py
@@ -7,6 +7,11 @@
 
 _ACTIVE = None
 LO_FLAG = 1 << 30
+
+
+class WeightImageError(Exception):
+    """A bf16 image was first asked for at a point where it cannot be packed (inside a stream capture).  Not a RuntimeError on
+    purpose: the Engine treats a RuntimeError during capture as 'continue with eager launches'; this must stop the run."""
 
 
 def active_bank():
@@ -25,9 +30,11 @@
                  "fwd16_off", "fwd16_bytes", "fwd16_tag")
 
     def fwd_ptr(self):
+        self.bank._want(self, "fwd")
         return N._vp(self.bank.packed.data_ptr() + self.fwd_off)
 
     def tr_ptr(self):
+        self.bank._want(self, "tr")
         return N._vp(self.bank.packed.data_ptr() + self.tr_off)
 
     def tr16_ptr(self):
@@ -45,6 +52,9 @@
 
     def bias(self):
         return self.bank.bias_buf[self.bias_off:self.bias_off + self.M] if self.has_bias else None
+
+
+PAIR_BLOCK = 512
 
 
 def _ids_like(p, flat_off):
@@ -82,9 +92,14 @@
         if self.numel >= LO_FLAG:
             raise ValueError("more than 2^30 parameters")
         self.sites = {}
-        self._tables, self._n_packed = [], 0
+        self._pair_tables, self._pair_desc, self._n_blocks, self._n_packed = [], [], 0, 0
+        self._images = {}
         self._bias_tables, self._n_bias = [], 0
-        self.packed = self.table = self.bias_buf = self.bias_table = None
+        self.packed = self.bias_buf = self.bias_table = None
+        self._table = self.pair_table = self.pair_desc = self.block_list = None
+        self.pack_on_demand = False
+        self._wanted, self._n_active, self._n_entries = [], 0, 0
+        self._wanted_set, self._retired = set(), []
         self._stamp = None
         self.book = None
         self._tables16, self._n16, self._segs = [], 0, []
@@ -138,12 +153,20 @@
                 self._tables16.append(torch.cat([img.to(torch.int32), torch.full((padn,), -1, dtype=torch.int32)]))
                 self._segs.append((self._n16, s))
                 self._n16 += img.numel() + padn
+        PB = PAIR_BLOCK
         for name, img in (("fwd", fwd), ("tr", tr)) if need_tr else (("fwd", fwd),):
-            lo = torch.where(img >= 0, img | LO_FLAG, img)
+            n = img.numel()
+            assert n % 16 == 0
             setattr(s, name + "_off", 2 * self._n_packed)
-            setattr(s, name + "_bytes", 4 * img.numel())
-            self._tables += [img.to(torch.int32), lo.to(torch.int32)]
-            self._n_packed += 2 * img.numel()
+            setattr(s, name + "_bytes", 4 * n)
+            nb = (n + PB - 1) // PB
+            self._pair_tables.append(torch.cat([img.to(torch.int32), torch.full((nb * PB - n,), -1, dtype=torch.int32)]))
+            first = self._n_packed + PB * np.arange(nb, dtype=np.int64)
+            self._pair_desc.append(np.stack([first & 0xffffffff, first >> 32, np.full(nb, n, dtype=np.int64),
+                                             np.minimum(PB, n - PB * np.arange(nb, dtype=np.int64))], axis=1))
+            self._images[(key, name)] = (self._n_blocks, nb, n)
+            self._n_blocks += nb
+            self._n_packed += 2 * n
         idn = ids.numpy()
         s.w_inv, s.w_R, s.w_shapes = [], [], [tuple(w.shape) for w in weights]
         for w in weights:
@@ -169,8 +192,26 @@
         self.packed = None
         return s
 
+    @property
+    def table(self):
+        if self._table is None and self._pair_tables:
+            parts = []
+            for (_, _, n), t in zip(self._images.values(), self._pair_tables):
+                img = t[:n]
+                parts += [img, torch.where(img >= 0, img | LO_FLAG, img)]
+            self._table = torch.cat(parts)
+        return self._table
+
     def _finalize(self):
-        self.table = torch.cat(self._tables).to(self.device) if self._tables else None
+        self._table = None
+        if self._pair_tables:
+            self.pair_table = torch.cat(self._pair_tables).to(self.device)
+            self.pair_desc = torch.from_numpy(np.concatenate(self._pair_desc).astype(np.uint32).view(np.int32)).to(self.device)
+            self.block_list = torch.zeros(self._n_blocks, dtype=torch.int32, device=self.device)
+            listed = [self._images[k] for k in self._wanted] if self.pack_on_demand else list(self._images.values())
+            self._n_active = self._n_entries = 0
+            if listed:
+                self._list(np.concatenate([np.arange(first, first + nb) for first, nb, _ in listed]), sum(n for _, _, n in listed))
         self.packed = torch.empty(max(self._n_packed, 8), dtype=torch.bfloat16, device=self.device)
         self.bias_table = torch.cat(self._bias_tables).to(self.device) if self._bias_tables else None
         self.bias_buf = torch.empty(max(self._n_bias, 1), dtype=torch.float32, device=self.device)
@@ -184,6 +225,49 @@
             self.block_slot = torch.repeat_interleave(torch.tensor([site.w_slot for _, site in self._segs], dtype=torch.int32),
                                                       torch.tensor(counts)).to(self.device)
 
+    def _list(self, blocks, n):
+        self.block_list[self._n_active:self._n_active + len(blocks)] = torch.from_numpy(np.asarray(blocks, dtype=np.int32))
+        self._n_active += len(blocks)
+        self._n_entries += n
+
+    def _pack(self, lib, st, start, n_blocks, n_entries):
+        if n_blocks:
+            if lib.ebfi_pack_pairs_block() != PAIR_BLOCK:
+                raise N.EbfiNativeError("the library packs blocks of %d entries, the bank's table has %d"
+                                        % (lib.ebfi_pack_pairs_block(), PAIR_BLOCK))
+            N.check(lib.ebfi_pack_pairs_bf16(N.ptr(self.flat), N.ptr(self.pair_table), N.ptr(self.pair_desc),
+                                             N._vp(self.block_list.data_ptr() + 4 * start), n_blocks, n_entries, N.ptr(self.packed), st),
+                    "ebfi_pack_pairs_bf16")
+
+    def _want(self, site, name):
+        if not self.pack_on_demand or (site.key, name) in self._wanted_set:
+            return
+        if (site.key, name) not in self._images:
+            raise KeyError("site %r has no %s image" % (site.key, name))
+        if self.device.type == "cuda" and torch.cuda.is_current_stream_capturing():
+            raise WeightImageError("weight bank: the bf16 %s image of site %r is first asked for inside a stream capture; the eager "
+                                   "passes before the capture must run the same kernels as the captured one" % (name, site.key))
+        self._wanted.append((site.key, name))
+        self._wanted_set.add((site.key, name))
+        if self.packed is None:
+            self.refresh()
+            return
+        first, nb, n = self._images[(site.key, name)]
+        start = self._n_active
+        self._list(np.arange(first, first + nb), n)
+        with torch.cuda.device(self.device):
+            self._pack(N.lib(), N.stream_ptr(self.device), start, nb, n)
+
+    def packed_images(self):
+        return list(self._wanted) if self.pack_on_demand else list(self._images)
+
+    def forget_requests(self):
+        if self.pack_on_demand and self._wanted:
+            self._wanted, self._wanted_set, self._n_active, self._n_entries = [], set(), 0, 0
+            if self.block_list is not None:
+                self._retired.append(self.block_list)
+                self.block_list = torch.zeros_like(self.block_list)
+
     def attach_scale_book(self, book):
         self.book = book
         self.packed = None
@@ -201,9 +285,8 @@
         lib = N.lib()
         with torch.cuda.device(self.device):
             st = N.stream_ptr(self.device)
-            if self.table is not None:
-                N.check(lib.ebfi_pack_table_bf16(N.ptr(self.flat), N.ptr(self.table), self.table.numel(), N.ptr(self.packed), st),
-                        "ebfi_pack_table_bf16")
+            if self.pair_table is not None:
+                self._pack(lib, st, 0, self._n_active, self._n_entries)
             if self.bias_table is not None:
                 N.check(lib.ebfi_gather_sum(N.ptr(self.flat), N.ptr(self.bias_table), N.ptr(self.bias_buf), self._n_bias, 1, st),
                         "ebfi_gather_sum")
diff --git a/include/ebfi_hip.h b/include/ebfi_hip.h
--- a/include/ebfi_hip.h
+++ b/include/ebfi_hip.h
@@ -109,6 +109,9 @@
 int ebfi_conv2d_pack_bf16x3(const void *weight, int Cin, int Cout, int ksize, int transposed, void *packed,
                             size_t packed_bytes, void *stream);
 int ebfi_pack_table_bf16(const float *src, const int32_t *table, int64_t n, void *out, void *stream);
+int ebfi_pack_pairs_block(void);
+int ebfi_pack_pairs_bf16(const float *src, const int32_t *table, const void *desc, const int32_t *active, int64_t n_active,
+                         int64_t n_entries, void *out, void *stream);
 
 int ebfi_conv2d_thin_forward(const void *input, const void *weight, const void *bias, void *output, int B, int Cin, int H, int W,
                              int Cout, int ksize, int stride, int pad, int act, float slope, void *stream);
@@ -265,6 +268,11 @@
 int ebfi_census_backward(const float *x, const float *y, const float *grad_loss, float *grad_x,
                          int B, int C, int H, int W, void *stream);
 
+int ebfi_census_pair_forward(const float *xa, const float *xb, const float *y, float wa, float wb, float *partial, float *loss,
+                             int B, int C, int H, int W, void *stream);
+int ebfi_census_pair_backward(const float *xa, const float *xb, const float *y, float wa, float wb, const float *grad_loss,
+                              float *grad_xa, float *grad_xb, int B, int C, int H, int W, void *stream);
+
 int64_t ebfi_laploss_workspace_floats(int64_t planes, int H, int W, int levels);
 int64_t ebfi_laploss_partials(int64_t planes, int H, int W, int levels);
 int ebfi_laploss_forward(const float *pred_a, const float *pred_b, const float *target, float coef_a, float coef_b,
```

Result: faster. 564.0 frames/s, median of 6 (+1.5%).
